# TurakhiaLab/TWILIGHT

Hardware: AMD Instinct MI355X
Metric: DP band cells/s, TALCO-XDrop progressive profile-profile alignment (bit-exact vs reference CPU path) (higher is better)
Workload: dtype f32

## Files before the change

include/twl_align.h:

```cpp
#ifndef TWL_ALIGN_H
#define TWL_ALIGN_H

#include <stdint.h>

#ifdef __cplusplus
extern "C" {
#endif

#define TWL_MAX_MATRIX 21
#define TWL_MAX_MARKER 1024

enum twl_status {
    TWL_OK = 0,
    TWL_ERR_NOT_INITIALIZED = -1,
    TWL_ERR_BAD_ARGUMENT = -2,
    TWL_ERR_HIP = -3,
    TWL_ERR_UNSUPPORTED = -4
};

typedef struct twl_params {
    int32_t P;
    float   matrix[TWL_MAX_MATRIX * TWL_MAX_MATRIX];
    float   gap_open;
    float   gap_extend;
    float   gap_boundary;
    float   gap_char;
    int32_t xdrop;
    int32_t flen;
    int32_t marker;
} twl_params;

typedef struct twl_stats {
    uint64_t band_cells;
    uint64_t nominal_cells;
    double   kernel_ms;
    double   pack_ms;
    double   total_ms;
    int32_t  n_launches;
    int32_t  n_relaunched;
    int32_t  window;
    int32_t  grid;
    int32_t  matrix_mode;
    int32_t  speculative;
    int32_t  mt_tiles_predicted;
    int32_t  mt_tiles_inline;
    int32_t  mt_scouts_failed;
    int32_t  reserved;
    char     kernel[160];
} twl_stats;

int  twl_init(const int *device_ids, int n_devices);
void twl_shutdown(void);
const char *twl_last_error(void);
const char *twl_version(void);

int twl_align_batch(const twl_params *p, int32_t n_pairs, int32_t seq_len,
                    const float *freq, const float *gap_open, const float *gap_extend,
                    const int32_t *len, const int32_t *num,
                    int8_t *aln_out, int32_t *aln_len_out, int16_t *err_out);

int twl_align_batch_device(int device, void *stream, const twl_params *p, int32_t n_pairs, int32_t seq_len,
                           const float *d_freq, const float *d_gap_open, const float *d_gap_extend,
                           const int32_t *d_len, const int32_t *d_num,
                           int8_t *d_aln_out, int32_t *d_aln_len_out, int16_t *d_err_out);

void *twl_host_alloc(uint64_t bytes);
void  twl_host_free(void *p);

int twl_copy_to_device(int device, void *dst_dev, const void *src, uint64_t bytes);
int twl_copy_from_device(int device, void *dst, const void *src_dev, uint64_t bytes);
int twl_copy_rows_from_device(int device, void *dst, uint64_t dst_pitch, const void *src_dev, uint64_t src_pitch, uint64_t width, uint64_t rows);

int twl_get_stats(int device, twl_stats *out);

int twl_get_pair_cells(int device, uint64_t *cells_out, int32_t n);

int twl_column_scores(const twl_params *p, int32_t seq_len, const float *freq, const int32_t *len, const int32_t *num, float *out);

int twl_dp_column_scores(const twl_params *p, int32_t seq_len, const float *freq, const float *gap_open, const float *gap_extend,
                         const int32_t *len, const int32_t *num, float *out);

#define TWL_COMM_ID_BYTES 128
int twl_comm_unique_id(void *id128);
int twl_comm_init(int device, int rank, int world, const void *id128);
int twl_comm_all_gather(int device, const void *d_send, void *d_recv, int64_t bytes_per_rank);
int twl_comm_all_gather_host(int device, const void *send, void *recv, int64_t bytes_per_rank);
int twl_comm_destroy(int device);

enum twl_knob { TWL_KNOB_MT_PERTURB = 1, TWL_KNOB_MT_MAX_PAIRS = 2, TWL_KNOB_MT_MIN_MARKER = 3, TWL_KNOB_MT_LEAD = 4, TWL_KNOB_MT_MARGIN = 5,
                TWL_KNOB_MT_ROUNDS = 6, TWL_KNOB_MT_THR_JOBS = 7, TWL_KNOB_FAIL_ROW_ALLOCS = 8,
                TWL_KNOB_PROT_MODE = 9, TWL_KNOB_ASSUME_ONEHOT_QUERY = 10, TWL_KNOB_MT_TAIL_PCT = 11, TWL_KNOB_MT_WIDE = 12, TWL_KNOB_NO_SPEC = 13, TWL_KNOB_SCOUT_XDROP_PCT = 14, TWL_KNOB_THR_SMALL = 15, TWL_KNOB_FORCE_GLOBAL = 16, TWL_KNOB_LEAF_STEP = 17, TWL_KNOB_POISON_TB = 18, TWL_KNOB_MT_ANCHOR = 19, TWL_KNOB_MT_LEAD2 = 20, TWL_KNOB_PROT_CORRIDOR = 21 };
int twl_set_knob(int key, int value);
int twl_plan_describe(const twl_params *p, int32_t n_pairs, const int32_t *len, int32_t num_cu, int32_t qry_onehot, int32_t wide_streak, char *out, int32_t cap);

#ifdef __cplusplus
}
#endif
#endif
```

include/twl_level.h:

```cpp
#ifndef TWL_LEVEL_H
#define TWL_LEVEL_H

#include "twl_align.h"

#ifdef __cplusplus
extern "C" {
#endif

typedef struct twl_store twl_store;

typedef struct twl_side {
    int32_t n_members;
    int32_t member_off;
    int32_t len;
    int32_t num;
    float   weight;
    int32_t cache_id;
    int32_t store_id;
    int32_t reserved;
} twl_side;

int  twl_store_create(int device, char type, int32_t n_seqs, const char *const *seqs, const int32_t *lens, twl_store **out);
void twl_store_destroy(twl_store *s);
int  twl_store_read_rows(twl_store *s, char *const *rows_out, int32_t *lens_out);
int  twl_store_read_rows_of(twl_store *s, int32_t n_ids, const int32_t *ids, char *out, int32_t *lens_out);
int  twl_store_write_rows(twl_store *s, int32_t n_ids, const int32_t *ids, const char *in, const int32_t *lens);
int  twl_store_write_cache(twl_store *s, int32_t id, const float *data, int32_t len);
int  twl_store_rows_to_block(twl_store *s, int32_t n_ids, const int32_t *ids, void *dev_block, int32_t *lens_out);
int  twl_store_rows_from_block(twl_store *s, int32_t n_ids, const int32_t *ids, const int32_t *lens, const void *dev_block);
int  twl_store_exchange_buffers(twl_store *s, int64_t send_bytes, int64_t recv_bytes, void **send_dev, void **recv_dev);
int  twl_store_read_cache(twl_store *s, int32_t id, float *out, int32_t *len_out);
int  twl_store_drop_cache(twl_store *s, int32_t id);

int twl_level_prepare(twl_store *s, const twl_params *p, float gappy_threshold, int32_t n_pairs, const twl_side *sides,
                      const int32_t *members, const float *member_weight, int32_t seq_len, int32_t *len_out, uint8_t *colinfo_out);

int twl_level_read_colinfo(twl_store *s, int32_t pair, int32_t side, uint8_t *out);
int twl_level_read_colinfo_many(twl_store *s, int32_t n_sel, const int32_t *pairs, uint8_t *out);

int twl_level_align(twl_store *s, const twl_params *p, const uint8_t *run_mask, int8_t *aln_out, int32_t *aln_len_out, int16_t *err_out);
int twl_level_align_mixed(twl_store *s, const twl_params *p, const uint8_t *run_mask, const uint8_t *zero_gap, int8_t *aln_out, int32_t *aln_len_out, int16_t *err_out);

int twl_level_read_path(twl_store *s, int32_t pair, int8_t *out, int32_t len);
int twl_level_read_paths(twl_store *s, int32_t n_sel, const int32_t *pairs, const int32_t *lens, int8_t *out, int32_t out_stride);

int twl_level_restore(twl_store *s, const twl_params *p, int32_t n_sel, const int32_t *pairs, int32_t out_stride, int32_t *final_len_out);
int twl_level_exchange_buffers(twl_store *s, int64_t send_bytes, int64_t recv_bytes, void **send_dev, void **recv_dev);
int twl_level_paths_to_block(twl_store *s, int32_t n_sel, const int32_t *pairs, const int32_t *lens, const uint8_t *where, void *blk_dev, const int64_t *blk_off);
int twl_level_paths_from_block(twl_store *s, int32_t n_sel, const int32_t *pairs, const int32_t *lens, const void *blk_dev, const int64_t *blk_off);
int twl_level_write_final(twl_store *s, int32_t pair, const int8_t *path, int32_t len);
int twl_level_read_final(twl_store *s, int32_t pair, int8_t *out, int32_t len);

int twl_level_commit(twl_store *s, const int8_t *paths, const int32_t *path_len, int32_t path_stride);

int twl_level_commit_from_dp(twl_store *s, const int8_t *paths, const int32_t *path_len, int32_t path_stride, const uint8_t *from_dp);

int twl_level_read_columns(twl_store *s, int32_t pair, int32_t side, float *out, int32_t max_cols);

int twl_level_timing(twl_store *s, double *prepare_ms, double *commit_ms);

#ifdef __cplusplus
}
#endif
#endif
```

twilight_amd/api.py:

```python
from __future__ import annotations

import ctypes as C
import os

import numpy as np

_HERE = os.path.dirname(os.path.abspath(__file__))
LIB_PATH = os.environ.get("TWL_LIB") or os.path.join(_HERE, "libtwl_align.so")
TWL_MAX_MATRIX = 21

_lib = None


class TwlError(RuntimeError):
    pass


class TwlParams(C.Structure):
    _fields_ = [("P", C.c_int32), ("matrix", C.c_float * (TWL_MAX_MATRIX * TWL_MAX_MATRIX)), ("gap_open", C.c_float),
                ("gap_extend", C.c_float), ("gap_boundary", C.c_float), ("gap_char", C.c_float), ("xdrop", C.c_int32),
                ("flen", C.c_int32), ("marker", C.c_int32)]


class TwlStats(C.Structure):
    _fields_ = [("band_cells", C.c_uint64), ("nominal_cells", C.c_uint64), ("kernel_ms", C.c_double),
                ("pack_ms", C.c_double), ("total_ms", C.c_double), ("n_launches", C.c_int32),
                ("n_relaunched", C.c_int32), ("window", C.c_int32), ("grid", C.c_int32), ("matrix_mode", C.c_int32), ("speculative", C.c_int32),
                ("mt_tiles_predicted", C.c_int32), ("mt_tiles_inline", C.c_int32), ("mt_scouts_failed", C.c_int32), ("reserved", C.c_int32),
                ("kernel", C.c_char * 160)]


_SYMBOLS = ["twl_init", "twl_shutdown", "twl_last_error", "twl_version", "twl_align_batch", "twl_align_batch_device",
            "twl_get_stats", "twl_get_pair_cells", "twl_column_scores", "twl_dp_column_scores", "twl_host_alloc", "twl_host_free", "twl_set_knob",
            "twl_copy_to_device", "twl_copy_from_device", "twl_copy_rows_from_device",
            "twl_comm_unique_id", "twl_comm_init", "twl_comm_all_gather", "twl_comm_all_gather_host", "twl_comm_destroy", "twl_plan_describe"]


def exported_symbols():
    return list(_SYMBOLS)


def load_library():
    global _lib
    if _lib is None:
        if not os.path.exists(LIB_PATH):
            raise TwlError(f"{LIB_PATH} not built: run `python -c 'import __graft_entry__ as g; g.build()'`")
        try:
            import torch
        except Exception:
            pass
        lib = C.CDLL(LIB_PATH)
        lib.twl_last_error.restype = C.c_char_p
        lib.twl_version.restype = C.c_char_p
        lib.twl_init.restype = C.c_int
        lib.twl_align_batch.restype = C.c_int
        lib.twl_align_batch_device.restype = C.c_int
        lib.twl_get_stats.restype = C.c_int
        lib.twl_get_pair_cells.restype = C.c_int
        lib.twl_column_scores.restype = C.c_int
        lib.twl_dp_column_scores.restype = C.c_int
        lib.twl_shutdown.restype = None
        lib.twl_set_knob.restype = C.c_int
        _lib = lib
    return _lib


def _check(rc):
    if rc != 0:
        raise TwlError(f"libtwl_align error {rc}: {load_library().twl_last_error().decode()}")


def make_params(matrix, *, gap_open=-50.0, gap_extend=-5.0, gap_boundary=None, gap_char=None, xdrop=None, flen=4096,
                marker=1024) -> TwlParams:
    m = np.asarray(matrix, dtype=np.float32)
    n = m.shape[0]
    p = TwlParams()
    p.P = n + 1
    flat = np.zeros(TWL_MAX_MATRIX * TWL_MAX_MATRIX, dtype=np.float32)
    flat[: n * n] = m.reshape(-1)
    p.matrix[:] = flat.tolist()
    p.gap_open = gap_open
    p.gap_extend = gap_extend
    p.gap_boundary = gap_extend if gap_boundary is None else gap_boundary
    p.gap_char = gap_extend if gap_char is None else gap_char
    p.xdrop = int(1000 * -gap_extend) if xdrop is None else int(xdrop)
    p.flen = flen
    p.marker = marker
    return p


def init(device_ids=None):
    lib = load_library()
    if device_ids is None:
        _check(lib.twl_init(None, 0))
    else:
        arr = (C.c_int * len(device_ids))(*device_ids)
        _check(lib.twl_init(arr, len(device_ids)))


def shutdown():
    load_library().twl_shutdown()


def _ptr(a, ty):
    return a.ctypes.data_as(C.POINTER(ty))


def align_batch(params: TwlParams, batch):
    lib = load_library()
    n, sl = batch.n_pairs, batch.seq_len
    freq = np.ascontiguousarray(batch.freq, dtype=np.float32)
    go = np.ascontiguousarray(batch.gap_open, dtype=np.float32)
    ge = np.ascontiguousarray(batch.gap_extend, dtype=np.float32)
    ln = np.ascontiguousarray(batch.len, dtype=np.int32)
    nm = np.ascontiguousarray(batch.num, dtype=np.int32)
    aln = np.zeros((n, 2 * sl), dtype=np.int8)
    aln_len = np.zeros(n, dtype=np.int32)
    err = np.zeros(n, dtype=np.int16)
    _check(lib.twl_align_batch(C.byref(params), C.c_int32(n), C.c_int32(sl), _ptr(freq, C.c_float), _ptr(go, C.c_float),
                               _ptr(ge, C.c_float), _ptr(ln, C.c_int32), _ptr(nm, C.c_int32), _ptr(aln, C.c_int8),
                               _ptr(aln_len, C.c_int32), _ptr(err, C.c_int16)))
    return aln, aln_len, err


def align_batch_device(params: TwlParams, n_pairs, seq_len, d_freq, d_gop, d_gex, d_len, d_num, d_aln, d_aln_len, d_err,
                       device=0, stream=None):
    lib = load_library()
    vp = C.c_void_p
    _check(lib.twl_align_batch_device(C.c_int(device), vp(stream or 0), C.byref(params), C.c_int32(n_pairs), C.c_int32(seq_len),
                                      vp(d_freq), vp(d_gop), vp(d_gex), vp(d_len), vp(d_num), vp(d_aln), vp(d_aln_len),
                                      vp(d_err)))


KNOB_MT_PERTURB, KNOB_MT_MAX_PAIRS, KNOB_MT_MIN_MARKER, KNOB_MT_LEAD, KNOB_MT_MARGIN, KNOB_MT_ROUNDS, KNOB_MT_THR_JOBS, KNOB_FAIL_ROW_ALLOCS = 1, 2, 3, 4, 5, 6, 7, 8
KNOB_PROT_MODE, KNOB_ASSUME_ONEHOT_QUERY, KNOB_MT_TAIL_PCT, KNOB_MT_WIDE, KNOB_NO_SPEC, KNOB_SCOUT_XDROP_PCT = 9, 10, 11, 12, 13, 14
KNOB_THR_SMALL = 15
KNOB_FORCE_GLOBAL = 16
KNOB_LEAF_STEP = 17
KNOB_POISON_TB = 18
KNOB_MT_ANCHOR = 19
KNOB_PROT_CORRIDOR = 21
KNOB_MT_LEAD2 = 20
PROT_MODES = {"auto": 0, "dense": 1, "sparse": 2, "presim": 3, "r1": 4, "lean_sparse": 5, "lean_presim": 6}


def set_knob(key: int, value: int):
    _check(load_library().twl_set_knob(C.c_int(key), C.c_int(value)))


def plan_describe(params, lens, num_cu=256, qry_onehot=False, wide_streak=0, small_state=0) -> str:
    wide_streak = int(wide_streak) + (100000 * (32 + int(small_state)) if small_state else 0)
    lens = np.ascontiguousarray(lens, dtype=np.int32)
    buf = C.create_string_buffer(256)
    _check(load_library().twl_plan_describe(C.byref(params), C.c_int32(lens.shape[0]), _ptr(lens, C.c_int32), C.c_int32(num_cu), C.c_int32(int(qry_onehot)), C.c_int32(wide_streak), buf, C.c_int32(256)))
    return buf.value.decode()


def version() -> str:
    return load_library().twl_version().decode()


def get_stats(device=0) -> TwlStats:
    st = TwlStats()
    _check(load_library().twl_get_stats(C.c_int(device), C.byref(st)))
    return st


def get_pair_cells(n, device=0):
    out = np.zeros(n, dtype=np.uint64)
    _check(load_library().twl_get_pair_cells(C.c_int(device), _ptr(out, C.c_uint64), C.c_int32(n)))
    return out


def column_scores(params: TwlParams, ref: np.ndarray, qry: np.ndarray, ref_num: int, qry_num: int) -> np.ndarray:
    ref = np.ascontiguousarray(ref, dtype=np.float32)
    qry = np.ascontiguousarray(qry, dtype=np.float32)
    R, Q, P = ref.shape[0], qry.shape[0], ref.shape[1]
    sl = max(R, Q)
    freq = np.zeros((2, sl, P), dtype=np.float32)
    freq[0, :R] = ref
    freq[1, :Q] = qry
    ln = np.array([R, Q], dtype=np.int32)
    nm = np.array([ref_num, qry_num], dtype=np.int32)
    out = np.zeros((Q, R), dtype=np.float32)
    _check(load_library().twl_column_scores(C.byref(params), C.c_int32(sl), _ptr(freq, C.c_float), _ptr(ln, C.c_int32), _ptr(nm, C.c_int32), _ptr(out, C.c_float)))
    return out


def dp_column_scores(params: TwlParams, batch, pair: int = 0) -> np.ndarray:
    sl = batch.seq_len
    freq = np.ascontiguousarray(batch.freq[pair], dtype=np.float32)
    gop = np.ascontiguousarray(batch.gap_open[pair], dtype=np.float32)
    gex = np.ascontiguousarray(batch.gap_extend[pair], dtype=np.float32)
    ln = np.ascontiguousarray(batch.len[pair], dtype=np.int32)
    nm = np.ascontiguousarray(batch.num[pair], dtype=np.int32)
    out = np.zeros((int(ln[1]), int(ln[0])), dtype=np.float32)
    _check(load_library().twl_dp_column_scores(C.byref(params), C.c_int32(sl), _ptr(freq, C.c_float), _ptr(gop, C.c_float), _ptr(gex, C.c_float),
                                               _ptr(ln, C.c_int32), _ptr(nm, C.c_int32), _ptr(out, C.c_float)))
    return out
```

twilight_amd/csrc/host/align_resident.cpp:

```cpp
#include "align_gpu.hpp"

#include <cstring>
#include <omp.h>

#include <algorithm>
#include <cstdio>
#include <cstdlib>
#include <iostream>
#include <string>
#include <thread>

namespace msa {
namespace progressive {
namespace gpu {

namespace {

inline twl_store *firstStore(const RunCtx &ctx) { return ctx.stores.empty() ? nullptr : ctx.stores[0]; }

std::vector<RunCtx::Raw> g_alnStage;
RunCtx::Raw g_finalStage, g_infoStage;

void createStore(RunCtx &ctx, SequenceDB *db, Option *option)
{
    const int n = (int)db->sequences.size();
    std::vector<const char *> rows(n);
    std::vector<int32_t> lens(n);
    for (int i = 0; i < n; ++i) {
        auto *s = db->sequences[i];
        if (s->id != i) { std::cerr << "ERROR: sequence ids are not dense.\n"; exit(1); }
        rows[i] = s->alnStorage[s->storage];
        lens[i] = s->len;
    }
    ctx.storeDev = selectedDevices();
    if (option->testVirtualDevices > 0) ctx.storeDev.assign((size_t)option->testVirtualDevices, selectedDevices()[0]);
    ctx.stores.assign(ctx.storeDev.size(), nullptr);
    std::vector<std::thread> th;
    std::vector<std::pair<int, std::string>> res(ctx.storeDev.size(), {TWL_OK, ""});
    for (size_t d = 0; d < ctx.storeDev.size(); ++d)
        th.emplace_back([&, d] {
            const int rc = twl_store_create(ctx.storeDev[d], option->type, n, rows.data(), lens.data(), &ctx.stores[d]);
            if (rc != TWL_OK) res[d] = {rc, twl_last_error()};
        });
    for (auto &t : th) t.join();
    for (auto &r : res)
        if (r.first != TWL_OK) { std::cerr << "ERROR: twl_store_create failed (" << r.first << "): " << r.second << '\n'; exit(1); }
}

template <class F>
void onAllStores(RunCtx &ctx, const char *what, F fn)
{
    const size_t nd = ctx.stores.size();
    std::vector<std::pair<int, std::string>> res(nd, {TWL_OK, ""});
    if (nd == 1) { const int rc = fn(0); if (rc != TWL_OK) res[0] = {rc, twl_last_error()}; }
    else {
        std::vector<std::thread> th;
        for (size_t d = 0; d < nd; ++d)
            th.emplace_back([&, d] { const int rc = fn((int)d); if (rc != TWL_OK) res[d] = {rc, twl_last_error()}; });
        for (auto &t : th) t.join();
    }
    for (auto &r : res)
        if (r.first != TWL_OK) { std::cerr << "ERROR: " << what << " failed (" << r.first << "): " << r.second << '\n'; exit(1); }
}

void materialise(Tree *T, SequenceDB *db, Option *option)
{
    RunCtx &ctx = ctxOf(db);
    if (!firstStore(ctx)) return;
    const double t0 = nowMs();
    const int n = (int)db->sequences.size();
    std::vector<int32_t> lens(n);
    int rc = twl_store_read_rows(firstStore(ctx), nullptr, lens.data());
    if (rc != TWL_OK) die("twl_store_read_rows", rc);
    std::vector<char *> rows(n);
    size_t total = 0;
    for (int i = 0; i < n; ++i) total += (size_t)lens[i];
    free(db->rowArena);
    db->rowArena = static_cast<char *>(malloc(2 * total + 1));
    if (!db->rowArena) { std::cerr << "ERROR: out of host memory for the final rows.\n"; exit(1); }
    size_t at = 0;
    for (int i = 0; i < n; ++i) {
        auto *s = db->sequences[i];
        if (!s->borrowed) { free(s->alnStorage[0]); free(s->alnStorage[1]); }
        s->borrowed = true;
        s->alnStorage[s->storage] = db->rowArena + at;
        s->alnStorage[!s->storage] = db->rowArena + total + at;
        s->memLen = lens[i];
        rows[i] = s->alnStorage[s->storage];
        at += (size_t)lens[i];
    }
    rc = twl_store_read_rows(firstStore(ctx), rows.data(), lens.data());
    if (rc != TWL_OK) die("twl_store_read_rows", rc);
    for (int i = 0; i < n; ++i) db->sequences[i]->len = lens[i];
    const int P = (option->type == 'n') ? 6 : 22;
    std::vector<Node *> keep{T->root};
    keep.insert(keep.end(), db->fallback_nodes.begin(), db->fallback_nodes.end());
    for (Node *nd : keep) {
        if (nd->cacheId < 0) continue;
        int32_t len = 0;
        if ((rc = twl_store_read_cache(firstStore(ctx), nd->cacheId, nullptr, &len)) != TWL_OK) die("twl_store_read_cache", rc);
        std::vector<float> flat((size_t)len * P);
        if ((rc = twl_store_read_cache(firstStore(ctx), nd->cacheId, flat.data(), &len)) != TWL_OK) die("twl_store_read_cache", rc);
        nd->msaFreq.assign(len, std::vector<float>(P));
        for (int t = 0; t < len; ++t) std::copy(&flat[(size_t)t * P], &flat[(size_t)t * P] + P, nd->msaFreq[t].begin());
        nd->cacheId = -1;
    }
    for (twl_store *st : ctx.stores) twl_store_destroy(st);
    ctx.stores.clear();
    ctx.finished = true;
    if (option->printDetail) std::cerr << "Rows back on the host in " << nowMs() - t0 << " ms\n";
}

struct PathRoute { bool procs, devX, inPlace; };
PathRoute routeOf(const Shard &sh, int nd)
{
    PathRoute r;
    r.procs = sh.world > 1;
    r.devX = (nd == 1 && (sh.exchangeDev != nullptr || sh.rccl));
    r.inPlace = (nd == 1 && ((!r.procs && !sh.exchange && !sh.rccl) || r.devX));
    return r;
}

struct Level {
    const RunCtx &ctx;
    const NodePairVec &nodes;
    SequenceDB *database;
    Option *option;
    Params &param;
    int task, n, nd;
    const char *letters;
    bool removal;
    PathRoute route;
    twl_params tp, tz;
    std::vector<twl_side> sides;
    std::vector<PairShape> ps;
    std::vector<int32_t> members;
    std::vector<float> weights;
    int stride = 1;
    int pathStride = 1;
    std::vector<int> needInfo;
    std::vector<char> needsHost;
    std::vector<uint8_t> maskZero;
    std::vector<char> takesPart;
    std::vector<int> owner;
    int meBase = 0;
    Level(const RunCtx &c, const NodePairVec &nv, SequenceDB *db, Option *o, Params &p)
        : ctx(c), nodes(nv), database(db), option(o), param(p), task(db->currentTask), n((int)nv.size()), nd((int)c.stores.size()),
          letters(consensusLetters(o->type)), removal(!(o->gappyVertical == 1.0)), route(routeOf(c.shard, nd)), tp(baseParams(p)), tz(tp)
    {
        tz.gap_char = 0;
    }
};

struct PairRows {
    std::vector<alnPath> paths;
    std::vector<int16_t> errs;
    std::vector<uint8_t> fromDp;
    std::vector<int32_t> dpLen;
    std::vector<ColumnInfo> cols;
    explicit PairRows(int n) : paths(n), errs(n, 0), fromDp(n, 0), dpLen(n, 0), cols(n) {}
};

struct ReplicaShare {
    double callMs = 0, totMs = 0;
    LevelRecord part;
    uint64_t nominalCells = 0;
    std::vector<int32_t> handedBack, handedBackLen;
};

void describeLevel(Level &lv, RunCtx &ctx, NodePairVec &nodes)
{
    const int n = lv.n;
    SequenceDB *database = lv.database;
    Option *option = lv.option;
    std::vector<twl_side> &sides = lv.sides;
    sides.resize(2 * (size_t)n);
    lv.ps.resize(n);
    size_t nMembers = 0;
#pragma omp parallel for schedule(static) if (n >= 512)
    for (int i = 0; i < n; ++i) {
        Node *nd[2] = {nodes[i].first, nodes[i].second};
        PairShape &s = lv.ps[i];
        s.refLen = nd[0]->getAlnLen(0); s.qryLen = nd[1]->getAlnLen(0);
        s.refNum = nd[0]->getAlnNum(0); s.qryNum = nd[1]->getAlnNum(0);
        for (int sd = 0; sd < 2; ++sd) {
            twl_side &x = sides[2 * (size_t)i + sd];
            x.n_members = (int32_t)nd[sd]->seqsIncluded.size();
            x.len = sd ? s.qryLen : s.refLen;
            x.num = sd ? s.qryNum : s.refNum;
            x.weight = nd[sd]->alnWeight;
            x.cache_id = nd[sd]->cacheId;
            x.store_id = -1;
            x.reserved = 0;
        }
        s.lowQ_r = lowQualitySide(option->alnMode == MERGE_MSA, s.refNum, firstSeqLowQuality(nd[0], database));
        s.lowQ_q = lowQualitySide(option->alnMode == MERGE_MSA, s.qryNum, firstSeqLowQuality(nd[1], database));
    }
    for (int i = 0; i < n; ++i) {
        const PairShape &s = lv.ps[i];
        Node *nd[2] = {nodes[i].first, nodes[i].second};
        const bool storeFreq = (s.refNum >= option->calProfileTh || s.qryNum >= option->calProfileTh) || (sides[2 * (size_t)i].cache_id >= 0 || sides[2 * (size_t)i + 1].cache_id >= 0);
        for (int sd = 0; sd < 2; ++sd) {
            twl_side &x = sides[2 * (size_t)i + sd];
            x.member_off = (int32_t)nMembers;
            if (storeFreq && x.cache_id < 0) x.store_id = nd[sd]->cacheId = ctx.nextCacheId++;
            nMembers += (size_t)x.n_members;
            lv.stride = std::max(lv.stride, x.len);
        }
        lv.pathStride = std::max(lv.pathStride, s.refLen + s.qryLen);
    }
    lv.members.resize(nMembers);
    lv.weights.resize(nMembers);
#pragma omp parallel for schedule(dynamic, 16) if (n >= 64)
    for (int i = 0; i < n; ++i) {
        Node *nd[2] = {nodes[i].first, nodes[i].second};
        for (int sd = 0; sd < 2; ++sd) {
            const twl_side &x = sides[2 * (size_t)i + sd];
            const float groupWeight = nd[sd]->alnWeight;
            for (int m = 0; m < x.n_members; ++m) {
                const int sIdx = nd[sd]->seqsIncluded[m];
                if (sIdx < 0) { std::cerr << "ERROR: compressed sequence group in device-resident mode.\n"; exit(1); }
                lv.members[x.member_off + m] = sIdx;
                lv.weights[x.member_off + m] = database->sequences[sIdx]->weight / groupWeight * x.num;
            }
        }
    }
}

void prepareOnReplicas(Level &lv, RunCtx &ctx)
{
    const int n = lv.n;
    std::vector<int32_t> lens(2 * (size_t)n);
    std::vector<std::vector<int32_t>> lensOf(lv.nd);
    onAllStores(ctx, "twl_level_prepare", [&](int d) {
        lensOf[d].resize(2 * (size_t)n);
        return twl_level_prepare(ctx.stores[d], &lv.tp, lv.option->gappyVertical, n, lv.sides.data(), lv.members.data(), lv.weights.data(), lv.stride,
                                 d == 0 ? lens.data() : lensOf[d].data(), nullptr);
    });
    for (int d = 1; d < lv.nd; ++d)
        if (lensOf[d] != lens) { std::cerr << "ERROR: device replicas disagree on the prepared level.\n"; exit(1); }
    lv.needsHost.assign(n, 0);
    for (int i = 0; i < n; ++i) {
        PairShape &s = lv.ps[i];
        s.lens = {lens[2 * i], lens[2 * i + 1]};
        if (s.lens.first != s.refLen || s.lens.second != s.qryLen) { lv.needInfo.push_back(i); lv.needsHost[i] = 1; }
    }
}

void fetchColumnInfo(const Level &lv, const std::vector<int> &which, bool wholeBlock, std::vector<ColumnInfo> &cols)
{
    if (which.empty()) return;
    const size_t stride = (size_t)lv.stride;
    uint8_t *info = reinterpret_cast<uint8_t *>(g_infoStage.get(2 * (wholeBlock ? (size_t)lv.n : which.size()) * stride));
    const int rc = wholeBlock ? twl_level_read_colinfo(firstStore(lv.ctx), -1, 0, info)
                              : twl_level_read_colinfo_many(firstStore(lv.ctx), (int32_t)which.size(), which.data(), info);
    if (rc != TWL_OK) die(wholeBlock ? "twl_level_read_colinfo" : "twl_level_read_colinfo_many", rc);
#pragma omp parallel for schedule(dynamic, 4)
    for (int t = 0; t < (int)which.size(); ++t) {
        const int i = which[t];
        const size_t slot = wholeBlock ? (size_t)i : (size_t)t;
        runsAndConsensus(&info[2 * slot * stride], lv.ps[i].refLen, lv.removal, lv.letters, cols[i].gappy.first, cols[i].consensus.first);
        runsAndConsensus(&info[(2 * slot + 1) * stride], lv.ps[i].qryLen, lv.removal, lv.letters, cols[i].gappy.second, cols[i].consensus.second);
    }
}

void planDp(Level &lv, PairRows &rows)
{
    const int n = lv.n;
    lv.maskZero.assign(n, 0);
    lv.takesPart.assign(n, 0);
    std::vector<long long> cost(n, 0);
    for (int i = 0; i < n; ++i) {
        const PairShape &s = lv.ps[i];
        rows.paths[i] = trivialPath(s);
        cost[i] = (long long)s.lens.first + s.lens.second;
        if (!goesToDp(s)) continue;
        lv.takesPart[i] = 1;
        lv.maskZero[i] = zeroGapChar(lv.task, s) ? 1 : 0;
    }
    lv.owner = dealPairs(cost, lv.takesPart, lv.route.procs ? lv.ctx.shard.world : lv.nd);
    lv.meBase = lv.route.procs ? lv.ctx.shard.rank : 0;
}

void addStats(const Level &lv, int d, bool firstCall, ReplicaShare &mine)
{
    const bool ownDevice = lv.nd == 1 || lv.ctx.storeDev[d] != lv.ctx.storeDev[(d + 1) % lv.nd];
    const bool nominal = firstCall && d == 0;
    twl_stats st{};
    if ((!ownDevice && !nominal) || twl_get_stats(lv.ctx.storeDev[d], &st) != TWL_OK) return;
    if (ownDevice) { foldStats(mine.part, st); mine.part.kernel_ms += st.kernel_ms; mine.totMs += st.total_ms; }
    if (nominal) mine.nominalCells += st.nominal_cells;
}

int retryDeferredPair(const Level &lv, int d, const std::vector<uint8_t> &mask, int8_t *aln, std::vector<int32_t> &alnLen, std::vector<int16_t> &err, ReplicaShare &mine)
{
    if (lv.n != 1) { std::cerr << "ERROR: a deferred-pass (task 1) level must hold exactly one pair; this one has " << lv.n << ".\n"; return (int)TWL_ERR_UNSUPPORTED; }
    if (!mask[0]) return (int)TWL_OK;
    twl_params tr = lv.maskZero[0] ? lv.tz : lv.tp;
    const uint8_t one = 1;
    int rc = TWL_OK;
    retryUntilPassed(tr, err[0], std::min(lv.ps[0].lens.first, lv.ps[0].lens.second), [&](const twl_params &grown) {
        if (lv.option->printDetail) std::cout << "Retry pair No. " << 0 << "\txdrop " << grown.xdrop << " flen " << grown.flen << '\n';
        const double tRetry = nowMs();
        rc = twl_level_align(lv.ctx.stores[d], &grown, &one, aln, alnLen.data(), err.data());
        if (rc != TWL_OK) return (int16_t)0;
        mine.callMs += nowMs() - tRetry;
        addStats(lv, d, false, mine);
        return err[0];
    });
    return rc;
}

int sortResults(const Level &lv, int d, const std::vector<uint8_t> &mask, const int8_t *aln, const std::vector<int32_t> &alnLen, const std::vector<int16_t> &err,
                PairRows &rows, ReplicaShare &mine)
{
    const size_t pitch = (size_t)2 * lv.stride;
    std::vector<int32_t> restore, restoreLen;
    for (int i = 0; i < lv.n; ++i) {
        if (!mask[i]) continue;
        rows.errs[i] = err[i];
        const int32_t len = (err[i] == 0) ? alnLen[i] : 0;
        if (!lv.route.inPlace) rows.paths[i].assign(&aln[i * pitch], &aln[i * pitch] + len);
        else if (lv.needsHost[i]) {
            if (len > 0 && !deferredLowQuality(lv.task, lv.ps[i])) { restore.push_back(i); restoreLen.push_back(len); } else rows.paths[i].clear();
        }
        else if (len > 0) { rows.fromDp[i] = 1; rows.dpLen[i] = len; }
    }
    if (restore.empty()) return (int)TWL_OK;
    std::vector<int32_t> fin(restore.size(), -1);
    const int rc = twl_level_restore(lv.ctx.stores[d], &lv.tp, (int32_t)restore.size(), restore.data(), lv.pathStride, fin.data());
    if (rc != TWL_OK) return rc;
    for (size_t t = 0; t < restore.size(); ++t) {
        if (fin[t] > 0) { rows.fromDp[restore[t]] = 2; rows.dpLen[restore[t]] = fin[t]; }
        else { mine.handedBack.push_back(restore[t]); mine.handedBackLen.push_back(restoreLen[t]); }
    }
    return (int)TWL_OK;
}

int alignShare(const Level &lv, int d, PairRows &rows, ReplicaShare &mine)
{
    const int n = lv.n;
    std::vector<uint8_t> mask(n, 0);
    int cnt = 0, cntZero = 0;
    for (int i = 0; i < n; ++i) if (lv.takesPart[i] && lv.owner[i] == lv.meBase + d) { mask[i] = 1; ++cnt; cntZero += lv.maskZero[i]; }
    if (!cnt) return (int)TWL_OK;
    int8_t *aln = lv.route.inPlace ? nullptr : reinterpret_cast<int8_t *>(g_alnStage[d].get((size_t)n * 2 * lv.stride));
    std::vector<int32_t> alnLen(n);
    std::vector<int16_t> err(n);
    const double tCall = nowMs();
    const int rc = (cntZero == cnt) ? twl_level_align(lv.ctx.stores[d], &lv.tz, mask.data(), aln, alnLen.data(), err.data())
                                    : twl_level_align_mixed(lv.ctx.stores[d], &lv.tp, mask.data(), cntZero ? lv.maskZero.data() : nullptr, aln, alnLen.data(), err.data());
    if (rc != TWL_OK) return rc;
    mine.callMs += nowMs() - tCall;
    addStats(lv, d, true, mine);
    if (lv.task == 1) {
        const int rr = retryDeferredPair(lv, d, mask, aln, alnLen, err, mine);
        if (rr != TWL_OK) return rr;
    }
    return sortResults(lv, d, mask, aln, alnLen, err, rows, mine);
}

#ifdef TWL_DEV
void dumpSchedule(const Level &lv, const PairRows &rows)
{
    const char *dump = getenv("TWL_DUMP_SCHEDULE");
    FILE *f = dump ? fopen(dump, "a") : nullptr;
    if (!f) return;
    std::vector<uint64_t> pc(lv.n, 0);
    if (lv.nd == 1) (void)twl_get_pair_cells(lv.ctx.storeDev[0], pc.data(), lv.n);
    for (int i = 0; i < lv.n; ++i)
        fprintf(f, "%d %d %d %d %d %d %d %llu\n", (int)lv.ctx.levels.size(), i, lv.nodes[i].first->seqsIncluded.empty() ? -1 : lv.nodes[i].first->seqsIncluded[0],
                lv.nodes[i].second->seqsIncluded.empty() ? -1 : lv.nodes[i].second->seqsIncluded[0], lv.ps[i].lens.first, lv.ps[i].lens.second, (int)rows.errs[i], (unsigned long long)pc[i]);
    fclose(f);
}
#endif

void mergeShares(const std::vector<ReplicaShare> &shares, RunCtx &ctx, LevelRecord &rec)
{
    double callMs = 0, totMs = 0;
    for (const ReplicaShare &s : shares) {
        callMs = std::max(callMs, s.callMs); totMs = std::max(totMs, s.totMs);
        rec.kernel_ms = std::max(rec.kernel_ms, s.part.kernel_ms);
        rec.band_cells += s.part.band_cells;
        rec.relaunched += s.part.relaunched;
    }
    const LevelRecord &p0 = shares[0].part;
    rec.matrix_mode = p0.matrix_mode; rec.speculative = p0.speculative; memcpy(rec.kernel, p0.kernel, sizeof rec.kernel);
    rec.mt_predicted += p0.mt_predicted; rec.mt_inline += p0.mt_inline;
    ctx.totals.call_ms += callMs;
    ctx.totals.total_ms += totMs;
    ctx.totals.nominal_cells += shares[0].nominalCells;
}

void postCheck(const Level &lv, int i, int alnRef, int alnQry)
{
    const PairShape &s = lv.ps[i];
    if (alnRef != s.refLen) std::cout << "R: Post " << lv.nodes[i].first->identifier << "(" << alnRef << "/" << s.refLen << ")\n";
    if (alnQry != s.qryLen) std::cout << "Q: Post " << lv.nodes[i].second->identifier << "(" << alnQry << "/" << s.qryLen << ")\n";
}

void joinHandedBack(const Level &lv, const ReplicaShare &share, PairRows &rows)
// ... 81 lines not shown
}

const char *consensusLetters(char type)
{
    static const char bases[] = {'A', 'C', 'G', 'T', 'N'};
    static const char acids[] = {'A', 'C', 'D', 'E', 'F', 'G', 'H', 'I', 'K', 'L', 'M', 'N', 'P', 'Q', 'R', 'S', 'T', 'V', 'W', 'Y', 'X'};
    return type == 'n' ? bases : acids;
}

IntPair restoreOnHost(alnPath &dp, ColumnInfo &cols, Params &param, int pathStride, alnPath &full)
{
    auto covers = [](const alnPath &p) { IntPair c{0, 0}; for (auto a : p) { c.first += a != 1; c.second += a != 2; } return c; };
    alignment_helper::addGappyColumnsBack(dp, full, cols.gappy, param, covers(dp), cols.consensus);
    if ((int)full.size() > pathStride) { std::cerr << "ERROR: path longer than both profiles together.\n"; exit(1); }
    return covers(full);
}

std::vector<int32_t> restoreHandedBack(twl_store *st, Params &param, const Option &option, const AlignedLevel &lv, const std::vector<int32_t> &pairs,
                                       const std::vector<int32_t> &dpLen, const std::function<void(int, int, int)> &post)
{
    const size_t sl = (size_t)lv.stride, m = pairs.size();
    const bool removal = !(option.gappyVertical == 1.0f);
    const char *letters = consensusLetters(option.type);
    std::vector<uint8_t> info(m * 2 * sl);
    std::vector<int8_t> raw(m * 2 * sl);
    int rc = twl_level_read_colinfo_many(st, (int32_t)m, pairs.data(), info.data());
    if (rc != TWL_OK) die("twl_level_read_colinfo_many", rc);
    if ((rc = twl_level_read_paths(st, (int32_t)m, pairs.data(), dpLen.data(), raw.data(), (int32_t)(2 * sl))) != TWL_OK) die("twl_level_read_paths", rc);
    std::vector<int32_t> fin(m);
    for (size_t k = 0; k < m; ++k) {
        const int32_t i = pairs[k];
        ColumnInfo c;
        runsAndConsensus(&info[2 * k * sl], lv.sideLen[2 * i], removal, letters, c.gappy.first, c.consensus.first);
        runsAndConsensus(&info[(2 * k + 1) * sl], lv.sideLen[2 * i + 1], removal, letters, c.gappy.second, c.consensus.second);
        alnPath dp(&raw[2 * k * sl], &raw[2 * k * sl] + dpLen[k]), full;
        const IntPair covers = restoreOnHost(dp, c, param, lv.pathStride, full);
        if (post) post(i, covers.first, covers.second);
        if ((rc = twl_level_write_final(st, i, full.data(), (int32_t)full.size())) != TWL_OK) die("twl_level_write_final", rc);
        fin[k] = (int32_t)full.size();
    }
    return fin;
}

FinalPaths finalPathsOfLevel(twl_store *st, const twl_params &tp, Params &param, const Option &option, const AlignedLevel &lv)
{
    FinalPaths f;
    f.fromDp.assign((size_t)lv.n, 0);
    f.pathLen.assign((size_t)lv.n, 0);
    std::vector<int32_t> sel;
    for (int32_t i = 0; i < lv.n; ++i) {
        if (lv.err[i] != 0) continue;
        f.pathLen[i] = lv.alnLen[i];
        f.fromDp[i] = 1;
        if (lv.lenOut[2 * i] < lv.sideLen[2 * i] || lv.lenOut[2 * i + 1] < lv.sideLen[2 * i + 1]) sel.push_back(i);
    }
    if (sel.empty()) return f;
    std::vector<int32_t> fin(sel.size(), -1), host, hostLen;
    const int rc = twl_level_restore(st, &tp, (int32_t)sel.size(), sel.data(), lv.pathStride, fin.data());
    if (rc != TWL_OK) die("twl_level_restore", rc);
    for (size_t k = 0; k < sel.size(); ++k) {
        f.fromDp[sel[k]] = 2;
        if (fin[k] > 0) f.pathLen[sel[k]] = fin[k];
        else { host.push_back(sel[k]); hostLen.push_back(lv.alnLen[sel[k]]); }
    }
    if (!host.empty()) {
        const std::vector<int32_t> full = restoreHandedBack(st, param, option, lv, host, hostLen);
        for (size_t k = 0; k < host.size(); ++k) f.pathLen[host[k]] = full[k];
        f.restoredOnHost = (int)host.size();
    }
    return f;
}

void alignWithRetry(twl_store *st, int device, const twl_params &prm, const Option &option, const std::string *retryWhat, const int16_t *knownErr, int32_t minLen,
                    int32_t *alnLen, int16_t *err, DpTotals &tot)
{
    auto runOnce = [&](const twl_params &p) {
        const int rc = twl_level_align(st, &p, nullptr, nullptr, alnLen, err);
        if (rc != TWL_OK) die("twl_level_align", rc);
        twl_stats ss{};
        if (twl_get_stats(device, &ss) == TWL_OK) { tot.cells += ss.band_cells; tot.kernel += ss.kernel_ms; }
        return err[0];
    };
    const int16_t first = knownErr ? *knownErr : runOnce(prm);
    if (!retryWhat) return;
    twl_params tr = prm;
    retryUntilPassed(tr, first, minLen, [&](const twl_params &grown) {
        ++tot.retries;
        if (option.printDetail) std::cout << "Retry " << *retryWhat << "\txdrop " << grown.xdrop << " flen " << grown.flen << '\n';
        return runOnce(grown);
    });
}

void runsAndConsensus(const uint8_t *info, int len, bool removal, const char *letters, IntPairVec &runs, std::string &cons)
{
    cons.resize(len);
    int start = -1;
    for (int t = 0; t < len; ++t) {
        cons[t] = letters[info[t] & 0x7f];
        if (!removal) continue;
        if (info[t] & 0x80) { if (start < 0) start = t; }
        else if (start >= 0) { runs.push_back({start, t - start}); start = -1; }
    }
    if (removal && start >= 0) runs.push_back({start, len - start});
}

void uploadSequences(SequenceDB *database, Option *option)
{
    RunCtx &ctx = ctxOf(database);
    if (firstStore(ctx) || ctx.finished) return;
    ensureInit(option);
    const double t0 = nowMs();
    createStore(ctx, database, option);
    for (auto *s : database->sequences) {
        if (!s->borrowed) { free(s->alnStorage[0]); free(s->alnStorage[1]); }
        s->alnStorage[0] = s->alnStorage[1] = nullptr;
        s->borrowed = true;
        s->memLen = 0;
    }
    if (option->printDetail) std::cerr << "Sequences resident on " << ctx.stores.size() << " device replica(s) in " << nowMs() - t0 << " ms\n";
    database->afterMainPass = [database, option](Tree *tree) { materialise(tree, database, option); };
    database->residentDeferred = true;
}

void downloadRows(SequenceDB *database, Tree *T)
{
    if (database->afterMainPass) { database->afterMainPass(T); database->afterMainPass = nullptr; }
}

void alignmentKernel_Resident(Tree *T, NodePairVec &nodes, SequenceDB *database, Option *option, Params &param)
{
    RunCtx &ctx = ctxOf(database);
    const int task = database->currentTask;
    if ((task != 0 && task != 1) || ctx.finished) {
        if (firstStore(ctx)) materialise(T, database, option);
        alignmentKernel_GPU(T, nodes, database, option, param);
        return;
    }
    refuseCpuOnly(option);
    ensureInit(option);
    uploadSequences(database, option);
    if (ctx.shard.world > 1 && ctx.stores.size() > 1) { std::cerr << "ERROR: several processes with several device replicas each are not supported.\n"; exit(1); }
    LevelRecord rec;
    rec.pairs = (int32_t)nodes.size();
    rec.task = task;
    const LevelTotals before = ctx.totals;
    const double tPrep = nowMs();
    const int n = (int)nodes.size(), nd = (int)ctx.stores.size();
    Level level(ctx, nodes, database, option, param);
    describeLevel(level, ctx, nodes);
    prepareOnReplicas(level, ctx);
    const Level &lv = level;
    PairRows rows(n);
    if (!lv.route.inPlace) fetchColumnInfo(lv, lv.needInfo, lv.needInfo.size() * 8 > (size_t)n, rows.cols);
    ctx.totals.prepare_ms += nowMs() - tPrep;

    planDp(level, rows);
    std::vector<ReplicaShare> shares(nd);
    if (g_alnStage.size() < (size_t)nd) g_alnStage.resize((size_t)nd);
    onAllStores(ctx, "twl_level_align", [&](int d) { return alignShare(lv, d, rows, shares[d]); });
#ifdef TWL_DEV
    dumpSchedule(lv, rows);
#endif
    mergeShares(shares, ctx, rec);
    joinHandedBack(lv, shares[0], rows);
    exchange(lv, ctx, rows, rec);
    std::vector<int> fallbackPairs = judgeFailures(lv, rows);

    const double tFin = nowMs();
    std::vector<int32_t> finalLen(n, 0);
    std::vector<char> deferred(n, 0);
    const int8_t *finalPaths = finalPathsOnHost(lv, rows, finalLen, deferred);
    const double tGappy = nowMs() - tFin;
    commitAndBookkeep(lv, ctx, nodes, finalPaths, finalLen, rows);
    ctx.totals.finish_ms += nowMs() - tFin;
    double devPrep = 0, devCommit = 0;
    if (option->printDetail) twl_level_timing(firstStore(ctx), &devPrep, &devCommit);
    ctx.totals.dev_prepare_ms += devPrep;
    ctx.totals.dev_commit_ms += devCommit;
    closeLevel(ctx, rec, tPrep, deferred, fallbackPairs, nodes, database, option);
    if (option->printDetail)
        std::cerr << "  phases (ms): prepare " << ctx.totals.prepare_ms - before.prepare_ms << " (device " << devPrep << ") call " << ctx.totals.call_ms - before.call_ms
                  << " (kernel " << rec.kernel_ms << ", exchange " << rec.exchange_ms << ") finish " << ctx.totals.finish_ms - before.finish_ms << " (device " << devCommit
                  << ") whole " << nowMs() - tPrep << "; relaunched pairs " << ctx.totals.relaunched - before.relaunched << "; pairs with removed columns " << lv.needInfo.size() << "; restored on the host " << shares[0].handedBack.size() << "; gappy columns back " << tGappy << " ms\n";
}

}
}
}
```

twilight_amd/csrc/host/progressive.cpp:

```cpp
#include "twl_host.hpp"

#include <algorithm>
#include <chrono>
#include <iostream>
#include <unordered_map>

namespace msa {
namespace progressive {

void getProgressivePairs(std::vector<std::pair<NodePair, int>> &alnOrder, std::stack<Node *> postStack, int grpID, int mode)
{
    struct LevelOf {
        std::vector<int> lvl;
        std::vector<const Node *> own;
        int &operator[](Node *n)
        {
            const int k = n->schedIdx;
            if (k < 0 || k >= (int)lvl.size() || own[k] != n) { n->schedIdx = (int)lvl.size(); lvl.push_back(-1); own.push_back(n); }
            return lvl[n->schedIdx];
        }
    } levelOf;
    levelOf.lvl.reserve(postStack.size() + 16);
    levelOf.own.reserve(postStack.size() + 16);
    auto nextLevel = [&](Node *id) { const int l = levelOf[id]; return l < 0 ? 0 : l + 1; };
    if (mode == 0) {
        std::vector<Node *> children, left;
        for (; !postStack.empty(); postStack.pop()) {
            Node *node = postStack.top();
            if (!(node->grpID == -1 || node->grpID == grpID) || node->is_leaf()) continue;
            children.clear();
            for (Node *c : node->children)
                if (c->grpID == grpID) children.push_back(c);
            if (children.empty() && node->seqsIncluded.empty()) {
                node->grpID = -2;
                auto &sib = node->parent->children;
                for (auto it = sib.begin(); it != sib.end(); ++it)
                    if ((*it)->identifier == node->identifier) { sib.erase(it); break; }
                continue;
            }
            if (children.size() == 1 && node->parent != nullptr && node->seqsIncluded.empty() && node->parent->grpID == grpID) {
                for (auto &slot : node->parent->children)
                    if (slot->identifier == node->identifier) {
                        slot = children[0];
                        children[0]->branchLength += node->branchLength;
                        children[0]->parent = node->parent;
                        break;
                    }
                continue;
            }
            while (children.size() > 1) {
                left.clear();
                for (size_t i = 0; i + 1 < children.size(); i += 2) {
                    const int lvl = std::max(nextLevel(children[i]), nextLevel(children[i + 1]));
                    levelOf[children[i]] = lvl;
                    levelOf[children[i + 1]] = lvl;
                    alnOrder.push_back({{children[i], children[i + 1]}, lvl});
                    left.push_back(children[i]);
                }
                if (children.size() % 2 == 1) left.push_back(children.back());
                children.swap(left);
            }
            if (children.size() == 1 && !node->seqsIncluded.empty()) {
                const int lvl = std::max(nextLevel(node), nextLevel(node->children[0]));
                levelOf[node] = lvl;
                levelOf[node->children[0]] = lvl;
                alnOrder.push_back({{node, node->children[0]}, lvl});
            }
            { const int l = levelOf[children[0]]; levelOf[node] = l; }
        }
    } else if (mode == 1) {
        for (; !postStack.empty(); postStack.pop()) {
            Node *node = postStack.top();
            if (node->parent == nullptr) continue;
            const int lvl = std::max(nextLevel(node), nextLevel(node->parent));
            levelOf[node] = lvl;
            levelOf[node->parent] = lvl;
            alnOrder.push_back({{node->parent, node}, lvl});
        }
    } else {
        for (; !postStack.empty(); postStack.pop())
            if (postStack.top()->parent != nullptr) alnOrder.push_back({{postStack.top()->parent, postStack.top()}, 0});
    }
}

void scheduling(Node *root, std::vector<NodePairVec> &levels, int mode)
{
    levels.clear();
    std::stack<Node *> post;
    root->collectPostOrder(post);
    std::vector<std::pair<NodePair, int>> pairs;
    getProgressivePairs(pairs, post, root->grpID, mode);
    for (auto &h : pairs) {
        if (levels.size() < (size_t)h.second + 1) levels.resize(h.second + 1);
        levels[h.second].push_back(h.first);
    }
}

static void materialise(Node *n, Node *partner, SequenceDB *db)
{
    if (n->is_leaf() && n->seqsIncluded.empty()) {
        auto *s = db->name_map.find(n->identifier)->second;
        n->seqsIncluded.push_back(s->id);
        n->alnLen = s->len;
        n->alnNum = 1;
        n->alnWeight = s->weight;
    } else if (n->seqsIncluded.empty()) {
        const int grp = n->grpID;
        for (Node *c : n->children) {
            if ((c->grpID == -1 || c->grpID == grp) && c->identifier != partner->identifier) {
                n->msaFreq = c->msaFreq;
                c->msaFreq.clear();
                n->cacheId = c->cacheId;
                c->cacheId = -1;
                n->seqsIncluded = std::move(c->seqsIncluded);
                c->seqsIncluded.clear();
                n->alnLen = c->alnLen;
                n->alnNum = c->alnNum;
                n->alnWeight = c->alnWeight;
                break;
            }
        }
    }
}

void updateNode(Tree *, NodePairVec &nodes, SequenceDB *database)
{
    const int n = (int)nodes.size();
#pragma omp parallel for schedule(static) if (n >= 512)
    for (int i = 0; i < n; ++i) {
        materialise(nodes[i].first, nodes[i].second, database);
        materialise(nodes[i].second, nodes[i].first, database);
    }
}

void progressiveAlignment(Tree *T, SequenceDB *database, Option *option, std::vector<NodePairVec> &levels, Params &param, alnFunction kernel)
{
    int level = 0;
    if (option->printDetail) std::cerr << "Total " << levels.size() << " levels.\n";
    size_t done = 0;
    if (database->ownedPrefix && database->currentTask == 0) done = database->ownedPrefix(T, levels, option, param);
    for (auto m : levels) {
        if ((size_t)level < done) { ++level; continue; }
        auto t0 = std::chrono::high_resolution_clock::now();
        updateNode(T, m, database);
        auto t1 = std::chrono::high_resolution_clock::now();
        kernel(T, m, database, option, param);
        auto ms = std::chrono::duration_cast<std::chrono::milliseconds>(std::chrono::high_resolution_clock::now() - t0).count();
        if (option->printDetail)
            std::cerr << "Level " << level + 1 << ", aligned " << m.size() << (m.size() > 1 ? " pairs in " : " pair in ") << ms << " ms (nodes "
                      << std::chrono::duration<double, std::milli>(t1 - t0).count() << " ms)\n";
        ++level;
    }
}

void updateAlignment(Node *node, SequenceDB *database)
{
    const int n = (int)database->sequences.size();
#pragma omp parallel for schedule(dynamic, 16)
    for (int idx = 0; idx < n; ++idx) {
        auto *s = database->sequences[idx];
        if (s->subtreeIdx >= -1) continue;
        const alnPath &aln = database->subtreeAln[s->subtreeIdx];
        s->memCheck((int)aln.size());
        const char *from = s->alnStorage[s->storage];
        char *to = s->alnStorage[1 - s->storage];
        int org = 0;
        for (size_t k = 0; k < aln.size(); ++k) to[k] = (aln[k] == 0) ? from[org++] : '-';
        s->len = (int)aln.size();
        s->changeStorage();
    }
    std::vector<int> members;
    for (int sIdx : node->seqsIncluded)
        if (sIdx >= 0) members.push_back(sIdx);
    for (auto *s : database->sequences)
        if (s->subtreeIdx < 0) members.push_back(s->id);
    node->seqsIncluded = members;
}

namespace {
struct UnionFind {
    std::vector<int> p;
    int find(int x) { while (p[x] != x) { p[x] = p[p[x]]; x = p[x]; } return x; }
    void unite(int a, int b) { a = find(a); b = find(b); if (a != b) p[std::max(a, b)] = std::min(a, b); }
};
}
OwnershipPlan planOwnership(Tree *T, const std::vector<NodePairVec> &levels, int world)
{
    OwnershipPlan plan;
    const int nLevels = (int)levels.size();
    if (world <= 1 || nLevels < 2) return plan;
    const long long want = 8ll * world;
    std::vector<long long> above((size_t)nLevels + 1, 0);
    for (int l = nLevels - 1; l >= 0; --l) above[l] = above[l + 1] + (long long)levels[l].size();
    int cut = -1;
    for (int l = nLevels - 2; l >= 0; --l)
        if (above[l + 1] + 1 >= want) { cut = l; break; }
    if (cut < 0) return plan;
    std::unordered_map<const Node *, int> idOf;
    auto id = [&](const Node *n) { auto it = idOf.find(n); if (it != idOf.end()) return it->second; const int k = (int)idOf.size(); idOf.emplace(n, k); return k; };
    const int grp = T->root->grpID;
    auto adopts = [&](const Node *c) { return c->grpID == -1 || c->grpID == grp; };
    for (int l = 0; l <= cut; ++l)
        for (auto &pr : levels[l])
            for (const Node *x : {pr.first, pr.second}) {
                id(x);
                if (!x->is_leaf()) for (const Node *c : x->children) if (adopts(c)) id(c);
            }
    UnionFind uf;
    uf.p.resize(idOf.size());
    for (size_t k = 0; k < uf.p.size(); ++k) uf.p[k] = (int)k;
    for (int l = 0; l <= cut; ++l)
        for (auto &pr : levels[l]) {
            uf.unite(idOf[pr.first], idOf[pr.second]);
            for (const Node *x : {pr.first, pr.second})
                if (!x->is_leaf()) for (const Node *c : x->children) if (adopts(c)) uf.unite(idOf[x], idOf[c]);
        }
    std::unordered_map<int, long long> cost;
    std::vector<int> firstSeen;
    for (int l = 0; l <= cut; ++l)
        for (auto &pr : levels[l]) { const int c = uf.find(idOf[pr.first]); if (!cost.count(c)) firstSeen.push_back(c); cost[c] += 1; }
    std::vector<std::pair<long long, int>> order;
    for (size_t k = 0; k < firstSeen.size(); ++k) order.push_back({cost[firstSeen[k]], (int)k});
    std::sort(order.begin(), order.end(), [](const std::pair<long long, int> &a, const std::pair<long long, int> &b) { return a.first != b.first ? a.first > b.first : a.second < b.second; });
    std::unordered_map<int, int> ownerOf;
    plan.load.assign((size_t)world, 0);
    for (auto &c : order) {
        const int r = (int)(std::min_element(plan.load.begin(), plan.load.end()) - plan.load.begin());
        ownerOf[firstSeen[(size_t)c.second]] = r;
        plan.load[r] += c.first;
    }
    plan.cut = cut;
    plan.subtrees = (int)order.size();
    plan.owner.resize((size_t)cut + 1);
    for (int l = 0; l <= cut; ++l) {
        plan.owner[l].resize(levels[l].size());
        for (size_t i = 0; i < levels[l].size(); ++i) plan.owner[l][i] = ownerOf[uf.find(idOf[levels[l][i].first])];
    }
    return plan;
}

void msaOnSubtree(Tree *T, SequenceDB *database, Option *option, Params &param, alnFunction kernel, alnFunction deferredKernel)
{
    auto t0 = std::chrono::high_resolution_clock::now();
    std::cerr << "============================\n";
    std::vector<NodePairVec> levels;
    scheduling(T->root, levels, database->currentTask == 0 ? 0 : 1);
    if (option->printDetail) std::cerr << "Levels scheduled in " << std::chrono::duration<double, std::milli>(std::chrono::high_resolution_clock::now() - t0).count() << " ms\n";
    progressiveAlignment(T, database, option, levels, param, kernel);
    const auto tLoop = std::chrono::high_resolution_clock::now();
    if (database->currentTask == 0) {
        Node *last = levels.back()[0].first;
        T->root->seqsIncluded = last->seqsIncluded;
        if (!last->msaFreq.empty()) T->root->msaFreq = last->msaFreq;
        if (last->cacheId >= 0) { T->root->cacheId = last->cacheId; last->cacheId = -1; }
        T->root->alnLen = last->alnLen;
        T->root->alnNum = last->alnNum;
        T->root->alnWeight = last->alnWeight;
        last->seqsIncluded.clear();
        last->msaFreq.clear();
        const bool stayResident = database->fallback_nodes.empty() ? database->lazyRows : database->residentDeferred;
        if (database->afterMainPass && !stayResident) { database->afterMainPass(T); database->afterMainPass = nullptr; }
    }
    if (database->fallback_nodes.empty()) updateAlignment(T->root, database);
    if (option->printDetail) std::cerr << "After the last level: " << std::chrono::duration<double, std::milli>(std::chrono::high_resolution_clock::now() - tLoop).count() << " ms\n";
    auto secs = std::chrono::duration_cast<std::chrono::seconds>(std::chrono::high_resolution_clock::now() - t0).count();
    std::cerr << "Alignment (length: " << T->root->alnLen << ") completed in " << secs << " s\n";
    if (database->fallback_nodes.empty()) return;

    database->currentTask = 1;
    int deferredSeqs = 0;
    levels.clear();
    for (Node *bad : database->fallback_nodes) deferredSeqs += (int)bad->seqsIncluded.size();
    std::sort(database->fallback_nodes.begin(), database->fallback_nodes.end(), [&](Node *&a, Node *&b) {
        if (a->alnNum == b->alnNum) return a->getAlnLen(database->currentTask) > b->getAlnLen(database->currentTask);
        return a->alnNum > b->alnNum;
    });
    for (Node *bad : database->fallback_nodes) levels.push_back(NodePairVec(1, {T->root, bad}));
    std::cerr << "Realign profiles that have been deferred. Total profiles/sequences: " << database->fallback_nodes.size() << " / " << deferredSeqs << '\n';
    database->fallback_nodes.clear();
    progressiveAlignment(T, database, option, levels, param, deferredKernel);
    if (database->afterMainPass && !database->lazyRows) { database->afterMainPass(T); database->afterMainPass = nullptr; }
    updateAlignment(T->root, database);
    database->currentTask = 0;
}

}
}
```

twilight_amd/csrc/host/twl_host.hpp:

```cpp
#pragma once
#include "level_policy.hpp"

#include <cstdint>
#include <cstdlib>
#include <functional>
#include <map>
#include <stack>
#include <string>
#include <unordered_map>
#include <unordered_set>
#include <utility>
#include <vector>

namespace phylogeny {

using Profile = std::vector<std::vector<float>>;

struct Node {
    Node(const std::string &id, float len);
    Node(const std::string &id, Node *par, float len);
    bool is_leaf() const { return identifier.compare(0, 4, "node") != 0; }
    void collectPostOrder(std::stack<Node *> &postStack);

    std::string identifier;
    Node *parent = nullptr;
    float branchLength = 0;
    size_t level = 1;
    std::vector<Node *> children;
    size_t numLeaves = 0;
    float weight = 0;
    bool placed = false;
    int grpID = -1;
    int schedIdx = -1;

    std::vector<int> seqsIncluded;
    Profile msaFreq;
    int cacheId = -1;
    int alnLen = 0;
    int alnNum = 0;
    float alnWeight = 0;
    int getAlnNum(int) const { return alnNum; }
    int getAlnLen(int) const { return alnLen; }
};

struct Tree {
    size_t m_currInternalNode = 0;
    size_t m_maxDepth = 0;
    size_t m_numLeaves = 0;
    float m_meanDepth = 0;
    Node *root = nullptr;
    std::unordered_map<std::string, Node *> allNodes;

    std::string newInternalNodeId() { return "node_" + std::to_string(++m_currInternalNode); }
    void calLeafNum();
    void calSeqWeight();
    void parseNewick(std::string &newick);
    void reroot();
    void convert2binaryTree();
    Tree *prune(std::unordered_set<std::string> &seqs);

    Tree() = default;
    explicit Tree(const std::string &newickFileName);
    Tree(Node *node, bool reroot);
    ~Tree();
};

void pruneTree(Tree *&T, std::unordered_set<std::string> &seqs);
void updateLevels(Node *node, size_t currentLevel);
void assignSinglePartition(Node *root);

}

char checkOnly(char c);
int letterIdx(char type, char c);

namespace msa {

enum Type { DEFAULT_ALN = 0, MERGE_MSA = 1, PLACE_WO_TREE = 2, PLACE_W_TREE = 3 };

using Node = phylogeny::Node;
using Tree = phylogeny::Tree;
using NodePair = std::pair<Node *, Node *>;
using NodePairVec = std::vector<NodePair>;
using stringPair = std::pair<std::string, std::string>;
using IntPair = std::pair<int, int>;
using IntPairVec = std::vector<IntPair>;
using FloatPair = std::pair<float, float>;
using alnPath = std::vector<int8_t>;
using Profile = std::vector<std::vector<float>>;

struct Option {
    int alnMode = DEFAULT_ALN;
    int gpuNum = 0;
    int cpuNum = 1;
    std::vector<int> gpuIdx;
    bool cpuOnly = false;
    int maxSubtree = INT32_MAX;
    float gappyVertical = 0.95f;
    float lenDev = 0;
    float maxAmbig = 0.1f;
    int maxLen = INT32_MAX;
    int minLen = 0;
    bool writeFiltered = false;
    bool debug = false;
    bool noFilter = true;
    bool reroot = true;
    bool compressed = false;
    char type = 'n';
    bool alignGappy = true;
    std::string treeFile, seqFile, outFile;
    bool printDetail = false;
    int calProfileTh = 1000, updateSeqTh = 1000;
    bool testForkHostStaged = false;
    bool testNoOwnership = false;
    int testVirtualDevices = 0;
    bool hostStaged = false;
    std::string backboneAlnFile;
    int testPlaceChunk = 0;
    std::string msaDir;
    bool typeGiven = false;
    float match = 18, mismatch = -8, transition = -4, gapOpen = -50, gapExtend = -5, xdrop = 600;
    bool hasGapEnds = false;
    float gapEnds = 0;
    bool wildcard = false;
    int blosum = 62;
    std::string matrixFile;
};

struct Params {
    float gapOpen, gapExtend, gapBoundary, xdrop, scaleFactor = 1;
    float **scoringMatrix;
    int matrixSize;
    Params(const Option &opt, char type);
    ~Params();
    Params(const Params &) = delete;
};

struct SequenceDB {
    struct SequenceInfo {
        int id;
        std::string name;
        std::string unalignedSeq;
        int len;
        bool lowQuality = false;
        int subtreeIdx;
        float weight;
        bool storage = false;
        bool borrowed = false;
        int memLen = 0;
        char *alnStorage[2] = {nullptr, nullptr};
        static constexpr int timesBigger = 2;
        void changeStorage() { storage = !storage; }
        void memCheck(int len);
        SequenceInfo(int id_, const std::string &name_, std::string &seq, int subtreeIdx_, float weight_, bool debug);
        ~SequenceInfo();
    };
    int currentTask = 0;
    int updateSeqTh = 1000;
    std::vector<SequenceInfo *> sequences;
    std::vector<Node *> fallback_nodes;
    std::unordered_map<std::string, SequenceInfo *> name_map;
    std::unordered_map<int, alnPath> subtreeAln;
    char *rowArena = nullptr;
    void *gpuCtx = nullptr;
    void (*gpuCtxFree)(void *) = nullptr;
    std::function<size_t(Tree *, std::vector<std::vector<std::pair<Node *, Node *>>> &, Option *, Params &)> ownedPrefix;
    std::function<void(Tree *)> afterMainPass;
    bool residentDeferred = false;
    bool lazyRows = false;
    void addSequence(int id, const std::string &name, std::string &seq, int subtreeIdx, float weight, bool debug);
    bool debug();
    ~SequenceDB();
};

namespace io {
void readSequences(const std::string &fileName, SequenceDB *database, Option *option, Tree *&T);
void writeAlignment(const std::string &fileName, SequenceDB *database, int alnLen);
void writeFinalMSA(SequenceDB *database, Option *option, int alnLen);
char detectType(const std::string &seqFile);
void readRecords(const std::string &fileName, const std::function<void(std::string &, std::string &)> &each);
int32_t readAlignedRows(const std::string &fileName, const char *kind, std::vector<std::string> &names, std::vector<std::string> &rows);
void writeRecords(const std::string &fileName, const std::vector<const std::string *> &names, const std::vector<const char *> &rows, int W);
}

using alnFunction = std::function<void(Tree *, NodePairVec &, SequenceDB *, Option *, Params &)>;

namespace alignment_helper {
void calculateProfile(float *profile, NodePair &nodes, SequenceDB *database, Option *option, int32_t memLen);
void removeGappyColumns(float *hostFreq, NodePair &nodes, Option *option, std::pair<IntPairVec, IntPairVec> &gappyColumns, int32_t memLen,
                        IntPair &lens, int currentTask);
void calculatePSGP(float *hostFreq, float *hostGapOp, float *hostGapEx, NodePair &nodes, SequenceDB *database, Option *option, int memLen,
                   IntPair offset, IntPair lens, Params &param);
void getConsensus(Option *option, float *profile, std::string &consensus, int len);
void pairwiseGlobal(const std::string &seq1, const std::string &seq2, alnPath &path, Params &param);
void addGappyColumnsBack(alnPath &aln_before, alnPath &aln_after, std::pair<IntPairVec, IntPairVec> &gappyColumns, Params &param,
                         IntPair rgcLens, stringPair orgSeqs);
void updateAlignment(NodePair &nodes, SequenceDB *database, Option *option, alnPath &aln);
void updateFrequency(NodePair &nodes, SequenceDB *database, alnPath &aln, FloatPair weights);
void fallback2cpu(std::vector<int> &fallbackPairs, NodePairVec &nodes, SequenceDB *database, Option *option);
}

namespace progressive {
void getProgressivePairs(std::vector<std::pair<NodePair, int>> &alnOrder, std::stack<Node *> postStack, int grpID, int mode);
void scheduling(Node *root, std::vector<NodePairVec> &levels, int mode);
void updateNode(Tree *tree, NodePairVec &nodes, SequenceDB *database);
void progressiveAlignment(Tree *T, SequenceDB *database, Option *option, std::vector<NodePairVec> &levels, Params &param, alnFunction kernel);
struct OwnershipPlan { int cut = -1; int subtrees = 0; std::vector<std::vector<int>> owner; std::vector<long long> load; };
OwnershipPlan planOwnership(Tree *T, const std::vector<NodePairVec> &levels, int world);
void msaOnSubtree(Tree *T, SequenceDB *database, Option *option, Params &param, alnFunction kernel, alnFunction deferredKernel);
void updateAlignment(Node *node, SequenceDB *database);

struct FloatBuf {
    std::vector<float> own;
    float *ext = nullptr;
    float *data() { return ext ? ext : own.data(); }
    const float *data() const { return ext ? ext : own.data(); }
    void assign(size_t n, float v) { ext = nullptr; own.assign(n, v); }
    void bind(float *slot, size_t n) { ext = slot; std::fill(slot, slot + n, 0.0f); }
};
struct PairInputs : PairShape {
    FloatBuf freq, gapOp, gapEx;
    std::pair<IntPairVec, IntPairVec> gappyColumns;
    stringPair consensus;
    int32_t memLen;
};
inline bool firstSeqLowQuality(const Node *node, const SequenceDB *database)
{
    const int s = node->seqsIncluded.empty() ? -1 : node->seqsIncluded[0];
    return s >= 0 && s < (int)database->sequences.size() && database->sequences[s]->lowQuality;
}
void preparePair(NodePair &nodes, SequenceDB *database, Option *option, Params &param, PairInputs &in, float *freqSlot = nullptr,
                 float *gapOpSlot = nullptr, float *gapExSlot = nullptr, int stride = 0);
bool finishPair(NodePair &nodes, SequenceDB *database, Option *option, Params &param, PairInputs &in, alnPath &aln_wo_gc);

namespace gpu {
void alignmentKernel_GPU(Tree *T, NodePairVec &alnPairs, SequenceDB *database, Option *option, Params &param);
void beginInit(Option *option);
void alignmentKernel_Resident(Tree *T, NodePairVec &alnPairs, SequenceDB *database, Option *option, Params &param);
struct LevelTotals { uint64_t band_cells = 0, pairs = 0, relaunched = 0, nominal_cells = 0 ; double kernel_ms = 0, total_ms = 0, prepare_ms = 0, stage_ms = 0, call_ms = 0, finish_ms = 0, dev_prepare_ms = 0, dev_commit_ms = 0, exchange_ms = 0; };
struct LevelRecord { int32_t pairs = 0, task = 0; uint64_t band_cells = 0, relaunched = 0; double kernel_ms = 0, level_ms = 0, exchange_ms = 0; int32_t matrix_mode = -1, speculative = 0;
                     int32_t mt_predicted = 0, mt_inline = 0; char kernel[160] = {0}; };
using ExchangeFn = int (*)(void *user, const void *send, int64_t bytes_per_rank, void *recv);
struct Shard { int rank = 0, world = 1; ExchangeFn exchange = nullptr; void *user = nullptr; ExchangeFn exchangeDev = nullptr; void *userDev = nullptr;
               bool rccl = false; };
int initRcclShard(SequenceDB *database, Option *option, int rank, int world, const void *id128);
void ensureDevicesUp(Option *option);
size_t ownedPrefix(Tree *T, std::vector<NodePairVec> &levels, SequenceDB *database, Option *option, Params &param);
struct RunCtx;
RunCtx &ctxOf(SequenceDB *database);
void setShard(SequenceDB *database, const Shard &shard);
const std::vector<LevelRecord> &levelRecords(SequenceDB *database);
const LevelTotals &runTotals(SequenceDB *database);
void uploadSequences(SequenceDB *database, Option *option);
void downloadRows(SequenceDB *database, Tree *T);
}

}

int runDefaultAlignment(Option &option, alnFunction kernel, alnFunction deferredKernel, bool writeOutput = true,
                        const std::function<void(SequenceDB *)> &atEnd = nullptr, const std::function<void(SequenceDB *)> &beforeAlign = nullptr);
bool parseCommandLine(int argc, char **argv, Option &option, bool allowPlacement = false, bool allowMerge = false);
int runPlacement(Option &option);
int runMerge(Option &option);

}
```

twilight_amd/csrc/level_kernels.hip.h:

```cpp
#pragma once
#include <hip/hip_runtime.h>
#include <stdint.h>

namespace twl {

struct SideDesc {
    int32_t n_members;
    int32_t member_off;
    int32_t len;
    int32_t num;
    float weight;
    int32_t cache_slot;
    int32_t store_slot;
    int32_t pad;
};

struct LevelArgs {
    const SideDesc *sides;
    const int32_t *member_seq;
    const float *member_w;
    const uint8_t *member_plane;
    const char *rows0, *rows1;
    int64_t cap;
    float *const *cache;
    const uint8_t *lut;
    float *raw;
    uint8_t *colinfo;
    float *cols;
    int32_t *len_out;
    int32_t *chunk_cnt;
    int32_t n_chunks;
    int32_t stride;
    float gappy_thr;
    int32_t remove;
    float gap_open, gap_extend, scale, min_gap_open, min_gap_extend;
};

template <int P>
__global__ void __launch_bounds__(256) profile_kernel(LevelArgs a)
{
    __shared__ uint8_t s_lut[256];
    __shared__ int s_kept[4];
    s_lut[threadIdx.x] = a.lut[threadIdx.x];
    __syncthreads();
    const int side = blockIdx.x;
    const SideDesc sd = a.sides[side];
    const int t0 = 4 * (blockIdx.y * 256 + threadIdx.x);
    const int nc = max(0, min(4, sd.len - t0));
    int kept = 0;
    if (nc > 0) {
    float acc[4][P];
#pragma unroll
    for (int k = 0; k < 4; ++k)
#pragma unroll
        for (int v = 0; v < P; ++v) acc[k][v] = 0.0f;
    const float fnum = (float)sd.num;
    if (sd.cache_slot >= 0) {
        const float *c = a.cache[sd.cache_slot] + (size_t)t0 * P;
#pragma unroll
        for (int k = 0; k < 4; ++k)
            if (k < nc) {
#pragma unroll
                for (int v = 0; v < P; ++v) acc[k][v] = c[k * P + v] / sd.weight * fnum;
            }
    } else {
        constexpr int U = (P == 6) ? 16 : 2;
        auto add = [&](uint32_t four, float w) __attribute__((always_inline)) {
#pragma unroll
            for (int k = 0; k < 4; ++k) {
                const int li = s_lut[(four >> (8 * k)) & 0xFFu];
#pragma unroll
                for (int v = 0; v < P; ++v) acc[k][v] += (li == v) ? w : 0.0f;
            }
        };
        int m = 0;
        for (; m + U <= sd.n_members; m += U) {
            uint32_t four[U];
            float w[U];
#pragma unroll
            for (int u = 0; u < U; ++u) {
                const int mi = sd.member_off + m + u;
                const char *row = (a.member_plane[mi] ? a.rows1 : a.rows0) + (size_t)a.member_seq[mi] * a.cap;
                four[u] = *reinterpret_cast<const uint32_t *>(row + t0);
                w[u] = a.member_w[mi];
            }
#pragma unroll
            for (int u = 0; u < U; ++u) add(four[u], w[u]);
        }
        for (; m < sd.n_members; ++m) {
            const int mi = sd.member_off + m;
            const char *row = (a.member_plane[mi] ? a.rows1 : a.rows0) + (size_t)a.member_seq[mi] * a.cap;
            add(*reinterpret_cast<const uint32_t *>(row + t0), a.member_w[mi]);
        }
        if (sd.store_slot >= 0) {
            float *c = a.cache[sd.store_slot] + (size_t)t0 * P;
#pragma unroll
            for (int k = 0; k < 4; ++k)
                if (k < nc) {
#pragma unroll
                    for (int v = 0; v < P; ++v) c[k * P + v] = acc[k][v] / fnum * sd.weight;
                }
        }
    }
    float *dst = a.raw + ((size_t)side * a.stride + t0) * P;
#pragma unroll
    for (int k = 0; k < 4; ++k) {
        if (k >= nc) continue;
#pragma unroll
        for (int v = 0; v < P; ++v) dst[k * P + v] = acc[k][v];
        {
            constexpr int CW = P + 2;
            float pc[CW];
#pragma unroll
            for (int v = 0; v < P; ++v) pc[v] = acc[k][v];
            const float g = acc[k][P - 1];
            if (g > 0) {
                const double frac = ((double)(fnum - g) * 1.0) / (double)sd.num;
                pc[P] = fminf(a.min_gap_open, (float)((double)(a.gap_open * a.scale) * frac));
                pc[P + 1] = fminf(a.min_gap_extend, (float)((double)a.gap_extend * frac));
            } else {
                pc[P] = a.gap_open;
                pc[P + 1] = a.gap_extend;
            }
            float4 *out = reinterpret_cast<float4 *>(a.cols + ((size_t)side * a.stride + t0 + k) * CW);
#pragma unroll
            for (int j = 0; j < CW / 4; ++j) out[j] = make_float4(pc[4 * j], pc[4 * j + 1], pc[4 * j + 2], pc[4 * j + 3]);
        }
        int best = P - 2;
        float bestCount = 0.0f;
#pragma unroll
        for (int v = 0; v < P - 2; ++v)
            if (acc[k][v] > bestCount) { bestCount = acc[k][v]; best = v; }
        const bool gappy = (acc[k][P - 1] / fnum > a.gappy_thr);
        a.colinfo[(size_t)side * a.stride + t0 + k] = (uint8_t)(best | (gappy ? 0x80 : 0));
        kept += (a.remove && gappy) ? 0 : 1;
    }
    }
    {
        int x = kept;
#pragma unroll
        for (int d = 1; d < 64; d <<= 1) x += __shfl_xor(x, d, 64);
        if ((threadIdx.x & 63) == 0) s_kept[threadIdx.x >> 6] = x;
        __syncthreads();
        if (threadIdx.x == 0) a.chunk_cnt[(size_t)side * a.n_chunks + blockIdx.y] = s_kept[0] + s_kept[1] + s_kept[2] + s_kept[3];
    }
}

__device__ inline int block_scan_256(bool flag, int *total, int *s_wave )
{
    const unsigned long long b = __ballot(flag);
    const int lane = threadIdx.x & 63, wave = threadIdx.x >> 6;
    const int before = __popcll(b & ((1ull << lane) - 1ull));
    __syncthreads();
    if (lane == 0) s_wave[wave] = __popcll(b);
    __syncthreads();
    int base = 0, sum = 0;
#pragma unroll
    for (int w = 0; w < 4; ++w) { const int c = s_wave[w]; if (w < wave) base += c; sum += c; }
    *total = sum;
    return base + before;
}

__device__ __forceinline__ int block_scan_int_256(int v, int *total, int *s_wave)
{
    const int lane = threadIdx.x & 63, wave = threadIdx.x >> 6;
    int x = v;
#pragma unroll
    for (int d = 1; d < 64; d <<= 1) {
        const int y = __shfl_up(x, d, 64);
        if (lane >= d) x += y;
    }
    __syncthreads();
    if (lane == 63) s_wave[wave] = x;
    __syncthreads();
    int base = 0, sum = 0;
#pragma unroll
    for (int w = 0; w < 4; ++w) { const int c = s_wave[w]; if (w < wave) base += c; sum += c; }
    *total = sum;
    return base + x - v;
}

template <int NW>
__device__ __forceinline__ int block_scan_int(int v, int *total, int *s_wave )
{
    const int lane = threadIdx.x & 63, wave = threadIdx.x >> 6;
    int x = v;
#pragma unroll
    for (int d = 1; d < 64; d <<= 1) {
        const int y = __shfl_up(x, d, 64);
        if (lane >= d) x += y;
    }
    __syncthreads();
    if (lane == 63) s_wave[wave] = x;
    __syncthreads();
    int base = 0, sum = 0;
#pragma unroll
    for (int w = 0; w < NW; ++w) { const int c = s_wave[w]; if (w < wave) base += c; sum += c; }
    *total = sum;
    return base + x - v;
}

template <int P>
__global__ void __launch_bounds__(256) compact_kernel(LevelArgs a)
{
    constexpr int CW = P + 2;
    __shared__ int s_wave[4];
    __shared__ int s_base;
    const int side = blockIdx.x;
    const SideDesc sd = a.sides[side];
    const int c0 = 1024 * blockIdx.y;
    const int lastChunk = (sd.len > 0) ? (sd.len - 1) / 1024 : 0;
    if ((int)blockIdx.y > lastChunk) return;
    const float fnum = (float)sd.num;
    const double dnum = (double)sd.num;
    int part = 0;
    for (int c = threadIdx.x; c < (int)blockIdx.y; c += 256) part += a.chunk_cnt[(size_t)side * a.n_chunks + c];
    int tot;
    (void)block_scan_int_256(part, &tot, s_wave);
    if (threadIdx.x == 0) s_base = tot;
    __syncthreads();
    const int base = s_base;
    const int t0 = c0 + 4 * threadIdx.x;
    bool keep[4];
    int cnt = 0;
#pragma unroll
    for (int k = 0; k < 4; ++k) {
        const int t = t0 + k;
        keep[k] = t < sd.len && !(a.remove && (a.colinfo[(size_t)side * a.stride + t] & 0x80));
        cnt += keep[k] ? 1 : 0;
    }
    int total;
    int dst = base + block_scan_int_256(cnt, &total, s_wave);
    if ((int)blockIdx.y == lastChunk && threadIdx.x == 0) a.len_out[side] = base + total;
    if (base == c0 && total == min(1024, sd.len - c0)) return;
#pragma unroll
    for (int k = 0; k < 4; ++k) {
        if (!keep[k]) continue;
        const float *src = a.raw + ((size_t)side * a.stride + t0 + k) * P;
        float v[CW];
#pragma unroll
        for (int j = 0; j < P; ++j) v[j] = src[j];
        const float g = v[P - 1];
        if (g > 0) {
            const double frac = ((double)(fnum - g) * 1.0) / dnum;
            v[P] = fminf(a.min_gap_open, (float)((double)(a.gap_open * a.scale) * frac));
            v[P + 1] = fminf(a.min_gap_extend, (float)((double)a.gap_extend * frac));
        } else {
            v[P] = a.gap_open;
            v[P + 1] = a.gap_extend;
        }
        float4 *out = reinterpret_cast<float4 *>(a.cols + ((size_t)side * a.stride + dst) * CW);
#pragma unroll
        for (int j = 0; j < CW / 4; ++j) out[j] = make_float4(v[4 * j], v[4 * j + 1], v[4 * j + 2], v[4 * j + 3]);
        ++dst;
    }
}

struct CommitArgs {
    const int8_t *paths;
    const int32_t *path_len;
    int32_t path_stride;
    int32_t *chunk_base;
    int32_t n_chunks;
    const SideDesc *sides;
    const int32_t *member_seq;
    const uint8_t *member_plane;
    char *rows0, *rows1;
    int64_t cap;
    const int32_t *work;
    float *const *cache;
    const int32_t *merge;
    const float *merge_w;
    const uint8_t *from_dp;
    const int8_t *paths_dp;
    int32_t dp_stride;
};

__device__ __forceinline__ const int8_t *path_row(const CommitArgs &a, int pair)
{
    return (a.from_dp && a.from_dp[pair] == 1) ? a.paths_dp + (size_t)pair * (size_t)a.dp_stride : a.paths + (size_t)pair * (size_t)a.path_stride;
}

__global__ void __launch_bounds__(256) path_scan_kernel(CommitArgs a)
{
    __shared__ int s_wave[4];
    const int pair = blockIdx.x;
    const int n = a.path_len[pair];
    const int8_t *path = path_row(a, pair);
    const bool aligned = ((size_t)path & 15u) == 0;
    const int nch = (n + 255) >> 8;
// ... 152 lines not shown
```

twilight_amd/csrc/twl_align.hip:

```cpp
#include "../../include/twl_align.h"
#include "../../include/twl_level.h"
#include "../../include/twl_place.h"
#include "../../include/twl_merge.h"
#include "level_kernels.hip.h"
#include "restore_kernels.hip.h"
#include "place_kernels.hip.h"
#include "merge_kernels.hip.h"
#include "talco_kernel.hip.h"
#include "talco_nuc.hip.h"
#include "talco_global.hip.h"

#include <hip/hip_runtime.h>
#include <dlfcn.h>

#include <algorithm>
#include <atomic>
#include <chrono>
#include <cmath>
#include <cstdio>
#include <cstring>
#include <memory>
#include <mutex>
#include <numeric>
#include <string>
// ... 386 lines not shown
    const int R = len[0], Q = len[1];
    const size_t pitch = ((size_t)Q + 63) & ~(size_t)63, simFloats = (size_t)(R + Q) * pitch;
    if ((rc = d->h2d_freq.ensure(2 * sl * P * sizeof(float)))) return rc;
    if ((rc = d->h2d_gop.ensure(2 * sl * sizeof(float)))) return rc;
    if ((rc = d->cols.ensure(2 * sl * CW * sizeof(float)))) return rc;
    if ((rc = d->h2d_len.ensure(2 * sizeof(int32_t)))) return rc;
    if ((rc = d->h2d_num.ensure(2 * sizeof(int32_t)))) return rc;
    if ((rc = d->items.ensure(sizeof(int32_t)))) return rc;
    if ((rc = d->sim.ensure(simFloats * sizeof(float)))) return rc;
    if ((rc = d->sim_off.ensure(sizeof(long long)))) return rc;
    if ((rc = d->blk_off.ensure(2 * sizeof(int32_t)))) return rc;
    if ((rc = d->m24.ensure(21 * 24 * sizeof(float)))) return rc;
    std::vector<float> m24(21 * 24, 0.0f);
    const int ms = p->P - 1;
    for (int l = 0; l < ms; ++l) for (int m = 0; m < ms; ++m) m24[(ms == 21 ? 24 : 5) * l + m] = p->matrix[ms * l + m];
    const int32_t item = 0, blk[2] = {0, (int32_t)(((R + Q - 1 + 63) / 64) * ((Q + 63) / 64))};
    const long long off = 0;
    HIP_TRY(hipMemcpyAsync(d->h2d_freq.p, freq, 2 * sl * P * sizeof(float), hipMemcpyHostToDevice, st));
    HIP_TRY(hipMemsetAsync(d->h2d_gop.p, 0, 2 * sl * sizeof(float), st));
    HIP_TRY(hipMemcpyAsync(d->h2d_len.p, len, 2 * sizeof(int32_t), hipMemcpyHostToDevice, st));
    HIP_TRY(hipMemcpyAsync(d->h2d_num.p, num, 2 * sizeof(int32_t), hipMemcpyHostToDevice, st));
    HIP_TRY(hipMemcpyAsync(d->items.p, &item, sizeof item, hipMemcpyHostToDevice, st));
    HIP_TRY(hipMemcpyAsync(d->sim_off.p, &off, sizeof off, hipMemcpyHostToDevice, st));
    HIP_TRY(hipMemcpyAsync(d->blk_off.p, blk, sizeof blk, hipMemcpyHostToDevice, st));
    HIP_TRY(hipMemcpyAsync(d->m24.p, m24.data(), m24.size() * sizeof(float), hipMemcpyHostToDevice, st));
    const size_t n_cols = 2 * sl;
    const int blocks = (int)((n_cols + 255) / 256);
    if (p->P == 22) hipLaunchKernelGGL(twl::pack_kernel<22>, dim3(blocks), dim3(256), 0, st, (const float *)d->h2d_freq.p, (const float *)d->h2d_gop.p, (const float *)d->h2d_gop.p, (float *)d->cols.p, n_cols);
    else hipLaunchKernelGGL(twl::pack_kernel<6>, dim3(blocks), dim3(256), 0, st, (const float *)d->h2d_freq.p, (const float *)d->h2d_gop.p, (const float *)d->h2d_gop.p, (float *)d->cols.p, n_cols);
    twl::ScoreArgs sa{};
    sa.cols = (const float *)d->cols.p; sa.len = (const int32_t *)d->h2d_len.p; sa.num = (const int32_t *)d->h2d_num.p;
    sa.items = (const int32_t *)d->items.p; sa.blk_off = (const int32_t *)d->blk_off.p; sa.n_items = 1; sa.seq_len = seq_len;
    sa.gap_char = p->gap_char; sa.M24 = (const float *)d->m24.p; sa.sim = (float *)d->sim.p; sa.sim_off = (const long long *)d->sim_off.p;
    if (p->P == 22) hipLaunchKernelGGL(twl::score_matrix_kernel<22>, dim3((unsigned)blk[1]), dim3(256), 0, st, sa);
    else hipLaunchKernelGGL(twl::score_matrix_kernel<6>, dim3((unsigned)blk[1]), dim3(256), 0, st, sa);
    HIP_TRY(hipGetLastError());
    std::vector<float> diag(simFloats);
    HIP_TRY(hipMemcpyAsync(diag.data(), d->sim.p, simFloats * sizeof(float), hipMemcpyDeviceToHost, st));
    HIP_TRY(hipStreamSynchronize(st));
    for (int i = 0; i < Q; ++i)
        for (int j = 0; j < R; ++j) out[(size_t)i * R + j] = diag[(size_t)(i + j) * pitch + i];
    return TWL_OK;
}

int twl_dp_column_scores(const twl_params *p, int32_t seq_len, const float *freq, const float *gap_open, const float *gap_extend,
                         const int32_t *len, const int32_t *num, float *out)
{
    if (!g_init) { g_err = "twl_init not called"; return TWL_ERR_NOT_INITIALIZED; }
    int rc = check_params(p);
    if (rc) return rc;
    if (seq_len < 1 || !freq || !gap_open || !gap_extend || !len || !num || !out || len[0] < 1 || len[1] < 1 || len[0] > seq_len || len[1] > seq_len) { g_err = "bad argument"; return TWL_ERR_BAD_ARGUMENT; }
    Device *d = g_devs[0];
    const size_t cells = (size_t)len[0] * (size_t)len[1];
    {
        std::lock_guard<std::mutex> lk(d->mu);
        HIP_TRY(hipSetDevice(d->id));
        if ((rc = d->simdump.ensure(cells * sizeof(float)))) return rc;
        HIP_TRY(hipMemset(d->simdump.p, 0xff, cells * sizeof(float)));
        d->dump_on = true;
    }
    std::vector<int8_t> aln(2 * (size_t)seq_len);
    int32_t alen = 0;
    int16_t aerr = 0;
    rc = twl_align_batch(p, 1, seq_len, freq, gap_open, gap_extend, len, num, aln.data(), &alen, &aerr);
    std::lock_guard<std::mutex> lk(d->mu);
    d->dump_on = false;
    if (rc) return rc;
    HIP_TRY(hipSetDevice(d->id));
    HIP_TRY(hipMemcpy(out, d->simdump.p, cells * sizeof(float), hipMemcpyDeviceToHost));
    return TWL_OK;
}

int twl_debug_read(int device, long long *out, int32_t n)
{
    Device *d = nullptr;
    if (find_dev(device, &d)) return TWL_ERR_BAD_ARGUMENT;
    const size_t base = d->pair_cells.size() * 16 * sizeof(int32_t);
    if (!d->dbg.p || base + (size_t)n * 8 > d->dbg.cap) return TWL_ERR_BAD_ARGUMENT;
    return hipMemcpy(out, (const char *)d->dbg.p + base, (size_t)n * 8, hipMemcpyDeviceToHost) == hipSuccess ? TWL_OK : TWL_ERR_HIP;
}

void *twl_host_alloc(uint64_t bytes)
{
    void *p = nullptr;
    if (!g_init || bytes == 0) return nullptr;
    if (hipHostMalloc(&p, (size_t)bytes, hipHostMallocDefault) != hipSuccess) { (void)hipGetLastError(); return nullptr; }
    return p;
}

void twl_host_free(void *p)
{
    if (p) (void)hipHostFree(p);
}

int twl_copy_to_device(int device, void *dst_dev, const void *src, uint64_t bytes)
{
    if (!g_init) { g_err = "twl_init not called"; return TWL_ERR_NOT_INITIALIZED; }
    Device *d = nullptr;
    int rc = find_dev(device, &d);
    if (rc) return rc;
    if (bytes == 0) return TWL_OK;
    if (!dst_dev || !src) { g_err = "bad argument"; return TWL_ERR_BAD_ARGUMENT; }
    HIP_TRY(hipSetDevice(d->id));
    HIP_TRY(hipMemcpy(dst_dev, src, (size_t)bytes, hipMemcpyHostToDevice));
    return TWL_OK;
}

int twl_copy_from_device(int device, void *dst, const void *src_dev, uint64_t bytes)
{
    if (!g_init) { g_err = "twl_init not called"; return TWL_ERR_NOT_INITIALIZED; }
    Device *d = nullptr;
    int rc = find_dev(device, &d);
    if (rc) return rc;
    if (bytes == 0) return TWL_OK;
    if (!dst || !src_dev) { g_err = "bad argument"; return TWL_ERR_BAD_ARGUMENT; }
    HIP_TRY(hipSetDevice(d->id));
    HIP_TRY(hipMemcpy(dst, src_dev, (size_t)bytes, hipMemcpyDeviceToHost));
    return TWL_OK;
}

int twl_copy_rows_from_device(int device, void *dst, uint64_t dst_pitch, const void *src_dev, uint64_t src_pitch, uint64_t width, uint64_t rows)
{
    if (!g_init) { g_err = "twl_init not called"; return TWL_ERR_NOT_INITIALIZED; }
    Device *d = nullptr;
    int rc = find_dev(device, &d);
    if (rc) return rc;
    if (width == 0 || rows == 0) return TWL_OK;
    if (!dst || !src_dev || dst_pitch < width || src_pitch < width) { g_err = "bad argument"; return TWL_ERR_BAD_ARGUMENT; }
    HIP_TRY(hipSetDevice(d->id));
    HIP_TRY(hipMemcpy2D(dst, (size_t)dst_pitch, src_dev, (size_t)src_pitch, (size_t)width, (size_t)rows, hipMemcpyDeviceToHost));
    return TWL_OK;
}

int twl_set_knob(int key, int value)
{
    std::lock_guard<std::mutex> lk(g_mu);
    switch (key) {
    case TWL_KNOB_MT_PERTURB: g_mt_perturb = std::max(0, value); return TWL_OK;
    case TWL_KNOB_MT_MAX_PAIRS: g_mt_max_pairs = std::max(0, value); return TWL_OK;
    case TWL_KNOB_MT_MIN_MARKER: g_mt_min_marker = std::max(2, value); return TWL_OK;
    case TWL_KNOB_MT_LEAD: g_mt_lead = std::max(16, value); return TWL_OK;
    case TWL_KNOB_MT_MARGIN: if (value < 0) { g_mt_marg = 40; g_mt_marg_lat = 64; } else g_mt_marg = g_mt_marg_lat = std::max(2, value); return TWL_OK;
    case TWL_KNOB_MT_ROUNDS: g_mt_rounds = std::max(1, std::min(7, value)); return TWL_OK;
    case TWL_KNOB_MT_THR_JOBS: g_mt_thr_jobs = std::max(0, value); return TWL_OK;
    case TWL_KNOB_FAIL_ROW_ALLOCS: g_fail_next_row_allocs = std::max(0, value); return TWL_OK;
    case TWL_KNOB_PROT_MODE: if (value < 0 || value > 6) { g_err = "protein mode 0..6"; return TWL_ERR_BAD_ARGUMENT; } g_prot_mode = value; return TWL_OK;
    case TWL_KNOB_ASSUME_ONEHOT_QUERY: g_assume_onehot_query = value ? 1 : 0; return TWL_OK;
    case TWL_KNOB_MT_TAIL_PCT: g_mt_tail_pct = std::max(0, std::min(100, value)); return TWL_OK;
    case TWL_KNOB_MT_WIDE: g_mt_wide = value ? 1 : 0; return TWL_OK;
    case TWL_KNOB_NO_SPEC: g_no_spec = value ? 1 : 0; return TWL_OK;
    case TWL_KNOB_FORCE_GLOBAL: g_force_global = value ? 1 : 0; return TWL_OK;
    case TWL_KNOB_LEAF_STEP: g_leaf_step = value ? 1 : 0; return TWL_OK;
    case TWL_KNOB_POISON_TB: g_poison_tb = value ? 1 : 0; return TWL_OK;
    case TWL_KNOB_MT_ANCHOR: g_mt_anchor = value ? 1 : 0; return TWL_OK;
    case TWL_KNOB_MT_LEAD2: if (value < 0) { g_mt_lead2 = 96; g_mt_lead2_lat = 128; } else g_mt_lead2 = g_mt_lead2_lat = std::max(16, value); return TWL_OK;
    case TWL_KNOB_PROT_CORRIDOR: g_prot_corridor = std::max(0, value); for (auto *d : g_devs) d->mem.forget_corridor(); return TWL_OK;
    case TWL_KNOB_SCOUT_XDROP_PCT: g_scout_xdrop_pct = std::max(10, std::min(100, value)); return TWL_OK;
    case TWL_KNOB_THR_SMALL: g_thr_small = std::max(0, std::min(2, value)); for (auto *d : g_devs) d->mem.forget_small(); return TWL_OK;
    default: g_err = "unknown knob"; return TWL_ERR_BAD_ARGUMENT;
    }
}

#include "twl_comm.inc.hip"

int twl_plan_describe(const twl_params *p, int32_t n_pairs, const int32_t *len, int32_t num_cu, int32_t qry_onehot, int32_t wide_streak, char *out, int32_t cap)
{
    if (!p || (p->P != 6 && p->P != 22) || n_pairs < 0 || (n_pairs > 0 && !len) || num_cu < 1 || !out || cap < 64) { g_err = "bad argument (nucleotide or protein parameters, a buffer of 64+ bytes)"; return TWL_ERR_BAD_ARGUMENT; }
    const PassMemory mem = memory_from_code(wide_streak);
    std::vector<int32_t> order;
    for (int32_t n = 0; n < n_pairs; ++n) if (len[2 * n] > 0 && len[2 * n + 1] > 0) order.push_back(n);
    std::stable_sort(order.begin(), order.end(), [&](int32_t x, int32_t y) { return (int64_t)len[2 * x] + len[2 * x + 1] > (int64_t)len[2 * y] + len[2 * y + 1]; });
    const int ms = p->P - 1;
    std::vector<float> M(p->matrix, p->matrix + ms * ms);
    if (p->P == 22) {
        ProtFacts pf;
        pf.n_run = (int)order.size(); pf.n_pairs = n_pairs; pf.num_cu = num_cu; pf.marker = p->marker; pf.M = M.data(); pf.gap_char = p->gap_char;
        pf.corridor_lost = mem.corridor_lost; pf.h_len = len; pf.order = order.data();
        const ProtPlan pl = plan_protein(pf, current_knobs());
        const int w = snprintf(out, (size_t)cap, "%s; mode %d; window %d", prot_first_name(pl.first), pl.mm, prot_first_window(pl.first));
        if (pl.presim && w > 0 && w < cap) snprintf(out + w, (size_t)(cap - w), "; %zu scores precomputed, corridor %d", pl.simFloats, pl.corridor);
        return TWL_OK;
    }
    NucFacts nf;
    nf.n_run = (int)order.size(); nf.num_cu = num_cu; nf.marker = p->marker; nf.M = M.data(); nf.gap_char = p->gap_char; nf.qry_onehot = qry_onehot != 0;
    nf.remember(mem); nf.h_len = len; nf.order = order.data();
    const NucPlan pl = plan_nucleotide(nf, current_knobs());
    snprintf(out, (size_t)cap, "%s; mode %d; window %d%s; bulk %d tail %d", nuc_first_name(pl.first), pl.mm5 ? 5 : pl.mm,
             pl.first == NucFirst::WideMt ? 3072 : ((pl.first == NucFirst::Throughput && pl.small) ? 512 : ((pl.first == NucFirst::Throughput && pl.four) ? 768 : 1024)), pl.probe ? " or 768 (a sample of the level decides)" : "", pl.bulk, pl.tail);
    return TWL_OK;
}

int twl_get_pair_cells(int device, uint64_t *cells_out, int32_t n)
{
    if (!g_init) { g_err = "twl_init not called"; return TWL_ERR_NOT_INITIALIZED; }
    Device *d = nullptr;
    int rc = find_dev(device, &d);
    if (rc) return rc;
    if (!cells_out || n < 0 || (size_t)n > d->pair_cells.size()) { g_err = "bad argument"; return TWL_ERR_BAD_ARGUMENT; }
    for (int32_t i = 0; i < n; ++i) cells_out[i] = d->pair_cells[i];
    return TWL_OK;
}

}

#include "twl_level_plan.inc.hip"
#include "twl_store.inc.hip"
#include "twl_level.inc.hip"
#include "twl_place.inc.hip"
#include "twl_merge.inc.hip"
```

twilight_amd/csrc/twl_knobs.inc.hip:

```cpp

int g_prot_corridor = 448;
int g_mt_perturb = 0;
int g_mt_lead = 320, g_mt_marg = 40;
int g_mt_marg_lat = 64, g_mt_lead2_lat = 128;
int g_mt_anchor = 1, g_mt_lead2 = 96;
int g_mt_max_pairs = 1024, g_mt_min_marker = 512, g_mt_rounds = 2, g_mt_thr_jobs = 256;
int g_scout_xdrop_pct = 100;
int g_no_spec = 0;
int g_thr_small = 0;
int g_mt_wide = 1;
int g_mt_tail_pct = 70;
int g_prot_mode = 0;
int g_force_global = 0;
int g_assume_onehot_query = 0;
int g_leaf_step = 1;
int g_poison_tb = 0;
```

twilight_amd/csrc/twl_level.inc.hip:

```cpp

namespace {

static_assert(sizeof(SideRow) == sizeof(twl::SideDesc) && offsetof(SideRow, weight) == offsetof(twl::SideDesc, weight) &&
              offsetof(SideRow, cache_slot) == offsetof(twl::SideDesc, cache_slot) && offsetof(SideRow, store_slot) == offsetof(twl::SideDesc, store_slot),
              "SideRow (twl_level_plan.inc.hip) is uploaded as twl::SideDesc");


int register_stored(twl_store *s, const PreparePlan &pp)
{
    std::vector<CacheEntry> fresh(pp.newIds.size());
    for (size_t k = 0; k < fresh.size(); ++k) {
        const int rc = fresh[k].take(s->d, pp.newLens[k], std::max<size_t>((size_t)pp.newLens[k] * (size_t)s->P * sizeof(float), 16));
        if (rc) return rc;
    }
    for (size_t k = 0; k < fresh.size(); ++k) s->cache[pp.newIds[k]] = std::move(fresh[k]);
    return TWL_OK;
}

int upload_prepare(twl_store *s, hipStream_t st, const PreparePlan &pp, const float *member_weight)
{
    LevelBufs *lv = s->lv;
    std::vector<float *> tab(pp.slotIds.size());
    for (size_t k = 0; k < tab.size(); ++k) tab[k] = (float *)s->cache.find(pp.slotIds[k])->second.buf.p;
    const size_t ns = pp.dsides.size();
    Arena &A = lv->up_prepare;
    int rc = A.begin(ns * (sizeof(SideRow) + sizeof(int32_t)) + pp.nm * (sizeof(int32_t) + sizeof(float) + 1) + tab.size() * sizeof(float *), 6);
    if (rc) return rc;
    A.put(lv->d_sides, pp.dsides);
    A.put(lv->d_mseq, s->members);
    A.put(lv->d_mw, member_weight, pp.nm);
    A.put(lv->d_mplane, pp.mplane);
    A.put(lv->d_tab, tab);
    A.put(lv->d_num, s->h_num);
    return A.flush(st);
}

int size_prepare(LevelBufs *lv, size_t ns, size_t sl, size_t P, size_t chunks)
{
    int rc;
    if ((rc = lv->d_raw.ensure(ns * sl * P * sizeof(float)))) return rc;
    if ((rc = lv->d_colinfo.ensure(ns * sl))) return rc;
    if ((rc = lv->d_cols.ensure(ns * sl * (P + 2) * sizeof(float)))) return rc;
    if ((rc = lv->d_len.ensure(ns * sizeof(int32_t)))) return rc;
    return lv->d_ccnt.ensure(ns * chunks * sizeof(int32_t));
}

twl::LevelArgs prepare_args(const twl_store *s, const twl_params *p, float gappy_threshold, int32_t chunks)
{
    const LevelBufs *lv = s->lv;
    twl::LevelArgs a{};
    a.sides = lv->d_sides.as<const twl::SideDesc>();
    a.member_seq = lv->d_mseq.as<const int32_t>();
    a.member_w = lv->d_mw.as<const float>();
    a.member_plane = lv->d_mplane.as<const uint8_t>();
    a.rows0 = (const char *)s->rows[0].p; a.rows1 = (const char *)s->rows[1].p;
    a.cap = s->cap;
    a.cache = lv->d_tab.as<float *const>();
    a.lut = (const uint8_t *)s->lut.p;
    a.raw = (float *)lv->d_raw.p;
    a.colinfo = (uint8_t *)lv->d_colinfo.p;
    a.cols = (float *)lv->d_cols.p;
    a.len_out = (int32_t *)lv->d_len.p;
    a.stride = s->seq_len;
    a.gappy_thr = gappy_threshold;
    a.remove = (gappy_threshold == 1.0) ? 0 : 1;
    a.gap_open = p->gap_open; a.gap_extend = p->gap_extend;
    a.scale = (s->type == 'n') ? 0.5f : 1.0f;
    a.min_gap_extend = p->gap_extend * 0.2;
    a.min_gap_open = p->gap_open * 0.1;
    a.chunk_cnt = (int32_t *)lv->d_ccnt.p;
    a.n_chunks = chunks;
    return a;
}

int launch_prepare(const twl_store *s, hipStream_t st, const twl::LevelArgs &a, dim3 grid)
{
    if (s->P == 6) {
        hipLaunchKernelGGL(twl::profile_kernel<6>, grid, dim3(256), 0, st, a);
        hipLaunchKernelGGL(twl::compact_kernel<6>, grid, dim3(256), 0, st, a);
    } else {
        hipLaunchKernelGGL(twl::profile_kernel<22>, grid, dim3(256), 0, st, a);
        hipLaunchKernelGGL(twl::compact_kernel<22>, grid, dim3(256), 0, st, a);
    }
    HIP_TRY(hipGetLastError());
    return TWL_OK;
}

int read_back_prepare(twl_store *s, hipStream_t st, size_t ns, int32_t *len_out, uint8_t *colinfo_out)
{
    LevelBufs *lv = s->lv;
    s->h_len.resize(ns);
    int rc;
    if ((rc = lv->back.ensure(ns * sizeof(int32_t)))) return rc;
    HIP_TRY(hipMemcpyAsync(lv->back.p, lv->d_len.p, ns * sizeof(int32_t), hipMemcpyDeviceToHost, st));
    if (colinfo_out) HIP_TRY(hipMemcpyAsync(colinfo_out, lv->d_colinfo.p, ns * (size_t)s->seq_len, hipMemcpyDeviceToHost, st));
    HIP_TRY(hipStreamSynchronize(st));
    memcpy(s->h_len.data(), lv->back.p, ns * sizeof(int32_t));
    for (size_t i = 0; i < ns; ++i) len_out[i] = s->h_len[i];
    return TWL_OK;
}


int upload_align(LevelBufs *lv, hipStream_t st, const std::vector<int32_t> &lm)
{
    Arena &A = lv->up_align;
    int rc = A.begin(lm.size() * sizeof(int32_t), 1);
    if (rc) return rc;
    A.put(lv->d_lenmask, lm);
    return A.flush(st);
}

int size_align(LevelBufs *lv, size_t n, size_t sl)
{
    int rc;
    if ((rc = lv->d_aln.ensure(n * 2 * sl))) return rc;
    if ((rc = lv->d_alnlen.ensure(n * sizeof(int32_t)))) return rc;
    return lv->d_err.ensure(n * sizeof(int16_t));
}

int read_back_align(twl_store *s, Device *d, hipStream_t st, int8_t *aln_out, int32_t *aln_len_out, int16_t *err_out)
{
    const int32_t n = s->n_pairs;
    const size_t sl = (size_t)s->seq_len;
    LevelBufs *lv = s->lv;
    if ((int32_t)d->last_err.size() == n && (int32_t)d->last_alnlen.size() == n) {
        std::copy(d->last_err.begin(), d->last_err.end(), err_out);
        std::copy(d->last_alnlen.begin(), d->last_alnlen.end(), aln_len_out);
        if (!aln_out) { d->stats.total_ms = d->stats.kernel_ms; return TWL_OK; }
    } else {
        HIP_TRY(hipMemcpyAsync(aln_len_out, lv->d_alnlen.p, (size_t)n * sizeof(int32_t), hipMemcpyDeviceToHost, st));
        HIP_TRY(hipMemcpyAsync(err_out, lv->d_err.p, (size_t)n * sizeof(int16_t), hipMemcpyDeviceToHost, st));
        HIP_TRY(hipStreamSynchronize(st));
    }
    int32_t ran = 0;
    for (int32_t i = 0; i < n; ++i) ran += aln_len_out[i] > 0;
    if (!aln_out) {}
    else if (ran * 2 >= n) HIP_TRY(hipMemcpyAsync(aln_out, lv->d_aln.p, (size_t)n * 2 * sl, hipMemcpyDeviceToHost, st));
    else
        for (int32_t i = 0; i < n; ++i)
            if (aln_len_out[i] > 0)
                HIP_TRY(hipMemcpyAsync(aln_out + (size_t)i * 2 * sl, (int8_t *)lv->d_aln.p + (size_t)i * 2 * sl, (size_t)aln_len_out[i], hipMemcpyDeviceToHost, st));
    HIP_TRY(hipEventRecord(d->ev[3], st));
    HIP_TRY(hipStreamSynchronize(st));
    float ms = 0.f;
    HIP_TRY(hipEventElapsedTime(&ms, d->ev[5], d->ev[3]));
    d->stats.total_ms = ms;
    return TWL_OK;
}


int size_restore(LevelBufs *lv, size_t ns, size_t n, size_t sl, unsigned nWch, unsigned nb, bool &soft)
{
    const size_t bstride = 2 * sl + 1;
    const struct { Buf *b; size_t bytes; bool soft; } want[] = {
        {&lv->r_oidx, 2 * ns * (sl + 1) * sizeof(int32_t), true},
        {&lv->r_run, ns * 4 * bstride * sizeof(int32_t), true},
        {&lv->r_seg, ns * bstride * sizeof(int32_t), true},
        {&lv->r_aoff, ns * bstride * sizeof(int32_t), true},
        {&lv->r_blist, ns * bstride * sizeof(int32_t), true},
        {&lv->r_nboth, ns * sizeof(int32_t), false},
        {&lv->r_wtot, ns * nWch * sizeof(int32_t), true},
        {&lv->r_arena, ns * 2 * sl, true},
        {&lv->r_outlen, n * sizeof(int32_t), false},
        {&lv->r_tb, ns * nb * twl::kNwThreads * (size_t)twl::kNwCells, true},
        {&lv->r_rows, ns * nb * twl::kNwThreads * 6 * (size_t)twl::kNwRow * sizeof(float), true},
    };
    for (const auto &w : want)
        if (const int rc = w.b->ensure(w.bytes)) { soft = w.soft; return rc; }
    return TWL_OK;
}

twl::RestoreArgs restore_args(const twl_store *s, const twl_params *p, int32_t n_sel, int32_t out_stride, unsigned nWch)
{
    const LevelBufs *lv = s->lv;
    const size_t sl = (size_t)s->seq_len;
    twl::RestoreArgs a{};
    a.aln = (const int8_t *)lv->d_aln.p; a.aln_len = (const int32_t *)lv->d_alnlen.p; a.aln_stride = (int32_t)(2 * sl);
    a.colinfo = (const uint8_t *)lv->d_colinfo.p; a.stride = s->seq_len;
    a.sides = lv->d_sides.as<const twl::SideDesc>(); a.len_red = (const int32_t *)lv->d_len.p;
    a.sel = lv->r_sel.as<const int32_t>(); a.n_sel = n_sel;
    a.orig_idx = (int32_t *)lv->r_oidx.p; a.run = (int32_t *)lv->r_run.p; a.seg = (int32_t *)lv->r_seg.p; a.aoff = (int32_t *)lv->r_aoff.p;
    a.both_list = (int32_t *)lv->r_blist.p; a.n_both = (int32_t *)lv->r_nboth.p;
    a.wtot = (int32_t *)lv->r_wtot.p; a.n_wchunks = (int32_t)nWch;
    a.arena = (int8_t *)lv->r_arena.p; a.arena_stride = (int32_t)(2 * sl); a.bstride = (int32_t)(2 * sl + 1);
    a.out = (int8_t *)lv->d_paths.p; a.out_stride = out_stride; a.out_len = (int32_t *)lv->r_outlen.p;
    a.tbs = (int8_t *)lv->r_tb.p; a.rows = (float *)lv->r_rows.p;
    a.ms = p->P - 1;
    for (int t = 0; t < a.ms * a.ms; ++t) a.M[t] = p->matrix[t];
    a.gap_open = p->gap_open; a.gap_extend = p->gap_extend;
    return a;
}

int restore_batch(twl_store *s, const twl_params *p, int32_t n_sel, const int32_t *pairs, int32_t out_stride, int32_t *final_len_out)
{
    int rc;
    const int32_t n = s->n_pairs;
    hipStream_t st = s->d->stream;
    LevelBufs *lv = s->lv;
    const size_t bstride = 2 * (size_t)s->seq_len + 1;
    {
        Arena &A = lv->up_restore;
        if ((rc = A.begin((size_t)n_sel * sizeof(int32_t), 1))) return rc;
        A.put(lv->r_sel, pairs, (size_t)n_sel);
        if ((rc = A.flush(st))) return rc;
    }
    const unsigned nWch = (unsigned)((bstride + (size_t)twl::kRsThreads * twl::kWrItems - 1) / ((size_t)twl::kRsThreads * twl::kWrItems));
    const unsigned nb = (unsigned)std::max(1, std::min(128, 4096 / n_sel));
    bool soft = false;
    if ((rc = size_restore(lv, (size_t)n_sel, (size_t)n, (size_t)s->seq_len, nWch, nb, soft))) {
        if (!soft) return rc;
        (void)hipGetLastError();
        for (int32_t t = 0; t < n_sel; ++t) final_len_out[t] = -1;
        return TWL_OK;
    }
    const twl::RestoreArgs a = restore_args(s, p, n_sel, out_stride, nWch);
    hipLaunchKernelGGL(twl::restore_index_kernel, dim3(2 * (unsigned)n_sel), dim3(twl::kRsThreads), 0, st, a);
    hipLaunchKernelGGL(twl::restore_runs_kernel, dim3((unsigned)n_sel), dim3(twl::kRsThreads), 0, st, a);
    hipLaunchKernelGGL(twl::restore_align_kernel, dim3((unsigned)n_sel, nb), dim3(twl::kNwThreads), 0, st, a);
    hipLaunchKernelGGL(twl::restore_count_kernel, dim3((unsigned)n_sel, nWch), dim3(twl::kRsThreads), 0, st, a);
    hipLaunchKernelGGL(twl::restore_write_kernel, dim3((unsigned)n_sel, nWch), dim3(twl::kRsThreads), 0, st, a);
    HIP_TRY(hipGetLastError());
    if ((rc = lv->back.ensure((size_t)n * sizeof(int32_t)))) return rc;
    HIP_TRY(hipMemcpyAsync(lv->back.p, lv->r_outlen.p, (size_t)n * sizeof(int32_t), hipMemcpyDeviceToHost, st));
    HIP_TRY(hipStreamSynchronize(st));
    const int32_t *all = (const int32_t *)lv->back.p;
    for (int32_t t = 0; t < n_sel; ++t) final_len_out[t] = all[pairs[t]];
    return TWL_OK;
}


int take_merged(twl_store *s, const int32_t *path_len, std::vector<CacheEntry> &merged)
{
    const CommitPlan &cp = s->commit;
    merged.resize(cp.nMerge());
    for (size_t k = 0; k < merged.size(); ++k) {
        const int32_t len = path_len[cp.merge[4 * k]];
        const int rc = merged[k].take(s->d, len, (size_t)len * (size_t)s->P * sizeof(float));
        if (rc) return rc;
    }
    return TWL_OK;
}

int stage_paths(twl_store *s, hipStream_t st, const int8_t *paths, const int32_t *path_len, int32_t path_stride, const uint8_t *from_dp)
{
    const size_t n = (size_t)s->n_pairs, ps = (size_t)path_stride;
    int rc;
    if ((rc = s->lv->d_paths.ensure(n * ps))) return rc;
    if (!from_dp) HIP_TRY(hipMemcpyAsync(s->lv->d_paths.p, paths, n * ps, hipMemcpyHostToDevice, st));
    else
        for (size_t i = 0; i < n; ++i)
            if (!from_dp[i] && path_len[i] > 0)
                HIP_TRY(hipMemcpyAsync((int8_t *)s->lv->d_paths.p + i * ps, paths + i * ps, (size_t)path_len[i], hipMemcpyHostToDevice, st));
    return s->lv->d_chunk.ensure(n * (size_t)s->commit.nChunks * 2 * sizeof(int32_t));
}

int upload_commit(twl_store *s, hipStream_t st, const std::vector<CacheEntry> &merged, const int32_t *path_len, const uint8_t *from_dp)
{
    const CommitPlan &cp = s->commit;
    LevelBufs *lv = s->lv;
    const size_t n = (size_t)s->n_pairs;
    std::vector<float *> &tab = s->h_tab;
    tab.clear();
    for (size_t k = 0; k < merged.size(); ++k)
        for (float *p : {(float *)s->cache.find(cp.mergeIds[2 * k])->second.buf.p, (float *)s->cache.find(cp.mergeIds[2 * k + 1])->second.buf.p, (float *)merged[k].buf.p})
            tab.push_back(p);
    Arena &A = lv->up_commit;
    int rc = A.begin((n + cp.work.size() + cp.merge.size()) * sizeof(int32_t) + cp.mergew.size() * sizeof(float) + tab.size() * sizeof(float *) + cp.mplane.size() + (from_dp ? n : 0), 7);
    if (rc) return rc;
    A.put(lv->d_pathlen, path_len, n);
    A.put(lv->d_work, cp.work);
    A.put(lv->d_merge, cp.merge);
    A.put(lv->d_mergew, cp.mergew);
    A.put(lv->d_tab, tab);
    A.put(lv->d_mplane, cp.mplane);
    if (from_dp) A.put(lv->d_fromdp, from_dp, n);
    return A.flush(st);
}

twl::CommitArgs commit_args(const twl_store *s, int32_t path_stride, bool fromDp)
{
    const LevelBufs *lv = s->lv;
    twl::CommitArgs a{};
    a.paths = (const int8_t *)lv->d_paths.p;
    if (fromDp) { a.from_dp = lv->d_fromdp.as<const uint8_t>(); a.paths_dp = (const int8_t *)lv->d_aln.p; a.dp_stride = (int32_t)(2 * (size_t)s->seq_len); }
    a.path_len = lv->d_pathlen.as<const int32_t>();
    a.path_stride = path_stride;
    a.chunk_base = (int32_t *)lv->d_chunk.p;
    a.n_chunks = s->commit.nChunks;
    a.sides = lv->d_sides.as<const twl::SideDesc>();
    a.member_seq = lv->d_mseq.as<const int32_t>();
    a.member_plane = lv->d_mplane.as<const uint8_t>();
    a.rows0 = (char *)s->rows[0].p; a.rows1 = (char *)s->rows[1].p;
    a.cap = s->cap;
    a.work = lv->d_work.as<const int32_t>();
    a.cache = lv->d_tab.as<float *const>();
    a.merge = lv->d_merge.as<const int32_t>();
    a.merge_w = lv->d_mergew.as<const float>();
    return a;
}

int rewrite_rows(twl_store *s, Device *d, hipStream_t st, const twl::CommitArgs &a)
{
    const CommitPlan &cp = s->commit;
    const dim3 grid(cp.nWork(), (unsigned)((cp.nChunks + 3) / 4));
    s->commit_side = false;
    if (!cp.nWork()) return TWL_OK;
    if (!cp.side) {
        const int rc = wait_rows(s, st);
        if (rc) return rc;
        hipLaunchKernelGGL(twl::apply_path_kernel, grid, dim3(256), 0, st, a);
        return TWL_OK;
    }
    LevelBufs *lv = s->lv;
    if (!lv->ev_scan) { HIP_TRY(hipEventCreateWithFlags(&lv->ev_scan, hipEventDisableTiming)); HIP_TRY(hipEventCreateWithFlags(&lv->ev_apply, hipEventDisableTiming)); }
    HIP_TRY(hipEventRecord(lv->ev_scan, st));
    HIP_TRY(hipStreamWaitEvent(d->stream2, lv->ev_scan, 0));
    HIP_TRY(hipEventRecord(d->ev2[0], d->stream2));
    hipLaunchKernelGGL(twl::apply_path_kernel, grid, dim3(256), 0, d->stream2, a);
    HIP_TRY(hipEventRecord(d->ev2[1], d->stream2));
    HIP_TRY(hipEventRecord(lv->ev_apply, d->stream2));
    lv->apply_pending = true;
    s->rows_event = lv->ev_apply;
    s->commit_side = true;
    return TWL_OK;
}

void apply_commit(twl_store *s, std::vector<CacheEntry> &merged)
{
    const CommitPlan &cp = s->commit;
    for (size_t k = 0; k < cp.flips.size(); k += 2) { s->plane[cp.flips[k]] ^= 1; s->len[cp.flips[k]] = cp.flips[k + 1]; }
    for (size_t k = 0; k < merged.size(); ++k) {
        s->cache[cp.mergeIds[2 * k]] = std::move(merged[k]);
        s->cache.erase(cp.mergeIds[2 * k + 1]);
    }
}

int level_rows_block(twl_store *s, bool toBlock, int32_t n_sel, const int32_t *pairs, const int32_t *lens, const uint8_t *where, void *blk_dev, const int64_t *blk_off)
{
    if (!s || !s->prepared || !s->lv || !s->staged_stride || n_sel < 0 || (n_sel > 0 && (!pairs || !lens || !blk_dev || !blk_off))) { g_err = "bad argument (twl_level_restore first)"; return TWL_ERR_BAD_ARGUMENT; }
    if (n_sel == 0) return TWL_OK;
    DEVICE_CALL(call, s->d);
    hipStream_t st = call.st;
    LevelBufs *lv = s->lv;
    const size_t sl2 = 2 * (size_t)s->seq_len, ps = (size_t)s->staged_stride;
    for (int which = 1; which <= 2; ++which) {
        std::vector<int64_t> ro, bo;
        std::vector<int32_t> ln;
        for (int32_t t = 0; t < n_sel; ++t) {
            const int w = where ? where[t] : 2;
            if (w != which || lens[t] <= 0) continue;
            if (pairs[t] < 0 || pairs[t] >= s->n_pairs || (size_t)lens[t] > (which == 1 ? sl2 : ps) || (which == 1 && !toBlock)) { g_err = "bad row selection"; return TWL_ERR_BAD_ARGUMENT; }
            ro.push_back((int64_t)pairs[t] * (int64_t)(which == 1 ? sl2 : ps)); bo.push_back(blk_off[t]); ln.push_back(lens[t]);
        }
        if (ro.empty()) continue;
        int rc;
        Ref rowoff, blkoff, len;
        Arena &A = lv->up_paths;
        if ((rc = A.begin(ro.size() * (2 * sizeof(int64_t) + sizeof(int32_t)), 3))) return rc;
        A.put(rowoff, ro);
        A.put(blkoff, bo);
        A.put(len, ln);
        if ((rc = A.flush(st))) return rc;
        int8_t *base = (int8_t *)(which == 1 ? lv->d_aln.p : lv->d_paths.p);
        if (toBlock) hipLaunchKernelGGL(twl::rows_to_block_kernel, dim3((unsigned)ro.size()), dim3(256), 0, st, (const int8_t *)base, rowoff.as<const int64_t>(), len.as<const int32_t>(), (int8_t *)blk_dev, blkoff.as<const int64_t>());
        else hipLaunchKernelGGL(twl::block_to_rows_kernel, dim3((unsigned)ro.size()), dim3(256), 0, st, base, rowoff.as<const int64_t>(), len.as<const int32_t>(), (const int8_t *)blk_dev, blkoff.as<const int64_t>());
        HIP_TRY(hipGetLastError());
        HIP_TRY(hipStreamSynchronize(st));
    }
    return TWL_OK;
}

}

extern "C" {

int twl_level_prepare(twl_store *s, const twl_params *p, float gappy_threshold, int32_t n_pairs, const twl_side *sides, const int32_t *members,
                      const float *member_weight, int32_t seq_len, int32_t *len_out, uint8_t *colinfo_out)
{
    if (!s) { g_err = "store is null"; return TWL_ERR_BAD_ARGUMENT; }
    int rc = check_params(p);
    if (rc) return rc;
    if (p->P != s->P) { g_err = "params.P does not match the store's sequence type"; return TWL_ERR_BAD_ARGUMENT; }
    if (n_pairs < 0 || seq_len < 1 || (n_pairs > 0 && (!sides || !len_out))) { g_err = "bad argument"; return TWL_ERR_BAD_ARGUMENT; }
    s->prepared = false;
    s->n_pairs = n_pairs;
    s->seq_len = seq_len;
    if (n_pairs == 0) { s->prepared = true; return TWL_OK; }
    DEVICE_CALL(call, s->d);
    Device *d = call.d;
    hipStream_t st = call.st;
    if (!s->lv) s->lv = acquire_level(d);
    const char *why = check_sides(n_pairs, sides, seq_len, members, member_weight, s->n_seqs, s->len.data(), [&](int32_t id) {
        const auto it = s->cache.find(id);
        return it == s->cache.end() ? -1 : it->second.len;
    });
    if (why) { g_err = why; return TWL_ERR_BAD_ARGUMENT; }
    PreparePlan pp = plan_prepare(n_pairs, sides, members, s->plane.data());
    const size_t ns = (size_t)n_pairs * 2;
    s->sides.assign(sides, sides + ns);
    s->members.assign(members, members + pp.nm);
    s->h_num.swap(pp.h_num);
    if ((rc = register_stored(s, pp))) return rc;
    if (pp.readsRows && (rc = wait_rows(s, st))) return rc;
    HIP_TRY(hipEventRecord(d->ev[0], st));
    if ((rc = upload_prepare(s, st, pp, member_weight))) return rc;
    const dim3 grid((unsigned)ns, (unsigned)((pp.maxLen + 1023) / 1024));
    if ((rc = size_prepare(s->lv, ns, (size_t)seq_len, (size_t)s->P, grid.y))) return rc;
    if ((rc = launch_prepare(s, st, prepare_args(s, p, gappy_threshold, (int32_t)grid.y), grid))) return rc;
    HIP_TRY(hipEventRecord(d->ev[1], st));
    if ((rc = read_back_prepare(s, st, ns, len_out, colinfo_out))) return rc;
    float ms = 0.f;
    HIP_TRY(hipEventElapsedTime(&ms, d->ev[0], d->ev[1]));
    s->prepare_ms = ms;
    s->prepared = true;
    return TWL_OK;
}

int twl_level_read_colinfo(twl_store *s, int32_t pair, int32_t side, uint8_t *out)
{
    if (!s || !s->prepared || !out || pair >= s->n_pairs || side < 0 || side > 1) { g_err = "bad argument"; return TWL_ERR_BAD_ARGUMENT; }
    DEVICE_CALL(call, s->d);
    if (pair < 0) {
        HIP_TRY(hipMemcpy(out, s->lv->d_colinfo.p, (size_t)s->n_pairs * 2 * (size_t)s->seq_len, hipMemcpyDeviceToHost));
        return TWL_OK;
    }
    const size_t idx = (size_t)pair * 2 + (size_t)side;
    const size_t len = (size_t)std::max(0, s->sides[idx].len);
    if (len) HIP_TRY(hipMemcpy(out, (const uint8_t *)s->lv->d_colinfo.p + idx * (size_t)s->seq_len, len, hipMemcpyDeviceToHost));
    return TWL_OK;
}

int twl_level_align(twl_store *s, const twl_params *p, const uint8_t *run_mask, int8_t *aln_out, int32_t *aln_len_out, int16_t *err_out)
{
    return twl_level_align_mixed(s, p, run_mask, nullptr, aln_out, aln_len_out, err_out);
}

int twl_level_align_mixed(twl_store *s, const twl_params *p, const uint8_t *run_mask, const uint8_t *zero_gap, int8_t *aln_out, int32_t *aln_len_out, int16_t *err_out)
{
    if (!s || !s->prepared) { g_err = "twl_level_prepare has not been called"; return TWL_ERR_BAD_ARGUMENT; }
    int rc = check_params(p);
    if (rc) return rc;
    if (p->P != s->P) { g_err = "params.P does not match the store's sequence type"; return TWL_ERR_BAD_ARGUMENT; }
    const int32_t n = s->n_pairs;
    if (n == 0) return TWL_OK;
    if (!aln_len_out || !err_out) { g_err = "bad argument"; return TWL_ERR_BAD_ARGUMENT; }
    DEVICE_CALL(call, s->d);
    Device *d = call.d;
    hipStream_t st = call.st;
    LevelBufs *lv = s->lv;
    const AlignPlan ap = plan_align(n, s->h_len, s->sides.data(), run_mask, g_leaf_step);
    if ((rc = upload_align(lv, st, ap.lm))) return rc;
    if ((rc = size_align(lv, (size_t)n, (size_t)s->seq_len))) return rc;
    HIP_TRY(hipEventRecord(d->ev[5], st));
    rc = run_device(d, st, p, n, s->seq_len, nullptr, nullptr, nullptr, lv->d_lenmask.as<const int32_t>(), lv->d_num.as<const int32_t>(), (int8_t *)lv->d_aln.p,
                    (int32_t *)lv->d_alnlen.p, (int16_t *)lv->d_err.p, ap.lm.data(), (const float *)lv->d_cols.p, ap.qryOneHot, zero_gap, ap.shape);
    if (rc) return rc;
    return read_back_align(s, d, st, aln_out, aln_len_out, err_out);
}

int twl_level_read_path(twl_store *s, int32_t pair, int8_t *out, int32_t len)
{
    if (!s || !s->prepared || !out || pair < 0 || pair >= s->n_pairs || len < 0 || len > 2 * s->seq_len || !s->lv || !s->lv->d_aln.p) { g_err = "bad argument"; return TWL_ERR_BAD_ARGUMENT; }
    DEVICE_CALL(call, s->d);
    if (len) HIP_TRY(hipMemcpy(out, (const int8_t *)s->lv->d_aln.p + (size_t)pair * 2 * (size_t)s->seq_len, (size_t)len, hipMemcpyDeviceToHost));
    return TWL_OK;
}

int twl_level_read_colinfo_many(twl_store *s, int32_t n_sel, const int32_t *pairs, uint8_t *out)
{
    if (!s || !s->prepared || n_sel < 0 || (n_sel > 0 && (!pairs || !out || !s->lv))) { g_err = "bad argument"; return TWL_ERR_BAD_ARGUMENT; }
    DEVICE_CALL(call, s->d);
    const size_t sl = (size_t)s->seq_len;
    for (int32_t t = 0; t < n_sel; ++t) {
        if (pairs[t] < 0 || pairs[t] >= s->n_pairs) { g_err = "pair index out of range"; return TWL_ERR_BAD_ARGUMENT; }
        HIP_TRY(hipMemcpyAsync(out + (size_t)t * 2 * sl, (const uint8_t *)s->lv->d_colinfo.p + (size_t)pairs[t] * 2 * sl, 2 * sl, hipMemcpyDeviceToHost, call.st));
    }
    HIP_TRY(hipStreamSynchronize(call.st));
    return TWL_OK;
}

int twl_level_read_paths(twl_store *s, int32_t n_sel, const int32_t *pairs, const int32_t *lens, int8_t *out, int32_t out_stride)
{
    if (!s || !s->prepared || n_sel < 0 || (n_sel > 0 && (!pairs || !lens || !out || !s->lv || !s->lv->d_aln.p)) || out_stride < 0) { g_err = "bad argument"; return TWL_ERR_BAD_ARGUMENT; }
    DEVICE_CALL(call, s->d);
    const size_t sl = (size_t)s->seq_len;
    for (int32_t t = 0; t < n_sel; ++t) {
        if (pairs[t] < 0 || pairs[t] >= s->n_pairs || lens[t] < 0 || lens[t] > out_stride || (size_t)lens[t] > 2 * sl) { g_err = "bad selection"; return TWL_ERR_BAD_ARGUMENT; }
        if (lens[t]) HIP_TRY(hipMemcpyAsync(out + (size_t)t * (size_t)out_stride, (const int8_t *)s->lv->d_aln.p + (size_t)pairs[t] * 2 * sl, (size_t)lens[t], hipMemcpyDeviceToHost, call.st));
    }
    HIP_TRY(hipStreamSynchronize(call.st));
    return TWL_OK;
}

int twl_level_restore(twl_store *s, const twl_params *p, int32_t n_sel, const int32_t *pairs, int32_t out_stride, int32_t *final_len_out)
{
    if (!s || !s->prepared || !s->lv || (n_sel > 0 && !s->lv->d_aln.p)) { g_err = "twl_level_align has not been called"; return TWL_ERR_BAD_ARGUMENT; }
    int rc = check_params(p);
    if (rc) return rc;
    const int32_t n = s->n_pairs;
    if (n_sel < 0 || (n_sel > 0 && (!pairs || !final_len_out)) || out_stride < 1) { g_err = "bad argument"; return TWL_ERR_BAD_ARGUMENT; }
    for (int32_t t = 0; t < n_sel; ++t) if (pairs[t] < 0 || pairs[t] >= n) { g_err = "pair index out of range"; return TWL_ERR_BAD_ARGUMENT; }
    DEVICE_CALL(call, s->d);
    if (s->staged_stride && s->staged_stride != out_stride) { g_err = "twl_level_restore: one row pitch per level"; return TWL_ERR_BAD_ARGUMENT; }
    if ((rc = s->lv->d_paths.ensure((size_t)n * (size_t)out_stride))) return rc;
    s->staged_stride = out_stride;
    constexpr int32_t kBatch = 4096;
    for (int32_t at = 0; at < n_sel; at += kBatch)
        if ((rc = restore_batch(s, p, std::min(kBatch, n_sel - at), pairs + at, out_stride, final_len_out + at))) return rc;
    return TWL_OK;
}

int twl_level_exchange_buffers(twl_store *s, int64_t send_bytes, int64_t recv_bytes, void **send_dev, void **recv_dev)
{
    if (!s || !s->prepared || !s->lv || send_bytes < 0 || recv_bytes < 0 || !send_dev || !recv_dev) { g_err = "bad argument"; return TWL_ERR_BAD_ARGUMENT; }
    DEVICE_CALL(call, s->d);
    int rc;
    if ((rc = s->lv->x_send.ensure(std::max<size_t>((size_t)send_bytes, 64)))) return rc;
    if ((rc = s->lv->x_recv.ensure(std::max<size_t>((size_t)recv_bytes, 64)))) return rc;
    *send_dev = s->lv->x_send.p; *recv_dev = s->lv->x_recv.p;
    return TWL_OK;
}

int twl_level_paths_to_block(twl_store *s, int32_t n_sel, const int32_t *pairs, const int32_t *lens, const uint8_t *where, void *blk_dev, const int64_t *blk_off)
{
    return level_rows_block(s, true, n_sel, pairs, lens, where, blk_dev, blk_off);
}

int twl_level_paths_from_block(twl_store *s, int32_t n_sel, const int32_t *pairs, const int32_t *lens, const void *blk_dev, const int64_t *blk_off)
{
    return level_rows_block(s, false, n_sel, pairs, lens, nullptr, const_cast<void *>(blk_dev), blk_off);
}

int twl_level_write_final(twl_store *s, int32_t pair, const int8_t *path, int32_t len)
{
    if (!s || !s->prepared || !s->lv || !s->staged_stride || pair < 0 || pair >= s->n_pairs || len < 0 || len > s->staged_stride || (len > 0 && !path)) { g_err = "bad argument (twl_level_restore first)"; return TWL_ERR_BAD_ARGUMENT; }
    DEVICE_CALL(call, s->d);
    if (len) HIP_TRY(hipMemcpy((int8_t *)s->lv->d_paths.p + (size_t)pair * (size_t)s->staged_stride, path, (size_t)len, hipMemcpyHostToDevice));
    return TWL_OK;
}

int twl_level_read_final(twl_store *s, int32_t pair, int8_t *out, int32_t len)
{
    if (!s || !s->prepared || !out || pair < 0 || pair >= s->n_pairs || len < 0 || !s->lv || !s->staged_stride || len > s->staged_stride) { g_err = "bad argument (twl_level_restore first)"; return TWL_ERR_BAD_ARGUMENT; }
    DEVICE_CALL(call, s->d);
    if (len) HIP_TRY(hipMemcpy(out, (const int8_t *)s->lv->d_paths.p + (size_t)pair * (size_t)s->staged_stride, (size_t)len, hipMemcpyDeviceToHost));
    return TWL_OK;
}

int twl_level_commit(twl_store *s, const int8_t *paths, const int32_t *path_len, int32_t path_stride)
{
    return twl_level_commit_from_dp(s, paths, path_len, path_stride, nullptr);
}

int twl_level_commit_from_dp(twl_store *s, const int8_t *paths, const int32_t *path_len, int32_t path_stride, const uint8_t *from_dp)
{
    if (!s || !s->prepared) { g_err = "twl_level_prepare has not been called"; return TWL_ERR_BAD_ARGUMENT; }
    const int32_t n = s->n_pairs;
    if (const char *why = check_commit(n, s->seq_len, s->staged_stride, s->lv && s->lv->d_aln.p, paths != nullptr, path_len, path_stride, from_dp)) { g_err = why; return TWL_ERR_BAD_ARGUMENT; }
    DEVICE_CALL(call, s->d);
    Device *d = call.d;
    hipStream_t st = call.st;
    s->prepared = false;
    s->staged_stride = 0;
    struct GiveBack { twl_store *s; ~GiveBack() { release_level(s->lv); } } giveBack{s};
    if (n == 0 || max_path(n, path_len) == 0) return TWL_OK;
    CommitPlan &cp = s->commit;
    plan_commit(cp, n, s->sides.data(), s->members, s->plane.data(), path_len, from_dp);
// ... 52 lines not shown
```

twilight_amd/csrc/twl_level_plan.inc.hip:

```cpp
#include <algorithm>
#include <cstdint>
#include <unordered_map>
#include <vector>
#include "../../include/twl_level.h"

struct SideRow { int32_t n_members, member_off, len, num; float weight; int32_t cache_slot, store_slot, pad; };

template <class CacheLen>
const char *check_sides(int32_t n_pairs, const twl_side *sides, int32_t seq_len, const int32_t *members, const float *member_weight, int32_t n_seqs,
                        const int32_t *row_len, CacheLen cacheLen)
{
    const size_t ns = (size_t)n_pairs * 2;
    size_t nm = 0;
    for (size_t i = 0; i < ns; ++i) {
        const twl_side &sd = sides[i];
        if (sd.n_members < 0 || sd.member_off < 0 || sd.len < 0 || sd.len > seq_len || sd.num < 1) return "bad side descriptor";
        nm = std::max(nm, (size_t)sd.member_off + (size_t)sd.n_members);
    }
    if (nm > 0 && (!members || !member_weight)) return "member tables missing";
    std::unordered_map<int32_t, int32_t> stored;
    for (size_t i = 0; i < ns; ++i) {
        const twl_side &sd = sides[i];
        for (int32_t m = 0; m < sd.n_members; ++m) {
            const int32_t q = members[sd.member_off + m];
            if (q < 0 || q >= n_seqs) return "member sequence id out of range";
            if (row_len[q] != sd.len) return "member row length differs from the side's len";
        }
        if (sd.cache_id >= 0) {
            const auto it = stored.find(sd.cache_id);
            if ((it != stored.end() ? it->second : cacheLen(sd.cache_id)) != sd.len) return "cache id unknown or of another length";
        } else if (sd.store_id >= 0) {
            if (stored.count(sd.store_id) || cacheLen(sd.store_id) >= 0) return "store_id already in use";
            stored[sd.store_id] = sd.len;
        }
    }
    return nullptr;
}

struct PreparePlan {
    size_t nm = 0;
    std::vector<SideRow> dsides;
    std::vector<int32_t> slotIds;
    std::vector<int32_t> newIds, newLens;
    std::vector<uint8_t> mplane;
    std::vector<int32_t> h_num;
    bool readsRows = false;
    int32_t maxLen = 1;
};

inline PreparePlan plan_prepare(int32_t n_pairs, const twl_side *sides, const int32_t *members, const uint8_t *plane)
{
    PreparePlan pp;
    const size_t ns = (size_t)n_pairs * 2;
    for (size_t i = 0; i < ns; ++i) pp.nm = std::max(pp.nm, (size_t)sides[i].member_off + (size_t)sides[i].n_members);
    pp.mplane.assign(pp.nm, 0);
    pp.dsides.resize(ns);
    pp.h_num.resize(ns);
    std::unordered_map<int32_t, int32_t> slotOf;
    auto slot = [&](int32_t id) {
        const auto it = slotOf.find(id);
        if (it != slotOf.end()) return it->second;
        pp.slotIds.push_back(id);
        return slotOf[id] = (int32_t)pp.slotIds.size() - 1;
    };
    for (size_t i = 0; i < ns; ++i) {
        const twl_side &sd = sides[i];
        for (int32_t m = 0; m < sd.n_members; ++m) pp.mplane[sd.member_off + m] = plane[members[sd.member_off + m]];
        SideRow &ds = pp.dsides[i];
        ds.n_members = sd.n_members; ds.member_off = sd.member_off; ds.len = sd.len; ds.num = sd.num; ds.weight = sd.weight;
        ds.cache_slot = ds.store_slot = -1; ds.pad = 0;
        if (sd.cache_id >= 0) ds.cache_slot = slot(sd.cache_id);
        else if (sd.store_id >= 0) { pp.newIds.push_back(sd.store_id); pp.newLens.push_back(sd.len); ds.store_slot = slot(sd.store_id); }
        pp.h_num[i] = sd.num;
        pp.readsRows = pp.readsRows || (sd.cache_id < 0 && sd.n_members > 0);
        pp.maxLen = std::max(pp.maxLen, sd.len);
    }
    return pp;
}

struct AlignPlan {
    std::vector<int32_t> lm;
    bool qryOneHot = true;
    int shape = 0;
};

inline AlignPlan plan_align(int32_t n, const std::vector<int32_t> &h_len, const twl_side *sides, const uint8_t *run_mask, int leaf_step)
{
    AlignPlan ap;
    ap.lm = h_len;
    if (run_mask)
        for (int32_t i = 0; i < n; ++i) if (!run_mask[i]) ap.lm[2 * i] = ap.lm[2 * i + 1] = 0;
    auto runs = [&](int32_t i) { return ap.lm[2 * i] > 0 && ap.lm[2 * i + 1] > 0; };
    for (int32_t i = 0; i < n && ap.qryOneHot; ++i)
        if (runs(i)) ap.qryOneHot = sides[2 * (size_t)i + 1].n_members == 1 && sides[2 * (size_t)i + 1].cache_id < 0;
    if (leaf_step) {
        bool leaf = true, any = false;
        for (int32_t i = 0; i < n && leaf; ++i) {
            if (!runs(i)) continue;
            any = true;
            for (int side = 0; side < 2; ++side) {
                const twl_side &sd = sides[2 * (size_t)i + side];
                leaf = leaf && sd.n_members == 1 && sd.cache_id < 0 && sd.num == 1;
            }
        }
        ap.shape = (any && leaf) ? 2 : 0;
    }
    return ap;
}

inline const char *check_commit(int32_t n, int32_t seq_len, int32_t staged, bool haveDp, bool havePaths, const int32_t *path_len, int32_t path_stride,
                                const uint8_t *from_dp)
{
    if (n > 0 && ((!havePaths && !from_dp) || !path_len || path_stride < 1)) return "bad argument";
    if (staged && (!from_dp || staged != path_stride)) return "commit after twl_level_restore: from_dp and the restore's row pitch are required";
    if (from_dp && !staged) for (int32_t i = 0; i < n; ++i) if (from_dp[i] == 2) return "from_dp == 2 without twl_level_restore";
    if (from_dp) {
        for (int32_t i = 0; i < n; ++i) {
            if (from_dp[i] == 1 && (!haveDp || path_len[i] > 2 * seq_len)) return "from_dp without a DP output of this level";
            if (!from_dp[i] && path_len[i] > 0 && !havePaths) return "bad argument";
        }
    }
    for (int32_t i = 0; i < n; ++i) if (path_len[i] < 0 || path_len[i] > path_stride) return "path_len outside [0, path_stride]";
    return nullptr;
}

constexpr int kRowGroup = 64;

struct CommitPlan {
    int32_t maxPath = 0, nChunks = 0;
    std::vector<int32_t> work;
    std::vector<int32_t> merge;
    std::vector<float> mergew;
    std::vector<int32_t> mergeIds;
    std::vector<uint8_t> mplane;
    std::vector<int32_t> flips;
    bool hostRows = false;
    bool side = false;
    unsigned nWork() const { return (unsigned)(work.size() / 3); }
    unsigned nMerge() const { return (unsigned)(merge.size() / 4); }
};

inline int32_t max_path(int32_t n, const int32_t *path_len)
{
    int32_t m = 0;
    for (int32_t i = 0; i < n; ++i) m = std::max(m, path_len[i]);
    return m;
}

inline void plan_commit(CommitPlan &cp, int32_t n, const twl_side *sides, const std::vector<int32_t> &members, const uint8_t *plane, const int32_t *path_len,
                        const uint8_t *from_dp)
{
    cp.work.clear(); cp.merge.clear(); cp.mergew.clear(); cp.mergeIds.clear(); cp.flips.clear();
    cp.maxPath = max_path(n, path_len);
    cp.nChunks = (cp.maxPath + 255) / 256;
    cp.hostRows = !from_dp;
    for (int32_t i = 0; i < n; ++i) {
        if (path_len[i] == 0) continue;
        if (from_dp && !from_dp[i]) cp.hostRows = true;
        for (int sd = 0; sd < 2; ++sd) {
            const twl_side &x = sides[2 * (size_t)i + sd];
            for (int32_t m = 0; m < x.n_members; m += kRowGroup) { cp.work.push_back(2 * i + sd); cp.work.push_back(m); cp.work.push_back(std::min(kRowGroup, x.n_members - m)); }
            for (int32_t m = 0; m < x.n_members; ++m) { cp.flips.push_back(members[x.member_off + m]); cp.flips.push_back(path_len[i]); }
        }
        const twl_side &r = sides[2 * (size_t)i], &q = sides[2 * (size_t)i + 1];
        const int32_t rid = r.cache_id >= 0 ? r.cache_id : r.store_id, qid = q.cache_id >= 0 ? q.cache_id : q.store_id;
        if (rid >= 0 && qid >= 0) {
            const int32_t at = 3 * (int32_t)cp.nMerge();
            cp.merge.insert(cp.merge.end(), {i, at, at + 1, at + 2});
            cp.mergew.push_back(r.weight); cp.mergew.push_back(q.weight);
            cp.mergeIds.push_back(rid); cp.mergeIds.push_back(qid);
        }
    }
    cp.mplane.resize(members.size());
    for (size_t k = 0; k < members.size(); ++k) cp.mplane[k] = plane[members[k]];
    cp.side = cp.nWork() > 0 && n <= 32 && !cp.hostRows;
}
```

twilight_amd/csrc/twl_store.inc.hip:

```cpp
#include <cstdlib>
#include "twl_path_source.inc.hip"

namespace {

struct DeviceCall {
    Device *d;
    hipStream_t st;
    std::lock_guard<std::mutex> lk;
    int rc;
    explicit DeviceCall(Device *dev) : d(dev), st(dev->stream), lk(dev->mu), rc(make_current()) {}
    int make_current() { HIP_TRY(hipSetDevice(d->id)); return TWL_OK; }
};
#define DEVICE_CALL(name, dev) DeviceCall name(dev); if (name.rc) return name.rc

}

struct Ref {
    void *p = nullptr;
    template <class T> T *as() const { return static_cast<T *>(p); }
};
struct PinBuf {
    void *p = nullptr;
    size_t cap = 0;
    int ensure(size_t bytes)
    {
        if (bytes <= cap) return TWL_OK;
        if (p) (void)hipHostFree(p);
        p = nullptr; cap = 0;
        HIP_TRY(hipHostMalloc(&p, bytes + bytes / 2 + 256, hipHostMallocDefault));
        cap = bytes + bytes / 2 + 256;
        return TWL_OK;
    }
    void release() { if (p) (void)hipHostFree(p); p = nullptr; cap = 0; }
};
struct Arena {
    char *h = nullptr;
    size_t hcap = 0, used = 0;
    Buf d;
    int begin(size_t bytes, size_t tables)
    {
        const size_t want = bytes + 256 * (tables + 1);
        if (want > hcap) {
            if (h) (void)hipHostFree(h);
            h = nullptr; hcap = 0;
            const size_t cap = want + want / 2;
            HIP_TRY(hipHostMalloc((void **)&h, cap, hipHostMallocDefault));
            hcap = cap;
        }
        used = 0;
        return d.ensure(hcap);
    }
    template <class T>
    void put(Ref &r, const T *src, size_t n)
    {
        used = (used + 255) & ~(size_t)255;
        if (n) memcpy(h + used, src, n * sizeof(T));
        r.p = (char *)d.p + used;
        used += std::max<size_t>(n * sizeof(T), 16);
    }
    template <class T> void put(Ref &r, const std::vector<T> &v) { put(r, v.data(), v.size()); }
    int flush(hipStream_t st)
    {
        if (used) HIP_TRY(hipMemcpyAsync(d.p, h, used, hipMemcpyHostToDevice, st));
        return TWL_OK;
    }
    void release() { if (h) (void)hipHostFree(h); h = nullptr; hcap = 0; d.release(); }
};

struct LevelBufs {
    Arena up_prepare, up_align, up_restore, up_commit;
    Arena up_paths;
    PinBuf back;
    Ref d_sides, d_mseq, d_mw, d_mplane, d_tab, d_num;
    Ref d_lenmask;
    Ref r_sel;
    Ref d_pathlen, d_work, d_merge, d_mergew, d_fromdp;
    Buf d_raw, d_colinfo, d_cols, d_len, d_aln, d_alnlen, d_err;
    Buf d_paths, d_chunk, d_ccnt;
    Buf r_oidx, r_run, r_seg, r_aoff, r_blist, r_nboth, r_wtot, r_arena, r_outlen, r_tb, r_rows;
    Buf x_send, x_recv;
    bool busy = false;
    hipEvent_t ev_scan = nullptr, ev_apply = nullptr;
    bool apply_pending = false;
    void release_all()
    {
        if (ev_scan) (void)hipEventDestroy(ev_scan);
        if (ev_apply) (void)hipEventDestroy(ev_apply);
        ev_scan = ev_apply = nullptr; apply_pending = false;
        for (Buf *b : {&d_raw, &d_colinfo, &d_cols, &d_len, &d_aln, &d_alnlen, &d_err,
                       &d_paths, &d_chunk, &d_ccnt, &r_oidx, &r_run, &r_seg, &r_aoff, &r_blist, &r_nboth, &r_wtot, &r_arena, &r_outlen, &r_tb, &r_rows, &x_send, &x_recv})
            b->release();
        for (Arena *a : {&up_prepare, &up_align, &up_restore, &up_commit, &up_paths}) a->release();
        back.release();
    }
};

namespace {
std::vector<std::unique_ptr<LevelBufs>> &level_pool(Device *d)
{
    static std::mutex mu;
    static std::unordered_map<Device *, std::vector<std::unique_ptr<LevelBufs>>> pools;
    std::lock_guard<std::mutex> lk(mu);
    return pools[d];
}
LevelBufs *acquire_level(Device *d)
{
    auto &pool = level_pool(d);
    LevelBufs *waiting = nullptr;
    for (const auto &own : pool) {
        LevelBufs *b = own.get();
        if (b->busy) continue;
        if (b->apply_pending && hipEventQuery(b->ev_apply) != hipSuccess) { (void)hipGetLastError(); if (!waiting) waiting = b; continue; }
        b->apply_pending = false;
        b->busy = true;
        return b;
    }
    if (waiting && pool.size() >= 3) {
        (void)hipStreamWaitEvent(d->stream, waiting->ev_apply, 0);
        waiting->apply_pending = false;
        waiting->busy = true;
        return waiting;
    }
    pool.push_back(std::make_unique<LevelBufs>());
    pool.back()->busy = true;
    return pool.back().get();
}
void release_level(LevelBufs *&lv) { if (lv) { lv->busy = false; lv = nullptr; } }

std::vector<Buf> &cache_pool(Device *d)
{
    static std::mutex mu;
    static std::unordered_map<Device *, std::vector<Buf>> pools;
    std::lock_guard<std::mutex> lk(mu);
    return pools[d];
}
int cache_buf_get(Device *d, Buf &b, size_t bytes)
{
    auto &pool = cache_pool(d);
    size_t best = pool.size();
    for (size_t k = 0; k < pool.size(); ++k)
        if (pool[k].cap >= bytes && (best == pool.size() || pool[k].cap < pool[best].cap)) best = k;
    if (best != pool.size()) { b = pool[best]; pool[best] = pool.back(); pool.pop_back(); return TWL_OK; }
    b = Buf{};
    return b.ensure(bytes + bytes / 4);
}
void cache_buf_put(Device *d, Buf &b)
{
    if (!b.p) return;
    auto &pool = cache_pool(d);
    if (pool.size() >= 4096) {
        size_t small = 0;
        for (size_t k = 1; k < pool.size(); ++k) if (pool[k].cap < pool[small].cap) small = k;
        if (pool[small].cap < b.cap) std::swap(pool[small], b);
        b.release();
        return;
    }
    pool.push_back(b);
    b = Buf{};
}

struct CacheEntry {
    Device *d = nullptr;
    Buf buf;
    int32_t len = 0;
    CacheEntry() = default;
    CacheEntry(CacheEntry &&o) noexcept : d(o.d), buf(o.buf), len(o.len) { o.buf = Buf{}; }
    CacheEntry &operator=(CacheEntry &&o) noexcept
    {
        if (this != &o) { cache_buf_put(d, buf); d = o.d; buf = o.buf; len = o.len; o.buf = Buf{}; }
        return *this;
    }
    ~CacheEntry() { cache_buf_put(d, buf); }
    int take(Device *dev, int32_t n, size_t bytes) { d = dev; len = n; return cache_buf_get(dev, buf, bytes); }
};
}

static void twl_level_pool_release(Device *d)
{
    auto &pool = level_pool(d);
    for (const auto &b : pool) b->release_all();
    pool.clear();
    for (Buf &b : cache_pool(d)) b.release();
    cache_pool(d).clear();
}

struct twl_store {
    Device *d = nullptr;
    int P = 6;
    char type = 'n';
    int32_t n_seqs = 0;
    int64_t cap = 0;
    Buf rows[2];
    std::vector<uint8_t> plane;
    std::vector<int32_t> len;
    std::unordered_map<int32_t, CacheEntry> cache;
    Buf lut;
    int32_t n_pairs = 0, seq_len = 0;
    bool prepared = false;
    std::vector<twl_side> sides;
    std::vector<int32_t> members;
    std::vector<int32_t> h_len, h_num;
    CommitPlan commit;
    std::vector<float *> h_tab;
    bool commit_pending = false;
    bool commit_side = false;
    hipEvent_t rows_event = nullptr;
    LevelBufs *lv = nullptr;
    int32_t staged_stride = 0;
    Arena up_rows;
    Buf d_gather;
    Buf x_send, x_recv;
    double prepare_ms = 0, commit_ms = 0;
};

namespace {

void build_lut(char type, uint8_t *lut)
{
    for (int c = 0; c < 256; ++c) {
        const int u = (c >= 'a' && c <= 'z') ? c - 32 : c;
        int v;
        if (type == 'n') {
            switch (u) {
            case 'A': v = 0; break;
            case 'C': v = 1; break;
            case 'G': v = 2; break;
            case 'T': case 'U': v = 3; break;
            case '-': case '.': v = 5; break;
            default: v = 4; break;
            }
        } else {
            static const char acids[] = "ACDEFGHIKLMNPQRSTVWY";
            v = 20;
            for (int k = 0; k < 20; ++k) if (u == acids[k]) v = k;
            if (u == '-' || u == '.') v = 21;
        }
        lut[c] = (uint8_t)v;
    }
}

int64_t rows_budget_cap(twl_store *s)
{
    size_t freeB = 0, totalB = 0;
    if (hipMemGetInfo(&freeB, &totalB) != hipSuccess) { (void)hipGetLastError(); return INT64_MAX; }
    const int64_t budget = (int64_t)(totalB / 6);
    return std::max<int64_t>(256, budget / (2 * std::max<int64_t>(1, s->n_seqs)));
}

int g_fail_next_row_allocs = 0;

int grow_rows(twl_store *s, int64_t need, int64_t want = 0)
{
    if (need <= s->cap) return TWL_OK;
    Device *d = s->d;
    HIP_TRY(hipStreamSynchronize(d->stream2));
    s->rows_event = nullptr;
    const int64_t minCap = (need + 255) & ~(int64_t)255;
    int64_t ncap = std::max(need, std::min(std::max(want, need + need / 2), rows_budget_cap(s)));
    ncap = (ncap + 255) & ~(int64_t)255;
    Buf nb[2];
    auto alloc_both = [&](int64_t cap) {
        for (int pl = 0; pl < 2; ++pl) {
            int rc = TWL_ERR_HIP;
            if (g_fail_next_row_allocs > 0) { --g_fail_next_row_allocs; g_err = "row allocation failed (test knob)"; }
            else rc = nb[pl].ensure((size_t)s->n_seqs * (size_t)cap);
            if (rc) { nb[0].release(); nb[1].release(); (void)hipGetLastError(); return rc; }
        }
        return (int)TWL_OK;
    };
    int rc = alloc_both(ncap);
    if (rc && ncap > minCap) { ncap = minCap; rc = alloc_both(ncap); }
    if (rc) return rc;
    for (int pl = 0; pl < 2; ++pl)
        if (s->rows[pl].p)
            HIP_TRY(hipMemcpy2DAsync(nb[pl].p, (size_t)ncap, s->rows[pl].p, (size_t)s->cap, (size_t)s->cap, (size_t)s->n_seqs, hipMemcpyDeviceToDevice, d->stream));
    HIP_TRY(hipStreamSynchronize(d->stream));
    for (int pl = 0; pl < 2; ++pl) { s->rows[pl].release(); s->rows[pl] = nb[pl]; }
    s->cap = ncap;
    return TWL_OK;
}

struct StoreEnd {
    void operator()(twl_store *raw) const
    {
        std::unique_ptr<twl_store> s(raw);
        (void)hipSetDevice(s->d->id);
        (void)hipStreamSynchronize(s->d->stream);
        (void)hipStreamSynchronize(s->d->stream2);
        s->cache.clear();
        release_level(s->lv);
        for (Buf *b : {&s->rows[0], &s->rows[1], &s->lut, &s->d_gather, &s->x_send, &s->x_recv}) b->release();
        s->up_rows.release();
        s->d->live_stores -= 1;
    }
};

int wait_rows(twl_store *s, hipStream_t st)
{
    if (s->rows_event) { HIP_TRY(hipStreamWaitEvent(st, s->rows_event, 0)); s->rows_event = nullptr; }
    return TWL_OK;
}

template <class Args>
void fill_row_planes(const twl_store *s, Args &a)
{
    a.rows0 = (const char *)s->rows[0].p; a.rows1 = (const char *)s->rows[1].p;
    a.out0 = (char *)s->rows[0].p; a.out1 = (char *)s->rows[1].p;
    a.cap = s->cap;
}
void rows_rewritten(twl_store *s, const std::vector<int32_t> &ids, int32_t W) { for (int32_t id : ids) { s->plane[id] ^= 1; s->len[id] = W; } }

PathLevelView path_level_view(const twl_store *s)
{
    const bool prepared = s->prepared && s->lv;
    return PathLevelView{prepared, s->n_pairs, 2 * (int64_t)s->seq_len, prepared && s->lv->d_aln.p, s->staged_stride};
}
int upload_host_paths(Buf &buf, const int8_t *paths, const int32_t *path_len, int32_t path_stride, const std::vector<int32_t> &hostRows, hipStream_t st)
{
    const size_t pitch = (size_t)path_stride;
    if (!hostRows.empty()) { const int rc = buf.ensure(hostRows.size() * pitch); if (rc) return rc; }
    for (size_t k = 0; k < hostRows.size(); ++k)
        HIP_TRY(hipMemcpyAsync((int8_t *)buf.p + k * pitch, paths + (size_t)hostRows[k] * pitch, (size_t)path_len[hostRows[k]], hipMemcpyHostToDevice, st));
    return TWL_OK;
}
twl::PathSrc path_src(const twl_store *s, const uint8_t *from_dp, const Buf &hostRows, const Ref &which, const Ref &srcOff, const Ref &plen)
{
    return twl::PathSrc{{(const int8_t *)hostRows.p, from_dp ? (const int8_t *)s->lv->d_aln.p : nullptr, from_dp ? (const int8_t *)s->lv->d_paths.p : nullptr},
                        which.as<const uint8_t>(), srcOff.as<const int64_t>(), plen.as<const int32_t>()};
}

struct RowTables { std::vector<int64_t> off; int64_t total = 0; int32_t maxLen = 1; };
RowTables row_offsets(int32_t n, const int32_t *lens)
{
    RowTables t;
    t.off.resize((size_t)n);
    for (int32_t k = 0; k < n; ++k) { t.off[k] = t.total; t.total += lens[k]; t.maxLen = std::max(t.maxLen, lens[k]); }
    return t;
}

struct RowRefs { Ref plane, ids, len, off; };
int upload_row_tables(twl_store *s, hipStream_t st, int32_t n, const int32_t *ids, const int32_t *lens, const int64_t *off, RowRefs &r)
{
    Arena &A = s->up_rows;
    int rc = A.begin(s->plane.size() + (size_t)n * ((ids ? sizeof(int32_t) : 0) + (lens ? sizeof(int32_t) : 0) + (off ? sizeof(int64_t) : 0)), 4);
    if (rc) return rc;
    A.put(r.plane, s->plane);
    if (ids) A.put(r.ids, ids, (size_t)n);
    if (lens) A.put(r.len, lens, (size_t)n);
    if (off) A.put(r.off, off, (size_t)n);
    return A.flush(st);
}

struct RowMove {
    bool write = false;
    int32_t n = 0;
    const int32_t *ids = nullptr;
    const int32_t *lens = nullptr;
    char *host = nullptr;
    void *block = nullptr;
};

int move_rows(twl_store *s, hipStream_t st, const RowMove &m, const RowTables &t)
{
    int rc;
    if ((rc = wait_rows(s, st))) return rc;
    if (m.write && (rc = grow_rows(s, (int64_t)t.maxLen + 1))) return rc;
    char *packed = (char *)m.block;
    if (!packed) {
        if ((rc = s->d_gather.ensure((size_t)std::max<int64_t>(t.total, 16)))) return rc;
        packed = (char *)s->d_gather.p;
    }
    RowRefs r;
    if ((rc = upload_row_tables(s, st, m.n, m.ids, m.lens, t.off.data(), r))) return rc;
    if (m.write && m.host && t.total) HIP_TRY(hipMemcpyAsync(packed, m.host, (size_t)t.total, hipMemcpyHostToDevice, st));
    const dim3 grid((unsigned)m.n, (unsigned)((t.maxLen + 255) / 256));
    if (m.write)
        hipLaunchKernelGGL(twl::scatter_rows_of_kernel, grid, dim3(256), 0, st, (char *)s->rows[0].p, (char *)s->rows[1].p, s->cap, r.plane.as<const uint8_t>(),
                           r.ids.as<const int32_t>(), r.len.as<const int32_t>(), r.off.as<const int64_t>(), (const char *)packed);
    else if (m.ids)
        hipLaunchKernelGGL(twl::gather_rows_of_kernel, grid, dim3(256), 0, st, (const char *)s->rows[0].p, (const char *)s->rows[1].p, s->cap, r.plane.as<const uint8_t>(),
                           r.ids.as<const int32_t>(), r.len.as<const int32_t>(), r.off.as<const int64_t>(), packed);
    else
        hipLaunchKernelGGL(twl::gather_rows_kernel, grid, dim3(256), 0, st, (const char *)s->rows[0].p, (const char *)s->rows[1].p, s->cap, r.plane.as<const uint8_t>(),
                           r.len.as<const int32_t>(), r.off.as<const int64_t>(), packed);
    HIP_TRY(hipGetLastError());
    if (!m.write && m.host && t.total) HIP_TRY(hipMemcpyAsync(m.host, packed, (size_t)t.total, hipMemcpyDeviceToHost, st));
    HIP_TRY(hipStreamSynchronize(st));
    if (m.write) for (int32_t k = 0; k < m.n; ++k) s->len[m.ids[k]] = m.lens[k];
    return TWL_OK;
}

using HostBytes = std::unique_ptr<char, decltype(&std::free)>;
HostBytes host_bytes(size_t n) { return HostBytes((char *)std::malloc(std::max<size_t>(n, 1)), &std::free); }

bool rows_in_range(const twl_store *s, int32_t n_ids, const int32_t *ids, const int32_t *lens)
{
    for (int32_t t = 0; t < n_ids; ++t) if (ids[t] < 0 || ids[t] >= s->n_seqs || (lens && lens[t] < 0)) return false;
    return true;
}

}

extern "C" {

int twl_store_create(int device, char type, int32_t n_seqs, const char *const *seqs, const int32_t *lens, twl_store **out)
{
    if (!g_init) { g_err = "twl_init not called"; return TWL_ERR_NOT_INITIALIZED; }
    if (!out || n_seqs < 0 || (n_seqs > 0 && (!seqs || !lens)) || (type != 'n' && type != 'p')) { g_err = "bad argument"; return TWL_ERR_BAD_ARGUMENT; }
    Device *d = nullptr;
    int rc = find_dev(device, &d);
    if (rc) return rc;
    DEVICE_CALL(call, d);
    std::unique_ptr<twl_store, StoreEnd> s(std::make_unique<twl_store>().release());
    d->live_stores += 1;
    s->d = d;
    s->type = type;
    s->P = (type == 'n') ? 6 : 22;
    s->n_seqs = n_seqs;
    s->plane.assign((size_t)n_seqs, 0);
    s->len.assign(lens, lens + n_seqs);
    int64_t maxLen = 1;
    for (int32_t i = 0; i < n_seqs; ++i) {
        if (lens[i] < 0) { g_err = "negative sequence length"; return TWL_ERR_BAD_ARGUMENT; }
        maxLen = std::max<int64_t>(maxLen, lens[i]);
    }
    const double lg = std::log10((double)std::max<int32_t>(n_seqs, 10));
    const int64_t factor = (int64_t)std::min(48.0, std::max(8.0, 8.0 * lg - 16.0));
    if ((rc = grow_rows(s.get(), maxLen + 1, factor * maxLen + 256))) return rc;
    if (n_seqs > 0) {
        const size_t hp = (size_t)maxLen;
        const HostBytes img = host_bytes((size_t)n_seqs * hp);
        if (!img) { g_err = "out of host memory"; return TWL_ERR_HIP; }
        for (int32_t i = 0; i < n_seqs; ++i) { memcpy(img.get() + (size_t)i * hp, seqs[i], (size_t)lens[i]); memset(img.get() + (size_t)i * hp + (size_t)lens[i], '-', hp - (size_t)lens[i]); }
        HIP_TRY(hipMemcpy2D(s->rows[0].p, (size_t)s->cap, img.get(), hp, hp, (size_t)n_seqs, hipMemcpyHostToDevice));
    }
    uint8_t lut[256];
    build_lut(type, lut);
    if ((rc = s->lut.ensure(256))) return rc;
    HIP_TRY(hipMemcpy(s->lut.p, lut, 256, hipMemcpyHostToDevice));
    *out = s.release();
    return TWL_OK;
}

void twl_store_destroy(twl_store *s)
{
    if (!s) return;
    std::lock_guard<std::mutex> lk(s->d->mu);
    StoreEnd()(s);
}

int twl_store_read_rows(twl_store *s, char *const *rows_out, int32_t *lens_out)
{
    if (!s || !lens_out) { g_err = "bad argument"; return TWL_ERR_BAD_ARGUMENT; }
    for (int32_t i = 0; i < s->n_seqs; ++i) lens_out[i] = s->len[i];
    if (!rows_out || s->n_seqs == 0) return TWL_OK;
    DEVICE_CALL(call, s->d);
    const RowTables t = row_offsets(s->n_seqs, s->len.data());
    RowMove m;
    m.n = s->n_seqs; m.lens = s->len.data();
    bool packed = true;
    for (int32_t i = 0; i < s->n_seqs && packed; ++i) packed = (s->len[i] == 0) || (rows_out[i] == rows_out[0] + (t.off[i] - t.off[0]) && rows_out[0] != nullptr);
    if (packed && s->len[0] > 0) { m.host = rows_out[0]; return move_rows(s, call.st, m, t); }
    const HostBytes host = host_bytes((size_t)t.total);
    if (!host) { g_err = "out of host memory"; return TWL_ERR_HIP; }
    m.host = host.get();
    const int rc = move_rows(s, call.st, m, t);
    if (rc) return rc;
    const int nt = (int)std::min<size_t>(8, std::max<size_t>(1, (size_t)t.total >> 24));
    std::vector<std::thread> th;
    for (int k = 0; k < nt; ++k)
        th.emplace_back([&, k] {
            for (int32_t i = k; i < s->n_seqs; i += nt)
                if (rows_out[i] && s->len[i] > 0) memcpy(rows_out[i], host.get() + t.off[i], (size_t)s->len[i]);
        });
    for (auto &x : th) x.join();
    return TWL_OK;
}

int twl_store_read_rows_of(twl_store *s, int32_t n_ids, const int32_t *ids, char *out, int32_t *lens_out)
{
    if (!s || n_ids < 0 || (n_ids > 0 && (!ids || !lens_out))) { g_err = "bad argument"; return TWL_ERR_BAD_ARGUMENT; }
    if (!rows_in_range(s, n_ids, ids, nullptr)) { g_err = "sequence id out of range"; return TWL_ERR_BAD_ARGUMENT; }
    for (int32_t t = 0; t < n_ids; ++t) lens_out[t] = s->len[ids[t]];
    const RowTables t = row_offsets(n_ids, lens_out);
    if (!out || n_ids == 0 || t.total == 0) return TWL_OK;
    DEVICE_CALL(call, s->d);
    RowMove m;
    m.n = n_ids; m.ids = ids; m.lens = lens_out; m.host = out;
    return move_rows(s, call.st, m, t);
}

int twl_store_write_rows(twl_store *s, int32_t n_ids, const int32_t *ids, const char *in, const int32_t *lens)
{
    if (!s || n_ids < 0 || (n_ids > 0 && (!ids || !lens || !in))) { g_err = "bad argument"; return TWL_ERR_BAD_ARGUMENT; }
    if (n_ids == 0) return TWL_OK;
    if (!rows_in_range(s, n_ids, ids, lens)) { g_err = "sequence id or length out of range"; return TWL_ERR_BAD_ARGUMENT; }
    DEVICE_CALL(call, s->d);
    RowMove m;
    m.write = true; m.n = n_ids; m.ids = ids; m.lens = lens; m.host = const_cast<char *>(in);
    return move_rows(s, call.st, m, row_offsets(n_ids, lens));
}

int twl_store_rows_to_block(twl_store *s, int32_t n_ids, const int32_t *ids, void *dev_block, int32_t *lens_out)
{
    if (!s || n_ids < 0 || (n_ids > 0 && (!ids || !lens_out || !dev_block))) { g_err = "bad argument"; return TWL_ERR_BAD_ARGUMENT; }
    if (!rows_in_range(s, n_ids, ids, nullptr)) { g_err = "sequence id out of range"; return TWL_ERR_BAD_ARGUMENT; }
    for (int32_t t = 0; t < n_ids; ++t) lens_out[t] = s->len[ids[t]];
    if (n_ids == 0) return TWL_OK;
    DEVICE_CALL(call, s->d);
    RowMove m;
    m.n = n_ids; m.ids = ids; m.lens = lens_out; m.block = dev_block;
    return move_rows(s, call.st, m, row_offsets(n_ids, lens_out));
}
int twl_store_rows_from_block(twl_store *s, int32_t n_ids, const int32_t *ids, const int32_t *lens, const void *dev_block)
{
    if (!s || n_ids < 0 || (n_ids > 0 && (!ids || !lens || !dev_block))) { g_err = "bad argument"; return TWL_ERR_BAD_ARGUMENT; }
    if (!rows_in_range(s, n_ids, ids, lens)) { g_err = "sequence id or length out of range"; return TWL_ERR_BAD_ARGUMENT; }
    if (n_ids == 0) return TWL_OK;
    DEVICE_CALL(call, s->d);
    RowMove m;
    m.write = true; m.n = n_ids; m.ids = ids; m.lens = lens; m.block = const_cast<void *>(dev_block);
    return move_rows(s, call.st, m, row_offsets(n_ids, lens));
}
int twl_store_exchange_buffers(twl_store *s, int64_t send_bytes, int64_t recv_bytes, void **send_dev, void **recv_dev)
{
    if (!s || send_bytes < 0 || recv_bytes < 0 || !send_dev || !recv_dev) { g_err = "bad argument"; return TWL_ERR_BAD_ARGUMENT; }
    DEVICE_CALL(call, s->d);
    int rc;
    if ((rc = s->x_send.ensure((size_t)std::max<int64_t>(send_bytes, 16)))) return rc;
    if ((rc = s->x_recv.ensure((size_t)std::max<int64_t>(recv_bytes, 16)))) return rc;
    *send_dev = s->x_send.p; *recv_dev = s->x_recv.p;
    return TWL_OK;
}

int twl_store_write_cache(twl_store *s, int32_t id, const float *data, int32_t len)
{
    if (!s || !data || len < 0 || id < 0) { g_err = "bad argument"; return TWL_ERR_BAD_ARGUMENT; }
    if (s->cache.count(id)) { g_err = "cache id in use"; return TWL_ERR_BAD_ARGUMENT; }
    DEVICE_CALL(call, s->d);
    CacheEntry e;
    const size_t bytes = (size_t)len * s->P * sizeof(float);
    int rc = e.take(call.d, len, std::max<size_t>(bytes, 16));
    if (rc) return rc;
    if (bytes) HIP_TRY(hipMemcpyAsync(e.buf.p, data, bytes, hipMemcpyHostToDevice, call.st));
    HIP_TRY(hipStreamSynchronize(call.st));
    s->cache[id] = std::move(e);
    return TWL_OK;
}

int twl_store_read_cache(twl_store *s, int32_t id, float *out, int32_t *len_out)
{
    if (!s) { g_err = "bad argument"; return TWL_ERR_BAD_ARGUMENT; }
    auto it = s->cache.find(id);
    if (it == s->cache.end()) { g_err = "unknown cache id"; return TWL_ERR_BAD_ARGUMENT; }
    if (len_out) *len_out = it->second.len;
    if (!out) return TWL_OK;
    DEVICE_CALL(call, s->d);
    HIP_TRY(hipStreamSynchronize(call.st));
    HIP_TRY(hipMemcpy(out, it->second.buf.p, (size_t)it->second.len * s->P * sizeof(float), hipMemcpyDeviceToHost));
    return TWL_OK;
}

int twl_store_drop_cache(twl_store *s, int32_t id)
{
    if (!s) { g_err = "bad argument"; return TWL_ERR_BAD_ARGUMENT; }
    auto it = s->cache.find(id);
    if (it == s->cache.end()) return TWL_OK;
    std::lock_guard<std::mutex> lk(s->d->mu);
    (void)hipSetDevice(s->d->id);
    (void)hipStreamSynchronize(s->d->stream);
    s->cache.erase(it);
    return TWL_OK;
}
// ... 3 lines not shown
```

twilight_amd/level.py:

```python
from __future__ import annotations

import ctypes as C
from dataclasses import dataclass
from typing import List, Optional, Sequence

import numpy as np

from . import api


class TwlSide(C.Structure):
    _fields_ = [("n_members", C.c_int32), ("member_off", C.c_int32), ("len", C.c_int32), ("num", C.c_int32), ("weight", C.c_float),
                ("cache_id", C.c_int32), ("store_id", C.c_int32), ("reserved", C.c_int32)]


_SYMBOLS = ["twl_store_create", "twl_store_destroy", "twl_store_read_rows", "twl_store_read_rows_of", "twl_store_write_rows", "twl_store_write_cache", "twl_store_rows_to_block", "twl_store_rows_from_block", "twl_store_exchange_buffers", "twl_store_read_cache", "twl_store_drop_cache",
            "twl_level_prepare", "twl_level_read_colinfo", "twl_level_read_colinfo_many", "twl_level_align", "twl_level_align_mixed", "twl_level_read_path", "twl_level_read_paths", "twl_level_commit", "twl_level_commit_from_dp", "twl_level_read_columns", "twl_level_timing",
            "twl_level_restore", "twl_level_read_final", "twl_level_exchange_buffers", "twl_level_paths_to_block", "twl_level_paths_from_block",
            "twl_level_write_final"]


def exported_symbols():
    return list(_SYMBOLS)


def _lib():
    lib = api.load_library()
    for name in _SYMBOLS:
        if name != "twl_store_destroy":
            getattr(lib, name).restype = C.c_int
    lib.twl_store_destroy.restype = None
    return lib


@dataclass
class Side:
    members: Sequence[int]
    member_weight: Sequence[float]
    len: int
    num: int
    weight: float
    cache_id: int = -1
    store_id: int = -1


class Store:

    def __init__(self, seqs: List[bytes], seq_type: str = "n", device: int = 0):
        lib = _lib()
        self.P = 6 if seq_type == "n" else 22
        self.n = len(seqs)
        arr = (C.c_char_p * self.n)(*seqs)
        lens = (C.c_int32 * self.n)(*[len(s) for s in seqs])
        self._h = C.c_void_p()
        api._check(lib.twl_store_create(C.c_int(device), C.c_char(seq_type.encode()), C.c_int32(self.n), arr, lens, C.byref(self._h)))
        self._n_pairs = 0
        self._seq_len = 0

    def close(self):
        if self._h:
            _lib().twl_store_destroy(self._h)
            self._h = C.c_void_p()

    def __del__(self):
        try:
            self.close()
        except Exception:
            pass

    def rows(self) -> List[bytes]:
        lib = _lib()
        lens = (C.c_int32 * self.n)()
        api._check(lib.twl_store_read_rows(self._h, None, lens))
        bufs = [C.create_string_buffer(max(int(n), 1)) for n in lens]
        ptrs = (C.c_void_p * self.n)(*[C.cast(b, C.c_void_p) for b in bufs])
        api._check(lib.twl_store_read_rows(self._h, ptrs, lens))
        return [bufs[i].raw[: lens[i]] for i in range(self.n)]

    def rows_of(self, ids: Sequence[int]) -> List[bytes]:
        lib = _lib()
        n = len(ids)
        idv = (C.c_int32 * n)(*ids)
        lens = (C.c_int32 * n)()
        api._check(lib.twl_store_read_rows_of(self._h, C.c_int32(n), idv, None, lens))
        buf = C.create_string_buffer(max(1, sum(lens)))
        api._check(lib.twl_store_read_rows_of(self._h, C.c_int32(n), idv, buf, lens))
        out, at = [], 0
        for k in range(n):
            out.append(buf.raw[at: at + lens[k]])
            at += lens[k]
        return out

    def write_rows(self, ids: Sequence[int], rows: Sequence[bytes], via_device_block: bool = False):
        lib = _lib()
        n = len(ids)
        idv = (C.c_int32 * n)(*ids)
        lens = (C.c_int32 * n)(*[len(r) for r in rows])
        blob = b"".join(rows)
        if not via_device_block:
            api._check(lib.twl_store_write_rows(self._h, C.c_int32(n), idv, blob, lens))
            return
        send, recv = C.c_void_p(), C.c_void_p()
        api._check(lib.twl_store_exchange_buffers(self._h, C.c_int64(len(blob)), C.c_int64(len(blob)), C.byref(send), C.byref(recv)))
        api._check(lib.twl_copy_to_device(C.c_int(0), recv, blob, C.c_uint64(len(blob))))
        api._check(lib.twl_store_rows_from_block(self._h, C.c_int32(n), idv, lens, recv))

    def rows_to_block(self, ids: Sequence[int]) -> List[bytes]:
        lib = _lib()
        n = len(ids)
        idv = (C.c_int32 * n)(*ids)
        lens = (C.c_int32 * n)()
        api._check(lib.twl_store_read_rows_of(self._h, C.c_int32(n), idv, None, lens))
        total = max(1, sum(lens))
        send, recv = C.c_void_p(), C.c_void_p()
        api._check(lib.twl_store_exchange_buffers(self._h, C.c_int64(total), C.c_int64(total), C.byref(send), C.byref(recv)))
        api._check(lib.twl_store_rows_to_block(self._h, C.c_int32(n), idv, send, lens))
        buf = C.create_string_buffer(total)
        api._check(lib.twl_copy_from_device(C.c_int(0), buf, send, C.c_uint64(total)))
        out, at = [], 0
        for k in range(n):
            out.append(buf.raw[at: at + lens[k]])
            at += lens[k]
        return out

    def write_cache(self, cache_id: int, profile: np.ndarray):
        prof = np.ascontiguousarray(profile, dtype=np.float32)
        api._check(_lib().twl_store_write_cache(self._h, C.c_int32(cache_id), prof.ctypes.data_as(C.POINTER(C.c_float)), C.c_int32(prof.shape[0])))

    def cache(self, cache_id: int) -> np.ndarray:
        lib = _lib()
        n = C.c_int32(0)
        api._check(lib.twl_store_read_cache(self._h, C.c_int32(cache_id), None, C.byref(n)))
        out = np.zeros((n.value, self.P), dtype=np.float32)
        api._check(lib.twl_store_read_cache(self._h, C.c_int32(cache_id), out.ctypes.data_as(C.POINTER(C.c_float)), C.byref(n)))
        return out

    def prepare(self, params: api.TwlParams, pairs: Sequence[Sequence[Side]], gappy_threshold: float = 0.95, seq_len: Optional[int] = None):
        lib = _lib()
        n = len(pairs)
        sides = (TwlSide * (2 * n))()
        members, weights = [], []
        for i, pr in enumerate(pairs):
            for sd in range(2):
                s = pr[sd]
                x = sides[2 * i + sd]
                x.n_members, x.member_off, x.len, x.num, x.weight = len(s.members), len(members), s.len, s.num, s.weight
                x.cache_id, x.store_id, x.reserved = s.cache_id, s.store_id, 0
                members.extend(int(m) for m in s.members)
                weights.extend(s.member_weight)
        sl = seq_len if seq_len is not None else max([1] + [s.len for pr in pairs for s in pr])
        mem = np.asarray(members, dtype=np.int32)
        w = np.asarray(weights, dtype=np.float32)
        lens = np.zeros((n, 2), dtype=np.int32)
        info = np.zeros((n, 2, sl), dtype=np.uint8)
        api._check(lib.twl_level_prepare(self._h, C.byref(params), C.c_float(gappy_threshold), C.c_int32(n), sides,
                                         mem.ctypes.data_as(C.POINTER(C.c_int32)), w.ctypes.data_as(C.POINTER(C.c_float)), C.c_int32(sl),
                                         lens.ctypes.data_as(C.POINTER(C.c_int32)), info.ctypes.data_as(C.POINTER(C.c_uint8))))
        self._n_pairs, self._seq_len, self._lens = n, sl, lens
        return lens, info

    def columns(self, pair: int, side: int) -> np.ndarray:
        n = int(self._lens[pair, side])
        out = np.zeros((n, self.P + 2), dtype=np.float32)
        api._check(_lib().twl_level_read_columns(self._h, C.c_int32(pair), C.c_int32(side), out.ctypes.data_as(C.POINTER(C.c_float)), C.c_int32(n)))
        return out

    def align(self, params: api.TwlParams, run_mask: Optional[np.ndarray] = None, zero_gap: Optional[np.ndarray] = None):
        n, sl = self._n_pairs, self._seq_len
        aln = np.zeros((n, 2 * sl), dtype=np.int8)
        aln_len = np.zeros(n, dtype=np.int32)
        err = np.zeros(n, dtype=np.int16)
        mask = None
# ... 68 lines not shown
```

Before: 232.7 billion.

## Build next-level profiles ahead on a side stream during current level

Adds a prepare-ahead path. While the current level is prepared, next-level operands whose nodes are not touched by this level have their frequency profiles built on a second stream into a dedicated buffer. The next prepare reuses these profiles when members, weights and row generations still match, which takes profile construction off the critical path. This costs extra row-generation tracking, a 256MB-bounded buffer, event synchronisation, and wasted work when built profiles go unused.

After: 232.0 billion. About the same (-0.3%).

```diff
diff --git a/include/twl_align.h b/include/twl_align.h
--- a/include/twl_align.h
+++ b/include/twl_align.h
@@ -89,7 +89,7 @@
 
 enum twl_knob { TWL_KNOB_MT_PERTURB = 1, TWL_KNOB_MT_MAX_PAIRS = 2, TWL_KNOB_MT_MIN_MARKER = 3, TWL_KNOB_MT_LEAD = 4, TWL_KNOB_MT_MARGIN = 5,
                 TWL_KNOB_MT_ROUNDS = 6, TWL_KNOB_MT_THR_JOBS = 7, TWL_KNOB_FAIL_ROW_ALLOCS = 8,
-                TWL_KNOB_PROT_MODE = 9, TWL_KNOB_ASSUME_ONEHOT_QUERY = 10, TWL_KNOB_MT_TAIL_PCT = 11, TWL_KNOB_MT_WIDE = 12, TWL_KNOB_NO_SPEC = 13, TWL_KNOB_SCOUT_XDROP_PCT = 14, TWL_KNOB_THR_SMALL = 15, TWL_KNOB_FORCE_GLOBAL = 16, TWL_KNOB_LEAF_STEP = 17, TWL_KNOB_POISON_TB = 18, TWL_KNOB_MT_ANCHOR = 19, TWL_KNOB_MT_LEAD2 = 20, TWL_KNOB_PROT_CORRIDOR = 21 };
+                TWL_KNOB_PROT_MODE = 9, TWL_KNOB_ASSUME_ONEHOT_QUERY = 10, TWL_KNOB_MT_TAIL_PCT = 11, TWL_KNOB_MT_WIDE = 12, TWL_KNOB_NO_SPEC = 13, TWL_KNOB_SCOUT_XDROP_PCT = 14, TWL_KNOB_THR_SMALL = 15, TWL_KNOB_FORCE_GLOBAL = 16, TWL_KNOB_LEAF_STEP = 17, TWL_KNOB_POISON_TB = 18, TWL_KNOB_MT_ANCHOR = 19, TWL_KNOB_MT_LEAD2 = 20, TWL_KNOB_PROT_CORRIDOR = 21, TWL_KNOB_PREPARE_AHEAD = 22 };
 int twl_set_knob(int key, int value);
 int twl_plan_describe(const twl_params *p, int32_t n_pairs, const int32_t *len, int32_t num_cu, int32_t qry_onehot, int32_t wide_streak, char *out, int32_t cap);
 
diff --git a/include/twl_level.h b/include/twl_level.h
--- a/include/twl_level.h
+++ b/include/twl_level.h
@@ -35,6 +35,9 @@
 int twl_level_prepare(twl_store *s, const twl_params *p, float gappy_threshold, int32_t n_pairs, const twl_side *sides,
                       const int32_t *members, const float *member_weight, int32_t seq_len, int32_t *len_out, uint8_t *colinfo_out);
 
+int twl_level_prepare_ahead(twl_store *s, int32_t n_sides, const twl_side *sides, const int32_t *members, const float *member_weight);
+int twl_level_ahead_counts(int64_t *built, int64_t *taken, int64_t *dropped);
+
 int twl_level_read_colinfo(twl_store *s, int32_t pair, int32_t side, uint8_t *out);
 int twl_level_read_colinfo_many(twl_store *s, int32_t n_sel, const int32_t *pairs, uint8_t *out);
 
diff --git a/twilight_amd/api.py b/twilight_amd/api.py
--- a/twilight_amd/api.py
+++ b/twilight_amd/api.py
@@ -141,6 +141,7 @@
 KNOB_MT_ANCHOR = 19
 KNOB_PROT_CORRIDOR = 21
 KNOB_MT_LEAD2 = 20
+KNOB_PREPARE_AHEAD = 22
 PROT_MODES = {"auto": 0, "dense": 1, "sparse": 2, "presim": 3, "r1": 4, "lean_sparse": 5, "lean_presim": 6}
 
 
diff --git a/twilight_amd/csrc/host/align_resident.cpp b/twilight_amd/csrc/host/align_resident.cpp
--- a/twilight_amd/csrc/host/align_resident.cpp
+++ b/twilight_amd/csrc/host/align_resident.cpp
@@ -1,4 +1,5 @@
 #include "align_gpu.hpp"
+#include "../twl_level_plan.inc.hip"
 
 #include <cstring>
 #include <omp.h>
@@ -9,6 +10,9 @@
 #include <iostream>
 #include <string>
 #include <thread>
+#include <unordered_map>
+
+extern "C" int twl_level_prepare_ahead(twl_store *, int32_t, const twl_side *, const int32_t *, const float *) __attribute__((weak));
 
 namespace msa {
 namespace progressive {
@@ -247,6 +251,63 @@
     }
 }
 
+Node *contentHolder(Node *x, const Node *partner)
+{
+    if (x->is_leaf() || !x->seqsIncluded.empty()) return x;
+    for (Node *c : x->children)
+        if ((c->grpID == -1 || c->grpID == x->grpID) && c->identifier != partner->identifier) return c;
+    return nullptr;
+}
+
+void prepareAhead(const Level &lv, RunCtx &ctx, const NodePairVec *next)
+{
+    constexpr size_t kAheadMaxPairs = 256;
+    if (!twl_level_prepare_ahead || !next || next->empty() || next->size() > kAheadMaxPairs || lv.nodes.size() > kAheadMaxPairs || lv.task != 0 || lv.nd != 1 || lv.route.procs || lv.route.devX || !lv.route.inPlace || lv.option->alnMode != DEFAULT_ALN) return;
+    std::unordered_map<const Node *, int32_t> idOf;
+    auto id = [&](const Node *n) { return n ? idOf.emplace(n, (int32_t)idOf.size()).first->second : -1; };
+    std::vector<int32_t> front;
+    for (const auto &pr : lv.nodes) { front.push_back(id(pr.first)); front.push_back(id(pr.second)); }
+    std::vector<AheadOperand> ops;
+    std::vector<Node *> holders;
+    for (const auto &pr : *next)
+        for (int sd = 0; sd < 2; ++sd) {
+            Node *x = sd ? pr.second : pr.first;
+            Node *h = contentHolder(x, sd ? pr.first : pr.second);
+            ops.push_back(h ? AheadOperand{id(x), h == x ? -1 : id(h)} : AheadOperand{-1, -1});
+            holders.push_back(h);
+        }
+    const std::vector<uint8_t> fin = plan_ahead_final((int32_t)lv.nodes.size(), front.data(), (int32_t)ops.size(), ops.data());
+    std::vector<twl_side> sides;
+    std::vector<int32_t> members;
+    std::vector<float> weights;
+    for (size_t t = 0; t < ops.size(); ++t) {
+        if (!fin[t]) continue;
+        const Node *h = holders[t];
+        twl_side x{};
+        x.member_off = (int32_t)members.size();
+        x.cache_id = x.store_id = -1;
+        if (h->is_leaf() && h->seqsIncluded.empty()) {
+            const auto it = lv.database->name_map.find(h->identifier);
+            if (it == lv.database->name_map.end()) continue;
+            const auto *q = it->second;
+            x.n_members = 1; x.len = q->len; x.num = 1; x.weight = q->weight;
+            members.push_back(q->id);
+            weights.push_back(q->weight / x.weight * x.num);
+        } else {
+            if (h->cacheId >= 0 || h->seqsIncluded.empty()) continue;
+            x.n_members = (int32_t)h->seqsIncluded.size(); x.len = h->alnLen; x.num = h->alnNum; x.weight = h->alnWeight;
+            bool plain = true;
+            for (int sIdx : h->seqsIncluded) plain = plain && sIdx >= 0;
+            if (!plain) continue;
+            for (int sIdx : h->seqsIncluded) { members.push_back(sIdx); weights.push_back(lv.database->sequences[sIdx]->weight / x.weight * x.num); }
+        }
+        sides.push_back(x);
+    }
+    if (sides.empty()) return;
+    const int rc = twl_level_prepare_ahead(firstStore(ctx), (int32_t)sides.size(), sides.data(), members.data(), weights.data());
+    if (rc != TWL_OK) die("twl_level_prepare_ahead", rc);
+}
+
 void fetchColumnInfo(const Level &lv, const std::vector<int> &which, bool wholeBlock, std::vector<ColumnInfo> &cols)
 {
     if (which.empty()) return;
@@ -634,6 +695,7 @@
     const Level &lv = level;
     PairRows rows(n);
     if (!lv.route.inPlace) fetchColumnInfo(lv, lv.needInfo, lv.needInfo.size() * 8 > (size_t)n, rows.cols);
+    prepareAhead(lv, ctx, database->nextLevel);
     ctx.totals.prepare_ms += nowMs() - tPrep;
 
     planDp(level, rows);
diff --git a/twilight_amd/csrc/host/progressive.cpp b/twilight_amd/csrc/host/progressive.cpp
--- a/twilight_amd/csrc/host/progressive.cpp
+++ b/twilight_amd/csrc/host/progressive.cpp
@@ -144,7 +144,9 @@
         auto t0 = std::chrono::high_resolution_clock::now();
         updateNode(T, m, database);
         auto t1 = std::chrono::high_resolution_clock::now();
+        database->nextLevel = (database->currentTask == 0 && (size_t)level + 1 < levels.size()) ? &levels[(size_t)level + 1] : nullptr;
         kernel(T, m, database, option, param);
+        database->nextLevel = nullptr;
         auto ms = std::chrono::duration_cast<std::chrono::milliseconds>(std::chrono::high_resolution_clock::now() - t0).count();
         if (option->printDetail)
             std::cerr << "Level " << level + 1 << ", aligned " << m.size() << (m.size() > 1 ? " pairs in " : " pair in ") << ms << " ms (nodes "
diff --git a/twilight_amd/csrc/host/twl_host.hpp b/twilight_amd/csrc/host/twl_host.hpp
--- a/twilight_amd/csrc/host/twl_host.hpp
+++ b/twilight_amd/csrc/host/twl_host.hpp
@@ -167,6 +167,7 @@
     std::function<size_t(Tree *, std::vector<std::vector<std::pair<Node *, Node *>>> &, Option *, Params &)> ownedPrefix;
     std::function<void(Tree *)> afterMainPass;
     bool residentDeferred = false;
+    const std::vector<std::pair<Node *, Node *>> *nextLevel = nullptr;
     bool lazyRows = false;
     void addSequence(int id, const std::string &name, std::string &seq, int subtreeIdx, float weight, bool debug);
     bool debug();
diff --git a/twilight_amd/csrc/level_kernels.hip.h b/twilight_amd/csrc/level_kernels.hip.h
--- a/twilight_amd/csrc/level_kernels.hip.h
+++ b/twilight_amd/csrc/level_kernels.hip.h
@@ -12,7 +12,7 @@
     float weight;
     int32_t cache_slot;
     int32_t store_slot;
-    int32_t pad;
+    int32_t ahead;
 };
 
 struct LevelArgs {
@@ -29,6 +29,7 @@
     float *cols;
     int32_t *len_out;
     int32_t *chunk_cnt;
+    float *ahead;
     int32_t n_chunks;
     int32_t stride;
     float gappy_thr;
@@ -36,7 +37,7 @@
     float gap_open, gap_extend, scale, min_gap_open, min_gap_extend;
 };
 
-template <int P>
+template <int P, bool AHEAD = false>
 __global__ void __launch_bounds__(256) profile_kernel(LevelArgs a)
 {
     __shared__ uint8_t s_lut[256];
@@ -63,6 +64,14 @@
 #pragma unroll
                 for (int v = 0; v < P; ++v) acc[k][v] = c[k * P + v] / sd.weight * fnum;
             }
+    } else if (!AHEAD && sd.ahead > 0) {
+        const float *c = a.ahead + ((size_t)(sd.ahead - 1) + t0) * P;
+#pragma unroll
+        for (int k = 0; k < 4; ++k)
+            if (k < nc) {
+#pragma unroll
+                for (int v = 0; v < P; ++v) acc[k][v] = c[k * P + v];
+            }
     } else {
         constexpr int U = (P == 6) ? 16 : 2;
         auto add = [&](uint32_t four, float w) __attribute__((always_inline)) {
@@ -92,15 +101,25 @@
             const char *row = (a.member_plane[mi] ? a.rows1 : a.rows0) + (size_t)a.member_seq[mi] * a.cap;
             add(*reinterpret_cast<const uint32_t *>(row + t0), a.member_w[mi]);
         }
-        if (sd.store_slot >= 0) {
-            float *c = a.cache[sd.store_slot] + (size_t)t0 * P;
-#pragma unroll
-            for (int k = 0; k < 4; ++k)
-                if (k < nc) {
-#pragma unroll
-                    for (int v = 0; v < P; ++v) c[k * P + v] = acc[k][v] / fnum * sd.weight;
-                }
-        }
+    }
+    if (AHEAD) {
+        float *dst = a.ahead + ((size_t)(sd.ahead - 1) + t0) * P;
+#pragma unroll
+        for (int k = 0; k < 4; ++k)
+            if (k < nc) {
+#pragma unroll
+                for (int v = 0; v < P; ++v) dst[k * P + v] = acc[k][v];
+            }
+        return;
+    }
+    if (sd.cache_slot < 0 && sd.store_slot >= 0) {
+        float *c = a.cache[sd.store_slot] + (size_t)t0 * P;
+#pragma unroll
+        for (int k = 0; k < 4; ++k)
+            if (k < nc) {
+#pragma unroll
+                for (int v = 0; v < P; ++v) c[k * P + v] = acc[k][v] / fnum * sd.weight;
+            }
     }
     float *dst = a.raw + ((size_t)side * a.stride + t0) * P;
 #pragma unroll
@@ -136,6 +155,7 @@
         kept += (a.remove && gappy) ? 0 : 1;
     }
     }
+    if (AHEAD) return;
     {
         int x = kept;
 #pragma unroll
diff --git a/twilight_amd/csrc/twl_align.hip b/twilight_amd/csrc/twl_align.hip
--- a/twilight_amd/csrc/twl_align.hip
+++ b/twilight_amd/csrc/twl_align.hip
@@ -562,6 +562,7 @@
     case TWL_KNOB_FORCE_GLOBAL: g_force_global = value ? 1 : 0; return TWL_OK;
     case TWL_KNOB_LEAF_STEP: g_leaf_step = value ? 1 : 0; return TWL_OK;
     case TWL_KNOB_POISON_TB: g_poison_tb = value ? 1 : 0; return TWL_OK;
+    case TWL_KNOB_PREPARE_AHEAD: g_prepare_ahead = value ? 1 : 0; return TWL_OK;
     case TWL_KNOB_MT_ANCHOR: g_mt_anchor = value ? 1 : 0; return TWL_OK;
     case TWL_KNOB_MT_LEAD2: if (value < 0) { g_mt_lead2 = 96; g_mt_lead2_lat = 128; } else g_mt_lead2 = g_mt_lead2_lat = std::max(16, value); return TWL_OK;
     case TWL_KNOB_PROT_CORRIDOR: g_prot_corridor = std::max(0, value); for (auto *d : g_devs) d->mem.forget_corridor(); return TWL_OK;
diff --git a/twilight_amd/csrc/twl_knobs.inc.hip b/twilight_amd/csrc/twl_knobs.inc.hip
--- a/twilight_amd/csrc/twl_knobs.inc.hip
+++ b/twilight_amd/csrc/twl_knobs.inc.hip
@@ -15,3 +15,4 @@
 int g_assume_onehot_query = 0;
 int g_leaf_step = 1;
 int g_poison_tb = 0;
+int g_prepare_ahead = 1;
diff --git a/twilight_amd/csrc/twl_level.inc.hip b/twilight_amd/csrc/twl_level.inc.hip
--- a/twilight_amd/csrc/twl_level.inc.hip
+++ b/twilight_amd/csrc/twl_level.inc.hip
@@ -15,6 +15,27 @@
     }
     for (size_t k = 0; k < fresh.size(); ++k) s->cache[pp.newIds[k]] = std::move(fresh[k]);
     return TWL_OK;
+}
+
+int take_ahead(twl_store *s, PreparePlan &pp, const twl_side *sides, const int32_t *members, const float *member_weight)
+{
+    AheadSet &ah = s->ahead;
+    if (ah.built.empty()) return 0;
+    int taken = 0;
+    pp.readsRows = false;
+    for (size_t i = 0; i < pp.dsides.size(); ++i) {
+        const twl_side &sd = sides[i];
+        if (sd.cache_id >= 0 || sd.n_members < 1) continue;
+        const auto it = ah.byFirst.find(members[sd.member_off]);
+        bool take = it != ah.byFirst.end() && ahead_matches(ah.built[it->second], sd, members, member_weight);
+        for (int32_t m = 0; take && m < sd.n_members; ++m) take = s->row_gen[members[sd.member_off + m]] <= ah.gen;
+        if (take) { pp.dsides[i].pad = (int32_t)(ah.built[it->second].col_off + 1); ++taken; }
+        else pp.readsRows = true;
+    }
+    g_ahead_counts[1] += taken;
+    g_ahead_counts[2] += (int64_t)ah.built.size() - taken;
+    ah.forget();
+    return taken;
 }
 
 int upload_prepare(twl_store *s, hipStream_t st, const PreparePlan &pp, const float *member_weight)
@@ -69,6 +90,7 @@
     a.min_gap_extend = p->gap_extend * 0.2;
     a.min_gap_open = p->gap_open * 0.1;
     a.chunk_cnt = (int32_t *)lv->d_ccnt.p;
+    a.ahead = (float *)s->ahead.raw.p;
     a.n_chunks = chunks;
     return a;
 }
@@ -329,6 +351,7 @@
 {
     const CommitPlan &cp = s->commit;
     for (size_t k = 0; k < cp.flips.size(); k += 2) { s->plane[cp.flips[k]] ^= 1; s->len[cp.flips[k]] = cp.flips[k + 1]; }
+    s->rows_written(cp.flips.data(), cp.flips.size() / 2, 2);
     for (size_t k = 0; k < merged.size(); ++k) {
         s->cache[cp.mergeIds[2 * k]] = std::move(merged[k]);
         s->cache.erase(cp.mergeIds[2 * k + 1]);
@@ -401,6 +424,8 @@
     s->members.assign(members, members + pp.nm);
     s->h_num.swap(pp.h_num);
     if ((rc = register_stored(s, pp))) return rc;
+    const int taken = take_ahead(s, pp, sides, members, member_weight);
+    if (taken) HIP_TRY(hipStreamWaitEvent(st, s->ahead.ev, 0));
     if (pp.readsRows && (rc = wait_rows(s, st))) return rc;
     HIP_TRY(hipEventRecord(d->ev[0], st));
     if ((rc = upload_prepare(s, st, pp, member_weight))) return rc;
@@ -413,6 +438,87 @@
     HIP_TRY(hipEventElapsedTime(&ms, d->ev[0], d->ev[1]));
     s->prepare_ms = ms;
     s->prepared = true;
+    if (taken) s->ahead.pending = false;
+    return TWL_OK;
+}
+
+int twl_level_prepare_ahead(twl_store *s, int32_t n_sides, const twl_side *sides, const int32_t *members, const float *member_weight)
+{
+    if (!s || n_sides < 0 || (n_sides > 0 && (!sides || !members || !member_weight))) { g_err = "bad argument"; return TWL_ERR_BAD_ARGUMENT; }
+    if (!g_prepare_ahead || n_sides == 0) return TWL_OK;
+    int32_t maxLen = 1;
+    size_t nm = 0;
+    for (int32_t i = 0; i < n_sides; ++i) {
+        const twl_side &sd = sides[i];
+        if (sd.n_members < 1 || sd.member_off < 0 || sd.len < 0 || sd.num < 1 || sd.cache_id >= 0) { g_err = "bad side descriptor (sides built ahead are built from rows)"; return TWL_ERR_BAD_ARGUMENT; }
+        for (int32_t m = 0; m < sd.n_members; ++m) {
+            const int32_t q = members[sd.member_off + m];
+            if (q < 0 || q >= s->n_seqs) { g_err = "member sequence id out of range"; return TWL_ERR_BAD_ARGUMENT; }
+            if (s->len[q] != sd.len) { g_err = "member row length differs from the side's len"; return TWL_ERR_BAD_ARGUMENT; }
+        }
+        maxLen = std::max(maxLen, sd.len);
+        nm = std::max(nm, (size_t)sd.member_off + (size_t)sd.n_members);
+    }
+    std::vector<int64_t> off;
+    int64_t bytes = 0;
+    if (!plan_ahead_layout(n_sides, sides, s->P, kAheadBudget, off, &bytes)) return TWL_OK;
+    DEVICE_CALL(call, s->d);
+    Device *d = call.d;
+    AheadSet &ah = s->ahead;
+    if (!ah.ev) { HIP_TRY(hipEventCreateWithFlags(&ah.ev_in, hipEventDisableTiming)); HIP_TRY(hipEventCreateWithFlags(&ah.ev, hipEventDisableTiming)); }
+    if (ah.pending) HIP_TRY(hipEventSynchronize(ah.ev));
+    ah.pending = false;
+    ah.forget();
+    int rc;
+    if ((rc = ah.raw.ensure(std::max<size_t>((size_t)bytes, 16)))) return rc;
+    std::vector<SideRow> rows((size_t)n_sides);
+    std::vector<uint8_t> mplane(nm, 0);
+    ah.built.resize((size_t)n_sides);
+    for (int32_t i = 0; i < n_sides; ++i) {
+        const twl_side &sd = sides[i];
+        rows[i] = SideRow{sd.n_members, sd.member_off, sd.len, sd.num, sd.weight, -1, -1, (int32_t)(off[i] + 1)};
+        for (int32_t m = 0; m < sd.n_members; ++m) mplane[sd.member_off + m] = s->plane[members[sd.member_off + m]];
+        AheadSide &b = ah.built[i];
+        b.side = sd; b.col_off = off[i];
+        b.members.assign(members + sd.member_off, members + sd.member_off + sd.n_members);
+        b.weights.assign(member_weight + sd.member_off, member_weight + sd.member_off + sd.n_members);
+        ah.byFirst[b.members[0]] = i;
+    }
+    ah.gen = s->gen;
+    Arena &A = ah.up;
+    if ((rc = A.begin((size_t)n_sides * sizeof(SideRow) + nm * (sizeof(int32_t) + sizeof(float) + 1), 4))) { ah.forget(); return rc; }
+    A.put(ah.d_sides, rows);
+    A.put(ah.d_mseq, members, nm);
+    A.put(ah.d_mw, member_weight, nm);
+    A.put(ah.d_mplane, mplane);
+    hipStream_t st2 = d->stream2;
+    HIP_TRY(hipEventRecord(ah.ev_in, call.st));
+    HIP_TRY(hipStreamWaitEvent(st2, ah.ev_in, 0));
+    if ((rc = A.flush(st2))) { ah.forget(); return rc; }
+    twl::LevelArgs a{};
+    a.sides = ah.d_sides.as<const twl::SideDesc>();
+    a.member_seq = ah.d_mseq.as<const int32_t>();
+    a.member_w = ah.d_mw.as<const float>();
+    a.member_plane = ah.d_mplane.as<const uint8_t>();
+    a.rows0 = (const char *)s->rows[0].p; a.rows1 = (const char *)s->rows[1].p;
+    a.cap = s->cap;
+    a.lut = (const uint8_t *)s->lut.p;
+    a.ahead = (float *)ah.raw.p;
+    const dim3 grid((unsigned)n_sides, (unsigned)((maxLen + 1023) / 1024));
+    if (s->P == 6) hipLaunchKernelGGL((twl::profile_kernel<6, true>), grid, dim3(256), 0, st2, a);
+    else hipLaunchKernelGGL((twl::profile_kernel<22, true>), grid, dim3(256), 0, st2, a);
+    ah.pending = true;
+    HIP_TRY(hipGetLastError());
+    HIP_TRY(hipEventRecord(ah.ev, st2));
+    g_ahead_counts[0] += n_sides;
+    return TWL_OK;
+}
+
+int twl_level_ahead_counts(int64_t *built, int64_t *taken, int64_t *dropped)
+{
+    if (built) *built = g_ahead_counts[0];
+    if (taken) *taken = g_ahead_counts[1];
+    if (dropped) *dropped = g_ahead_counts[2];
     return TWL_OK;
 }
 
diff --git a/twilight_amd/csrc/twl_level_plan.inc.hip b/twilight_amd/csrc/twl_level_plan.inc.hip
--- a/twilight_amd/csrc/twl_level_plan.inc.hip
+++ b/twilight_amd/csrc/twl_level_plan.inc.hip
@@ -1,5 +1,6 @@
 #include <algorithm>
 #include <cstdint>
+#include <cstring>
 #include <unordered_map>
 #include <vector>
 #include "../../include/twl_level.h"
@@ -78,6 +79,54 @@
     return pp;
 }
 
+
+struct AheadOperand { int32_t node, adopts_from; };
+
+inline std::vector<uint8_t> plan_ahead_final(int32_t n_front, const int32_t *front, int32_t n_next, const AheadOperand *next)
+{
+    std::vector<int32_t> busy(front, front + 2 * (size_t)n_front);
+    std::sort(busy.begin(), busy.end());
+    auto touched = [&](int32_t node) { return std::binary_search(busy.begin(), busy.end(), node); };
+    std::vector<uint8_t> fin((size_t)n_next, 0);
+    for (int32_t t = 0; t < n_next; ++t) {
+        const AheadOperand &o = next[t];
+        if (o.node < 0 || o.adopts_from < -1) continue;
+        fin[t] = !touched(o.node) && (o.adopts_from < 0 || !touched(o.adopts_from));
+    }
+    return fin;
+}
+
+constexpr int64_t kAheadBudget = 256ll << 20;
+
+inline bool plan_ahead_layout(int32_t n_sides, const twl_side *sides, int P, int64_t budget, std::vector<int64_t> &col_off, int64_t *bytes)
+{
+    col_off.assign((size_t)n_sides, 0);
+    int64_t cols = 0;
+    for (int32_t i = 0; i < n_sides; ++i) {
+        if (sides[i].n_members < 1 || sides[i].len < 0 || sides[i].cache_id >= 0) return false;
+        col_off[i] = cols;
+        cols += ((int64_t)sides[i].len + 3) & ~(int64_t)3;
+        if (cols * P * (int64_t)sizeof(float) > budget) return false;
+    }
+    *bytes = cols * P * (int64_t)sizeof(float);
+    return true;
+}
+
+struct AheadSide {
+    twl_side side;
+    std::vector<int32_t> members;
+    std::vector<float> weights;
+    int64_t col_off = 0;
+};
+
+inline bool ahead_matches(const AheadSide &built, const twl_side &now, const int32_t *members, const float *weights)
+{
+    const twl_side &b = built.side;
+    if (now.cache_id >= 0 || now.n_members != b.n_members || now.len != b.len || now.num != b.num || memcmp(&now.weight, &b.weight, sizeof(float))) return false;
+    if (memcmp(members + now.member_off, built.members.data(), (size_t)b.n_members * sizeof(int32_t))) return false;
+    return memcmp(weights + now.member_off, built.weights.data(), (size_t)b.n_members * sizeof(float)) == 0;
+}
+
 struct AlignPlan {
     std::vector<int32_t> lm;
     bool qryOneHot = true;
diff --git a/twilight_amd/csrc/twl_store.inc.hip b/twilight_amd/csrc/twl_store.inc.hip
--- a/twilight_amd/csrc/twl_store.inc.hip
+++ b/twilight_amd/csrc/twl_store.inc.hip
@@ -1,3 +1,4 @@
+#include <atomic>
 #include <cstdlib>
 #include "twl_path_source.inc.hip"
 
@@ -183,6 +184,26 @@
     for (Buf &b : cache_pool(d)) b.release();
     cache_pool(d).clear();
 }
+
+struct AheadSet {
+    Arena up;
+    Ref d_sides, d_mseq, d_mw, d_mplane;
+    Buf raw;
+    std::vector<AheadSide> built;
+    std::unordered_map<int32_t, int32_t> byFirst;
+    uint64_t gen = 0;
+    hipEvent_t ev_in = nullptr, ev = nullptr;
+    bool pending = false;
+    void forget() { built.clear(); byFirst.clear(); }
+    void release()
+    {
+        forget();
+        up.release(); raw.release();
+        if (ev_in) (void)hipEventDestroy(ev_in);
+        if (ev) (void)hipEventDestroy(ev);
+        ev_in = ev = nullptr; pending = false;
+    }
+};
 
 struct twl_store {
     Device *d = nullptr;
@@ -211,6 +232,10 @@
     Buf d_gather;
     Buf x_send, x_recv;
     double prepare_ms = 0, commit_ms = 0;
+    AheadSet ahead;
+    uint64_t gen = 0;
+    std::vector<uint64_t> row_gen;
+    void rows_written(const int32_t *ids, size_t n, size_t step = 1) { ++gen; for (size_t k = 0; k < n; ++k) row_gen[ids[k * step]] = gen; }
 };
 
 namespace {
@@ -247,6 +272,7 @@
     return std::max<int64_t>(256, budget / (2 * std::max<int64_t>(1, s->n_seqs)));
 }
 
+std::atomic<int64_t> g_ahead_counts[3];
 int g_fail_next_row_allocs = 0;
 
 int grow_rows(twl_store *s, int64_t need, int64_t want = 0)
@@ -291,6 +317,7 @@
         release_level(s->lv);
         for (Buf *b : {&s->rows[0], &s->rows[1], &s->lut, &s->d_gather, &s->x_send, &s->x_recv}) b->release();
         s->up_rows.release();
+        s->ahead.release();
         s->d->live_stores -= 1;
     }
 };
@@ -298,6 +325,7 @@
 int wait_rows(twl_store *s, hipStream_t st)
 {
     if (s->rows_event) { HIP_TRY(hipStreamWaitEvent(st, s->rows_event, 0)); s->rows_event = nullptr; }
+    if (s->ahead.pending) HIP_TRY(hipStreamWaitEvent(st, s->ahead.ev, 0));
     return TWL_OK;
 }
 
@@ -308,7 +336,11 @@
     a.out0 = (char *)s->rows[0].p; a.out1 = (char *)s->rows[1].p;
     a.cap = s->cap;
 }
-void rows_rewritten(twl_store *s, const std::vector<int32_t> &ids, int32_t W) { for (int32_t id : ids) { s->plane[id] ^= 1; s->len[id] = W; } }
+void rows_rewritten(twl_store *s, const std::vector<int32_t> &ids, int32_t W)
+{
+    for (int32_t id : ids) { s->plane[id] ^= 1; s->len[id] = W; }
+    s->rows_written(ids.data(), ids.size());
+}
 
 PathLevelView path_level_view(const twl_store *s)
 {
@@ -386,7 +418,7 @@
     HIP_TRY(hipGetLastError());
     if (!m.write && m.host && t.total) HIP_TRY(hipMemcpyAsync(m.host, packed, (size_t)t.total, hipMemcpyDeviceToHost, st));
     HIP_TRY(hipStreamSynchronize(st));
-    if (m.write) for (int32_t k = 0; k < m.n; ++k) s->len[m.ids[k]] = m.lens[k];
+    if (m.write) { for (int32_t k = 0; k < m.n; ++k) s->len[m.ids[k]] = m.lens[k]; s->rows_written(m.ids, (size_t)m.n); }
     return TWL_OK;
 }
 
@@ -419,6 +451,7 @@
     s->n_seqs = n_seqs;
     s->plane.assign((size_t)n_seqs, 0);
     s->len.assign(lens, lens + n_seqs);
+    s->row_gen.assign((size_t)n_seqs, 0);
     int64_t maxLen = 1;
     for (int32_t i = 0; i < n_seqs; ++i) {
         if (lens[i] < 0) { g_err = "negative sequence length"; return TWL_ERR_BAD_ARGUMENT; }
diff --git a/twilight_amd/level.py b/twilight_amd/level.py
--- a/twilight_amd/level.py
+++ b/twilight_amd/level.py
@@ -17,7 +17,7 @@
 _SYMBOLS = ["twl_store_create", "twl_store_destroy", "twl_store_read_rows", "twl_store_read_rows_of", "twl_store_write_rows", "twl_store_write_cache", "twl_store_rows_to_block", "twl_store_rows_from_block", "twl_store_exchange_buffers", "twl_store_read_cache", "twl_store_drop_cache",
             "twl_level_prepare", "twl_level_read_colinfo", "twl_level_read_colinfo_many", "twl_level_align", "twl_level_align_mixed", "twl_level_read_path", "twl_level_read_paths", "twl_level_commit", "twl_level_commit_from_dp", "twl_level_read_columns", "twl_level_timing",
             "twl_level_restore", "twl_level_read_final", "twl_level_exchange_buffers", "twl_level_paths_to_block", "twl_level_paths_from_block",
-            "twl_level_write_final"]
+            "twl_level_write_final", "twl_level_prepare_ahead", "twl_level_ahead_counts"]
 
 
 def exported_symbols():
```
